# foges/pogs

Measured on AMD Instinct MI355X. Metric: admm_iterations_per_sec_dense_lasso_fp32 (per-GPU shard, summed over GPUs), higher is better.
Workload: dtype f32; 1 GPU; solve_lasso dense fp32 A=100000x10000 per GPU, lambda=0.1, default tolerances (BASELINE.json configs[1]); rows_per_gpu=100000, cols=10000, projector=direct (MFMA Gram + Cholesky), parallelism=row-shard x1, rccl_nranks=0

## Files before the change

include/pogs_amd.h:

```cpp
#ifndef POGS_AMD_H_
#define POGS_AMD_H_

#include <stddef.h>

#ifdef __cplusplus
extern "C" {
#endif


enum ORD { COL_MAJ, ROW_MAJ };

enum FUNCTION { ABS, EXP, HUBER, IDENTITY, INDBOX01, INDEQ0, INDGE0, INDLE0,
                LOGISTIC, MAXNEG0, MAXPOS0, NEGENTR, NEGLOG, RECIPR, SQUARE, ZERO };

enum POGS_STATUS { POGS_SUCCESS = 0, POGS_INFEASIBLE = 1, POGS_UNBOUNDED = 2,
                   POGS_MAX_ITER = 3, POGS_NAN_FOUND = 4, POGS_INVALID_CONE = 5,
                   POGS_ERROR = 6 };

int PogsD(enum ORD ord, size_t m, size_t n, const double *A,
          const double *f_a, const double *f_b, const double *f_c,
          const double *f_d, const double *f_e, const enum FUNCTION *f_h,
          const double *g_a, const double *g_b, const double *g_c,
          const double *g_d, const double *g_e, const enum FUNCTION *g_h,
          double rho, double abs_tol, double rel_tol, unsigned int max_iter,
          unsigned int verbose, int adaptive_rho, int gap_stop,
          double *x, double *y, double *l, double *optval, unsigned int *final_iter);

int PogsS(enum ORD ord, size_t m, size_t n, const float *A,
          const float *f_a, const float *f_b, const float *f_c,
          const float *f_d, const float *f_e, const enum FUNCTION *f_h,
          const float *g_a, const float *g_b, const float *g_c,
          const float *g_d, const float *g_e, const enum FUNCTION *g_h,
          float rho, float abs_tol, float rel_tol, unsigned int max_iter,
          unsigned int verbose, int adaptive_rho, int gap_stop,
          float *x, float *y, float *l, float *optval, unsigned int *final_iter);

int PogsSparseD(enum ORD ord, size_t m, size_t n, size_t nnz,
                const double *data, const int *ptr, const int *ind,
                const double *f_a, const double *f_b, const double *f_c,
                const double *f_d, const double *f_e, const enum FUNCTION *f_h,
                const double *g_a, const double *g_b, const double *g_c,
                const double *g_d, const double *g_e, const enum FUNCTION *g_h,
                double rho, double abs_tol, double rel_tol, unsigned int max_iter,
                unsigned int verbose, int adaptive_rho, int gap_stop,
                double *x, double *y, double *l, double *optval,
                unsigned int *final_iter);

int PogsSparseS(enum ORD ord, size_t m, size_t n, size_t nnz,
                const float *data, const int *ptr, const int *ind,
                const float *f_a, const float *f_b, const float *f_c,
                const float *f_d, const float *f_e, const enum FUNCTION *f_h,
                const float *g_a, const float *g_b, const float *g_c,
                const float *g_d, const float *g_e, const enum FUNCTION *g_h,
                float rho, float abs_tol, float rel_tol, unsigned int max_iter,
                unsigned int verbose, int adaptive_rho, int gap_stop,
                float *x, float *y, float *l, float *optval,
                unsigned int *final_iter);


typedef struct PogsAmdSolver PogsAmdSolver;

enum POGS_AMD_DTYPE { POGS_AMD_F32 = 0, POGS_AMD_F64 = 1 };
enum POGS_AMD_MEM { POGS_AMD_HOST = 0, POGS_AMD_DEVICE = 1 };
enum POGS_AMD_PROJECTOR { POGS_AMD_PROJ_DEFAULT = 0,
                          POGS_AMD_PROJ_DIRECT = 1, POGS_AMD_PROJ_CGLS = 2 };

#define POGS_AMD_UNIQUE_ID_BYTES 128

typedef struct PogsAmdDist {
  int rank;
  int world;
  size_t m_global;
  char unique_id[POGS_AMD_UNIQUE_ID_BYTES];
} PogsAmdDist;

typedef struct PogsAmdOptions {
  int device;
  int projector;
  int profile;
  int reserved[5];
} PogsAmdOptions;

typedef struct PogsAmdStats {
  double t_total_s, t_init_s, t_loop_s, t_h2d_s;
  unsigned int iterations;
  unsigned int exact_iters;
  unsigned int norm_est_iters;
  unsigned int rho_updates;
  unsigned long long cg_iters;
  unsigned long long matvecs;
  unsigned long long matvecs_init;
  double rho_final, nrmA;
  double stream_ms;
  unsigned long long stream_launches;
  double stream_bytes;
  double equil_ms, normest_ms, gram_ms, chol_ms, trtri_ms;
  double gram_flops;
  double reserved[8];
} PogsAmdStats;

int PogsAmdDistUniqueId(char *out);

int PogsAmdCreateDense(PogsAmdSolver **out, int dtype, enum ORD ord, size_t m,
                       size_t n, const void *A, int mem,
                       const PogsAmdOptions *opt, const PogsAmdDist *dist);

int PogsAmdCreateSparse(PogsAmdSolver **out, int dtype, enum ORD ord, size_t m,
                        size_t n, size_t nnz, const void *data, const int *ptr,
                        const int *ind, int mem, const PogsAmdOptions *opt,
                        const PogsAmdDist *dist);

int PogsAmdSolve(PogsAmdSolver *s,
                 const void *f_a, const void *f_b, const void *f_c, const void *f_d,
                 const void *f_e, const int *f_h,
                 const void *g_a, const void *g_b, const void *g_c, const void *g_d,
                 const void *g_e, const int *g_h,
                 double rho, double abs_tol, double rel_tol, unsigned int max_iter,
                 unsigned int verbose, int adaptive_rho, int gap_stop,
                 void *x, void *y, void *l, void *mu, double *optval,
                 unsigned int *final_iter);

typedef struct PogsAmdFn {
  const void *a, *b, *c, *d, *e;
  const int *h;
  double a0, b0, c0, d0, e0;
  int h0;
} PogsAmdFn;
int PogsAmdSolveFn(PogsAmdSolver *s, const PogsAmdFn *f, const PogsAmdFn *g,
                   double rho, double abs_tol, double rel_tol, unsigned int max_iter,
                   unsigned int verbose, int adaptive_rho, int gap_stop,
                   void *x, void *y, void *l, void *mu, double *optval,
                   unsigned int *final_iter);
int PogsAmdBeginRunFn(PogsAmdSolver *s, const PogsAmdFn *f, const PogsAmdFn *g,
                      double rho, double abs_tol, double rel_tol, unsigned int max_iter,
                      int adaptive_rho, int gap_stop);

#define POGS_AMD_BATCH_MAX 16
int PogsAmdSolveBatchFn(PogsAmdSolver *s, int k, const PogsAmdFn *f, const PogsAmdFn *g, const double *rho,
                        double abs_tol, double rel_tol, unsigned int max_iter, unsigned int verbose,
                        int adaptive_rho, int gap_stop, void *x, void *y, void *l, void *mu,
                        double *optval, unsigned int *final_iter, int *status);

int PogsAmdSolveBatchSparseFn(PogsAmdSolver *s, int k, const PogsAmdFn *f, const PogsAmdFn *g, const double *rho,
                              double abs_tol, double rel_tol, unsigned int max_iter, unsigned int verbose,
                              int adaptive_rho, int gap_stop, void *x, void *y, void *l, void *mu,
                              double *optval, unsigned int *final_iter, int *status);

#define POGS_AMD_MANY_MIN_DIM_MAX 512
#define POGS_AMD_MANY_MAX_DIM_MAX 16384
int PogsAmdSolveManyFn(int dtype, enum ORD ord, int k, size_t m, size_t n, const void *A, int mem,
                       const PogsAmdOptions *opt, const PogsAmdFn *f, const PogsAmdFn *g, const double *rho,
                       double abs_tol, double rel_tol, unsigned int max_iter, unsigned int verbose,
                       int adaptive_rho, int gap_stop, void *x, void *y, void *l, void *mu,
                       double *optval, unsigned int *final_iter, int *status);

int PogsAmdBeginRun(PogsAmdSolver *s,
                    const void *f_a, const void *f_b, const void *f_c, const void *f_d,
                    const void *f_e, const int *f_h,
                    const void *g_a, const void *g_b, const void *g_c, const void *g_d,
                    const void *g_e, const int *g_h,
                    double rho, double abs_tol, double rel_tol, unsigned int max_iter,
                    int adaptive_rho, int gap_stop);
int PogsAmdIterate(PogsAmdSolver *s, unsigned int iters, double *seconds,
                   unsigned int *solves_completed);

int PogsAmdSetWarmStart(PogsAmdSolver *s, const void *x0, const void *l0);

int PogsAmdGetStats(const PogsAmdSolver *s, PogsAmdStats *out);
int PogsAmdResetStats(PogsAmdSolver *s);
void PogsAmdDestroy(PogsAmdSolver *s);

const char *PogsAmdLastError(void);

typedef struct PogsAmdPoolInfo {
  unsigned long long mallocs;
  unsigned long long reuses;
  unsigned long long frees;
  double malloc_ms, free_ms;
  size_t cached_bytes;
  size_t live_bytes;
  size_t peak_cached_bytes;
} PogsAmdPoolInfo;
int PogsAmdPoolStats(int device, PogsAmdPoolInfo *out);
int PogsAmdPoolTrim(int device, size_t *freed_bytes);


int PogsAmdProxEval(int dtype, size_t n, const int *h, const void *a, const void *b,
                    const void *c, const void *d, const void *e, double rho,
                    const void *in, void *out);
int PogsAmdFuncEval(int dtype, size_t n, const int *h, const void *a, const void *b,
                    const void *c, const void *d, const void *e, const void *in,
                    double *out);
int PogsAmdProjSubgradEval(int dtype, size_t n, const int *h, const void *a, const void *b,
                           const void *c, const void *d, const void *e, const void *x_in,
                           const void *v_in, void *v_out);
int PogsAmdGetEquil(const PogsAmdSolver *s, void *A_eq, void *d, void *e, double *nrmA);
int PogsAmdProject(PogsAmdSolver *s, const void *x0, const void *y0, double tol,
                   void *x, void *y);
int PogsAmdMul(PogsAmdSolver *s, char trans, double alpha, const void *x, double beta,
               void *y);
int PogsAmdReadBandwidth(int device, size_t bytes, int reps, double *gb_per_s, int *pattern);
int PogsAmdWaveSumCheck(int dtype, size_t n, const void *in_host, void *alu_host, void *lds_host);

int PogsAmdBatchRowsCheck(int dtype, int tri, int rows, int cols, const void *M, size_t ldm, int k, const int *act,
                          int nact, const void *X, size_t ldx, void *Y, size_t ldy);
int PogsAmdBatchColsCheck(int dtype, int rows, int cols, const void *M, size_t ldm, int k, const int *act, int nact,
                          const void *U, size_t ldu, const void *add, void *Z, size_t ldz, int *nrb_used, int *rpb);
int PogsAmdSpBatchSpmvCheck(int dtype, int nrows, int ncols, const int *ptr, const int *ind, const void *val, int k,
                            const int *act, int nact, const void *X, size_t ldx, double beta, const void *yin,
                            size_t ldin, void *Y, size_t ldy, double *part, int num_cu, int *geom);
int PogsAmdManySetupCheck(int dtype, enum ORD ord, int k, size_t m, size_t n, const void *A, int mem, void *A_eq,
                          void *d, void *e, double *nrmA, void *W);
int PogsAmdGramCheck(int dtype, int kdim, int k, const void *P, size_t lda, int num_cu, int force, void *G, size_t ldg,
                     int *info);
int PogsAmdCholCheck(int dtype, int n, const void *H, size_t ldh, void *L, void *W, void *U, size_t ldo);
int PogsAmdSpmvCheck(int dtype, enum ORD ord, int nrows, int ncols, const int *ptr, const int *ind, const void *val,
                     int num_cu, int format, int force_rr_rows, int force_ncg, double scale, char trans, int sq,
                     double x_nrm2, double alpha, double beta, const void *x, size_t xlen, void *y, size_t ylen,
                     double *sumsq, int *info, int *t_ptr, int *t_ind, void *t_val);
int PogsAmdGetFactor(const PogsAmdSolver *s, void *W, void *U);
int PogsAmdRandUniform(int dtype, size_t n, void *out_host);

#ifdef __cplusplus
}
#endif
#endif
```

pogs_amd/_lib.py:

```python
import ctypes
import os
import sys

_PKG = os.path.dirname(os.path.abspath(__file__))
LIB_PATH = os.path.join(_PKG, "libpogs_amd.so")

TORCH_LOADED_FIRST = "torch" in sys.modules
if not TORCH_LOADED_FIRST and os.environ.get("POGS_AMD_TORCH_PRELOAD", "0") == "1":
    try:
        import torch

        TORCH_LOADED_FIRST = True
    except ImportError:
        pass


def check_device_pointer_interop():
    if "torch" in sys.modules and not TORCH_LOADED_FIRST:
        raise RuntimeError(
            "pogs_amd was imported before torch: the two then run on separate HIP runtimes and a torch device "
            "pointer is not valid here.  Import torch first, or set POGS_AMD_TORCH_PRELOAD=1.")


if not os.path.exists(LIB_PATH):
    raise ImportError(
        "pogs_amd: %s not found. Build it with:\n"
        "  python pogs_amd/build.py        (needs hipcc; cross-compiles for gfx950 without a GPU)\n" % LIB_PATH
    )

lib = ctypes.CDLL(LIB_PATH)

c_int, c_uint, c_size_t, c_double, c_float, c_void_p, c_char = (
    ctypes.c_int, ctypes.c_uint, ctypes.c_size_t, ctypes.c_double, ctypes.c_float, ctypes.c_void_p, ctypes.c_char)

UNIQUE_ID_BYTES = 128
F32, F64 = 0, 1
HOST, DEVICE = 0, 1
COL_MAJ, ROW_MAJ = 0, 1
PROJ_DEFAULT, PROJ_DIRECT, PROJ_CGLS = 0, 1, 2


class PogsAmdDist(ctypes.Structure):
    _fields_ = [("rank", c_int), ("world", c_int), ("m_global", c_size_t), ("unique_id", c_char * UNIQUE_ID_BYTES)]


class PogsAmdOptions(ctypes.Structure):
    _fields_ = [("device", c_int), ("projector", c_int), ("profile", c_int), ("reserved", c_int * 5)]


class PogsAmdStats(ctypes.Structure):
    _fields_ = [
        ("t_total_s", c_double), ("t_init_s", c_double), ("t_loop_s", c_double), ("t_h2d_s", c_double),
        ("iterations", c_uint), ("exact_iters", c_uint), ("norm_est_iters", c_uint), ("rho_updates", c_uint),
        ("cg_iters", ctypes.c_ulonglong), ("matvecs", ctypes.c_ulonglong), ("matvecs_init", ctypes.c_ulonglong),
        ("rho_final", c_double), ("nrmA", c_double),
        ("stream_ms", c_double), ("stream_launches", ctypes.c_ulonglong), ("stream_bytes", c_double),
        ("equil_ms", c_double), ("normest_ms", c_double), ("gram_ms", c_double), ("chol_ms", c_double),
        ("trtri_ms", c_double), ("gram_flops", c_double), ("reserved", c_double * 8),
    ]

    def as_dict(self):
        d = {k: getattr(self, k) for k, _ in self._fields_ if k != "reserved"}
        d["spec_hits"], d["spec_misses"] = self.reserved[0], self.reserved[1]
        d["collectives"] = int(self.reserved[2])
        d["comm_nranks"] = int(self.reserved[3])
        d["batch_problem_iters"] = int(self.reserved[4])
        d["batch_pass_ms"], d["batch_pass_launches"] = self.reserved[5], int(self.reserved[6])
        d["batch_pass_bytes"] = self.reserved[7]
        return d


def _dense_sig(real):
    return [c_int, c_size_t, c_size_t, c_void_p] + [c_void_p] * 5 + [c_void_p] + [c_void_p] * 5 + [c_void_p] + \
        [real, real, real, c_uint, c_uint, c_int, c_int, c_void_p, c_void_p, c_void_p, c_void_p, c_void_p]


def _sparse_sig(real):
    return [c_int, c_size_t, c_size_t, c_size_t, c_void_p, c_void_p, c_void_p] + [c_void_p] * 5 + [c_void_p] + \
        [c_void_p] * 5 + [c_void_p] + [real, real, real, c_uint, c_uint, c_int, c_int,
                                        c_void_p, c_void_p, c_void_p, c_void_p, c_void_p]


lib.PogsD.argtypes = _dense_sig(c_double)
lib.PogsS.argtypes = _dense_sig(c_float)
lib.PogsSparseD.argtypes = _sparse_sig(c_double)
lib.PogsSparseS.argtypes = _sparse_sig(c_float)
for _f in (lib.PogsD, lib.PogsS, lib.PogsSparseD, lib.PogsSparseS):
    _f.restype = c_int

lib.PogsAmdDistUniqueId.argtypes = [c_void_p]
lib.PogsAmdCreateDense.argtypes = [ctypes.POINTER(c_void_p), c_int, c_int, c_size_t, c_size_t, c_void_p, c_int,
                                   ctypes.POINTER(PogsAmdOptions), ctypes.POINTER(PogsAmdDist)]
lib.PogsAmdCreateSparse.argtypes = [ctypes.POINTER(c_void_p), c_int, c_int, c_size_t, c_size_t, c_size_t, c_void_p,
                                    c_void_p, c_void_p, c_int, ctypes.POINTER(PogsAmdOptions),
                                    ctypes.POINTER(PogsAmdDist)]
lib.PogsAmdSolve.argtypes = [c_void_p] + [c_void_p] * 12 + [c_double, c_double, c_double, c_uint, c_uint, c_int, c_int,
                                                            c_void_p, c_void_p, c_void_p, c_void_p,
                                                            ctypes.POINTER(c_double), ctypes.POINTER(c_uint)]
class PogsAmdFn(ctypes.Structure):
    _fields_ = [("a", c_void_p), ("b", c_void_p), ("c", c_void_p), ("d", c_void_p), ("e", c_void_p), ("h", c_void_p),
                ("a0", c_double), ("b0", c_double), ("c0", c_double), ("d0", c_double), ("e0", c_double), ("h0", c_int)]


lib.PogsAmdSolveFn.argtypes = [c_void_p, ctypes.POINTER(PogsAmdFn), ctypes.POINTER(PogsAmdFn), c_double, c_double, c_double,
                               c_uint, c_uint, c_int, c_int, c_void_p, c_void_p, c_void_p, c_void_p,
                               ctypes.POINTER(c_double), ctypes.POINTER(c_uint)]
lib.PogsAmdSolveBatchFn.argtypes = [c_void_p, c_int, ctypes.POINTER(PogsAmdFn), ctypes.POINTER(PogsAmdFn), c_void_p,
                                    c_double, c_double, c_uint, c_uint, c_int, c_int, c_void_p, c_void_p, c_void_p,
                                    c_void_p, c_void_p, c_void_p, c_void_p]
lib.PogsAmdSolveBatchSparseFn.argtypes = lib.PogsAmdSolveBatchFn.argtypes
BATCH_MAX = 16
lib.PogsAmdSolveManyFn.argtypes = [c_int, c_int, c_int, c_size_t, c_size_t, c_void_p, c_int, ctypes.POINTER(PogsAmdOptions),
                                   ctypes.POINTER(PogsAmdFn), ctypes.POINTER(PogsAmdFn), c_void_p, c_double, c_double,
                                   c_uint, c_uint, c_int, c_int, c_void_p, c_void_p, c_void_p, c_void_p, c_void_p,
                                   c_void_p, c_void_p]
MANY_MIN_DIM_MAX = 512
MANY_MAX_DIM_MAX = 16384
lib.PogsAmdBeginRunFn.argtypes = [c_void_p, ctypes.POINTER(PogsAmdFn), ctypes.POINTER(PogsAmdFn), c_double, c_double, c_double,
                                  c_uint, c_int, c_int]
lib.PogsAmdBeginRun.argtypes = [c_void_p] + [c_void_p] * 12 + [c_double, c_double, c_double, c_uint, c_int, c_int]
lib.PogsAmdIterate.argtypes = [c_void_p, c_uint, ctypes.POINTER(c_double), ctypes.POINTER(c_uint)]
lib.PogsAmdSetWarmStart.argtypes = [c_void_p, c_void_p, c_void_p]
lib.PogsAmdGetStats.argtypes = [c_void_p, ctypes.POINTER(PogsAmdStats)]
lib.PogsAmdResetStats.argtypes = [c_void_p]
lib.PogsAmdDestroy.argtypes = [c_void_p]
lib.PogsAmdDestroy.restype = None
lib.PogsAmdLastError.restype = ctypes.c_char_p
lib.PogsAmdProxEval.argtypes = [c_int, c_size_t] + [c_void_p] * 6 + [c_double, c_void_p, c_void_p]
lib.PogsAmdFuncEval.argtypes = [c_int, c_size_t] + [c_void_p] * 6 + [c_void_p, ctypes.POINTER(c_double)]
lib.PogsAmdProjSubgradEval.argtypes = [c_int, c_size_t] + [c_void_p] * 6 + [c_void_p, c_void_p, c_void_p]
lib.PogsAmdGetEquil.argtypes = [c_void_p, c_void_p, c_void_p, c_void_p, ctypes.POINTER(c_double)]
lib.PogsAmdProject.argtypes = [c_void_p, c_void_p, c_void_p, c_double, c_void_p, c_void_p]
lib.PogsAmdMul.argtypes = [c_void_p, c_char, c_double, c_void_p, c_double, c_void_p]
lib.PogsAmdRandUniform.argtypes = [c_int, c_size_t, c_void_p]
lib.PogsAmdReadBandwidth.argtypes = [c_int, c_size_t, c_int, ctypes.POINTER(c_double), ctypes.POINTER(c_int)]
lib.PogsAmdWaveSumCheck.argtypes = [c_int, c_size_t, c_void_p, c_void_p, c_void_p]
lib.PogsAmdBatchRowsCheck.argtypes = [c_int, c_int, c_int, c_int, c_void_p, c_size_t, c_int, c_void_p, c_int,
                                      c_void_p, c_size_t, c_void_p, c_size_t]
lib.PogsAmdBatchColsCheck.argtypes = [c_int, c_int, c_int, c_void_p, c_size_t, c_int, c_void_p, c_int, c_void_p,
                                      c_size_t, c_void_p, c_void_p, c_size_t, ctypes.POINTER(c_int),
                                      ctypes.POINTER(c_int)]
lib.PogsAmdSpBatchSpmvCheck.argtypes = [c_int, c_int, c_int, c_void_p, c_void_p, c_void_p, c_int, c_void_p, c_int,
                                        c_void_p, c_size_t, c_double, c_void_p, c_size_t, c_void_p, c_size_t, c_void_p,
                                        c_int, c_void_p]
lib.PogsAmdManySetupCheck.argtypes = [c_int, c_int, c_int, c_size_t, c_size_t, c_void_p, c_int, c_void_p, c_void_p,
                                      c_void_p, c_void_p, c_void_p]
lib.PogsAmdGramCheck.argtypes = [c_int, c_int, c_int, c_void_p, c_size_t, c_int, c_int, c_void_p, c_size_t, c_void_p]
lib.PogsAmdCholCheck.argtypes = [c_int, c_int, c_void_p, c_size_t, c_void_p, c_void_p, c_void_p, c_size_t]
lib.PogsAmdSpmvCheck.argtypes = [c_int, c_int, c_int, c_int, c_void_p, c_void_p, c_void_p, c_int, c_int, c_int, c_int,
                                 c_double, c_char, c_int, c_double, c_double, c_double, c_void_p, c_size_t, c_void_p,
                                 c_size_t, ctypes.POINTER(c_double), c_void_p, c_void_p, c_void_p, c_void_p]
lib.PogsAmdGetFactor.argtypes = [c_void_p, c_void_p, c_void_p]
GRAM_AUTO, GRAM_NATIVE, GRAM_TILE_128, GRAM_TILE_256 = 0, 1, 128, 256
GRAM_INFO = ("path", "tile", "ksplit", "kchunk", "kacc", "units", "unit_rows", "tile_map")
SPMV_AUTO, SPMV_TAGS, SPMV_TWO, SPMV_PLAIN = 0, 1, 2, 3
SPMV_INFO = ("tiled", "two", "rr_rows", "nrr", "ncb", "ncg", "units", "why")
SPMV_WHY = {0: "tiled", 1: "no non-zeros", 2: "plan too large", 3: "planner range", 4: "padding", 5: "row count over 16 bits",
            6: "pinned plain"}


class PogsAmdPoolInfo(ctypes.Structure):
    _fields_ = [("mallocs", ctypes.c_ulonglong), ("reuses", ctypes.c_ulonglong), ("frees", ctypes.c_ulonglong),
                ("malloc_ms", c_double), ("free_ms", c_double), ("cached_bytes", c_size_t), ("live_bytes", c_size_t),
                ("peak_cached_bytes", c_size_t)]


lib.PogsAmdPoolStats.argtypes = [c_int, ctypes.POINTER(PogsAmdPoolInfo)]
lib.PogsAmdPoolTrim.argtypes = [c_int, ctypes.POINTER(c_size_t)]


def pool_stats(device=-1):
    info = PogsAmdPoolInfo()
    if lib.PogsAmdPoolStats(device, ctypes.byref(info)) != 0:
        raise RuntimeError(last_error())
    return {k: getattr(info, k) for k, _ in info._fields_}


def pool_trim(device=-1):
    freed = c_size_t(0)
    if lib.PogsAmdPoolTrim(device, ctypes.byref(freed)) != 0:
        raise RuntimeError(last_error())
    return freed.value

ABI_SYMBOLS = [
    "PogsD", "PogsS", "PogsSparseD", "PogsSparseS",
    "PogsAmdDistUniqueId", "PogsAmdCreateDense", "PogsAmdCreateSparse", "PogsAmdSolve", "PogsAmdSolveFn", "PogsAmdSolveBatchFn", "PogsAmdSolveBatchSparseFn",
    "PogsAmdSolveManyFn", "PogsAmdBeginRun", "PogsAmdBeginRunFn",
    "PogsAmdIterate", "PogsAmdSetWarmStart", "PogsAmdGetStats", "PogsAmdResetStats", "PogsAmdDestroy", "PogsAmdLastError",
    "PogsAmdPoolStats", "PogsAmdPoolTrim",
    "PogsAmdProxEval", "PogsAmdFuncEval", "PogsAmdProjSubgradEval", "PogsAmdGetEquil", "PogsAmdProject", "PogsAmdMul", "PogsAmdRandUniform",
    "PogsAmdReadBandwidth", "PogsAmdWaveSumCheck", "PogsAmdBatchRowsCheck", "PogsAmdBatchColsCheck",
    "PogsAmdSpBatchSpmvCheck", "PogsAmdManySetupCheck", "PogsAmdGramCheck", "PogsAmdCholCheck",
    "PogsAmdSpmvCheck", "PogsAmdGetFactor",
]


def read_bandwidth(device=-1, nbytes=4 << 30, reps=10):
    gbs, pat = c_double(0.0), c_int(0)
    if lib.PogsAmdReadBandwidth(device, nbytes, reps, ctypes.byref(gbs), ctypes.byref(pat)) != 0:
        raise RuntimeError(last_error())
    return gbs.value, ("side-by-side grid stride", "row blocks")[pat.value]


def wave_sum_check(values):
    import numpy as np
    v = np.ascontiguousarray(values)
    assert v.dtype in (np.float32, np.float64) and v.size % 64 == 0
    a, b = np.empty_like(v), np.empty_like(v)
    if lib.PogsAmdWaveSumCheck(0 if v.dtype == np.float32 else 1, v.size, v.ctypes.data, a.ctypes.data, b.ctypes.data) != 0:
        raise RuntimeError(last_error())
    return a, b


def _dtype_code(*arrays):
    import numpy as np
    dt = arrays[0].dtype
    if dt not in (np.float32, np.float64) or any(a.dtype != dt for a in arrays[1:]):
        raise ValueError("float32 or float64 arrays of one dtype")
    return 0 if dt == np.float32 else 1


def _act(act):
    import numpy as np
    return np.ascontiguousarray(act, dtype=np.int32).ravel()


def batch_rows_check(tri, M, cols, X, Y, act):
    import numpy as np
    M, X = np.ascontiguousarray(M), np.ascontiguousarray(X)
    Y = np.array(Y, order="C", copy=True)
    code = _dtype_code(M, X, Y)
    if M.ndim != 2 or X.ndim != 2 or Y.ndim != 2 or X.shape[0] != Y.shape[0]:
        raise ValueError("M (rows, ldm), X (k, ldx), Y (k, ldy)")
    a = _act(act)
    if lib.PogsAmdBatchRowsCheck(code, tri, M.shape[0], cols, M.ctypes.data, M.shape[1], X.shape[0], a.ctypes.data,
                                 a.size, X.ctypes.data, X.shape[1], Y.ctypes.data, Y.shape[1]) != 0:
        raise RuntimeError(last_error())
    return Y


def batch_cols_check(M, cols, U, Z, act, add=None):
    import numpy as np
    M, U = np.ascontiguousarray(M), np.ascontiguousarray(U)
    Z = np.array(Z, order="C", copy=True)
    arrays = (M, U, Z) if add is None else (M, U, Z, np.ascontiguousarray(add))
    code = _dtype_code(*arrays)
    if M.ndim != 2 or U.ndim != 2 or Z.ndim != 2 or U.shape[0] != Z.shape[0] or \
            (add is not None and arrays[3].shape != Z.shape):
        raise ValueError("M (rows, ldm), U (k, ldu), Z and add (k, ldz)")
    a = _act(act)
    nrb, rpb = c_int(0), c_int(0)
    if lib.PogsAmdBatchColsCheck(code, M.shape[0], cols, M.ctypes.data, M.shape[1], U.shape[0], a.ctypes.data, a.size,
                                 U.ctypes.data, U.shape[1], None if add is None else arrays[3].ctypes.data,
                                 Z.ctypes.data, Z.shape[1], ctypes.byref(nrb), ctypes.byref(rpb)) != 0:
        raise RuntimeError(last_error())
    return Z, nrb.value, rpb.value


def sp_batch_spmv_check(ptr, ind, val, ncols, X, Y, act, beta=0.0, yin=None, part_fill=None, num_cu=0):
    import numpy as np
    ptr, ind = np.ascontiguousarray(ptr, dtype=np.int32), np.ascontiguousarray(ind, dtype=np.int32)
    val, X = np.ascontiguousarray(val), np.ascontiguousarray(X)
    Y = np.array(Y, order="C", copy=True)
    arrays = (val, X, Y) if yin is None else (val, X, Y, np.ascontiguousarray(yin))
    code = _dtype_code(*arrays)
    nrows = ptr.size - 1
    if X.ndim != 2 or Y.ndim != 2 or X.shape[0] != Y.shape[0] or nrows < 0 or \
            (yin is not None and (arrays[3].ndim != 2 or arrays[3].shape[0] != Y.shape[0])):
        raise ValueError("ptr (nrows + 1), X (k, ldx), Y (k, ldy), yin (k, ldin)")
    nnz = max(int(ptr[-1]), 0) if ptr.size else 0
    if ind.size < nnz or val.size < nnz:
        raise ValueError("ind and val must hold ptr[-1] entries")
    a = _act(act)
    k = X.shape[0]
    part = None
    if part_fill is not None:
        part = np.full(k * max(1, -(-nrows // 4)), part_fill, dtype=np.float64)
    geom = np.zeros(3, dtype=np.int32)
    if lib.PogsAmdSpBatchSpmvCheck(code, nrows, ncols, ptr.ctypes.data, ind.ctypes.data, val.ctypes.data, k,
                                   a.ctypes.data, a.size, X.ctypes.data, X.shape[1], beta,
                                   None if yin is None else arrays[3].ctypes.data,
                                   0 if yin is None else arrays[3].shape[1], Y.ctypes.data, Y.shape[1],
                                   None if part is None else part.ctypes.data, num_cu, geom.ctypes.data) != 0:
        raise RuntimeError(last_error())
    grid = int(geom[2])
    return Y, (None if part is None else part[:k * grid].reshape(k, grid)), tuple(int(g) for g in geom)


def many_setup_check(A, ord=ROW_MAJ):
    import numpy as np
    A = np.asarray(A)
    if A.ndim != 3:
        raise ValueError("A must be k x m x n")
    code = _dtype_code(A)
    k, m, n = A.shape
    src = np.ascontiguousarray(A.transpose(0, 2, 1) if ord == COL_MAJ else A)
    K = min(m, n)
    out = dict(A_eq=np.empty((k, m, n), A.dtype), d=np.empty((k, m), A.dtype), e=np.empty((k, n), A.dtype),
               nrmA=np.empty(k, np.float64), W=np.empty((k, K, K), A.dtype))
    if lib.PogsAmdManySetupCheck(code, ord, k, m, n, src.ctypes.data, HOST, out["A_eq"].ctypes.data,
                                 out["d"].ctypes.data, out["e"].ctypes.data, out["nrmA"].ctypes.data,
                                 out["W"].ctypes.data) != 0:
        raise RuntimeError(last_error())
    return out


def gram_check(P, k, G, force=GRAM_AUTO, num_cu=0):
    import numpy as np
    P = np.ascontiguousarray(P)
    G = np.array(G, order="C", copy=True)
    code = _dtype_code(P, G)
    if P.ndim != 2 or G.ndim != 2 or G.shape[0] != k:
        raise ValueError("P (kdim, lda), G (k, ldg)")
    info = np.zeros(8, dtype=np.int32)
    if lib.PogsAmdGramCheck(code, P.shape[0], k, P.ctypes.data, P.shape[1], num_cu, force, G.ctypes.data, G.shape[1],
                            info.ctypes.data) != 0:
        raise RuntimeError(last_error())
    return G, dict(zip(GRAM_INFO, (int(v) for v in info)))


def spmv_check(ptr, ind, val, shape, x, y, trans="n", ord=ROW_MAJ, num_cu=0, format=SPMV_AUTO, force_rr_rows=0,
               force_ncg=0, scale=1.0, sq=False, x_nrm2=0.0, alpha=1.0, beta=0.0, transpose=False):
    import numpy as np
    ptr, ind = np.ascontiguousarray(ptr, dtype=np.int32), np.ascontiguousarray(ind, dtype=np.int32)
    val, x = np.ascontiguousarray(val), np.ascontiguousarray(x)
    y = np.array(y, order="C", copy=True)
    code = _dtype_code(val, x, y)
    nrows, ncols = int(shape[0]), int(shape[1])
    r1, c1 = (nrows, ncols) if ord == ROW_MAJ else (ncols, nrows)
    if ptr.ndim != 1 or ptr.size != r1 + 1 or x.ndim != 1 or y.ndim != 1:
        raise ValueError("ptr (rows of the given copy + 1), x and y vectors")
    nnz = max(int(ptr[-1]), 0)
    if ind.size < nnz or val.size < nnz:
        raise ValueError("ind and val must hold ptr[-1] entries")
    info = np.zeros(16, dtype=np.int32)
    sumsq = c_double(0.0)
    t = None
    if transpose:
        t = (np.zeros(c1 + 1, np.int32), np.zeros(max(nnz, 1), np.int32), np.zeros(max(nnz, 1), val.dtype))
    if lib.PogsAmdSpmvCheck(code, ord, nrows, ncols, ptr.ctypes.data, ind.ctypes.data, val.ctypes.data, num_cu, format,
                            force_rr_rows, force_ncg, scale, trans.encode(), int(bool(sq)), x_nrm2, alpha, beta,
                            x.ctypes.data, x.size, y.ctypes.data, y.size, ctypes.byref(sumsq), info.ctypes.data,
                            *((None, None, None) if t is None else (a.ctypes.data for a in t))) != 0:
        raise RuntimeError(last_error())
    infos = tuple(dict(zip(SPMV_INFO, (int(v) for v in info[8 * c:8 * c + 8]))) for c in range(2))
    if t is None:
        return y, sumsq.value, infos
    return y, sumsq.value, infos, (t[0], t[1][:nnz], t[2][:nnz])


def chol_check(H, ldo=None):
    import numpy as np
    H = np.ascontiguousarray(H)
    code = _dtype_code(H)
    if H.ndim != 2 or H.shape[1] < H.shape[0]:
        raise ValueError("H (n, ldh >= n)")
    n = H.shape[0]
    ldo = n if ldo is None else ldo
    L, W, U = (np.full((n, ldo), np.nan, H.dtype) for _ in range(3))
    if lib.PogsAmdCholCheck(code, n, H.ctypes.data, H.shape[1], L.ctypes.data, W.ctypes.data, U.ctypes.data, ldo) != 0:
        raise RuntimeError(last_error())
    return L, W, U


def get_factor(handle, k, dtype):
    import numpy as np
    W, U = np.zeros((k, k), dtype), np.zeros((k, k), dtype)
    if lib.PogsAmdGetFactor(handle, W.ctypes.data, U.ctypes.data) != 0:
        raise RuntimeError(last_error())
    return W, U


def last_error():
    msg = lib.PogsAmdLastError()
    return msg.decode() if msg else ""
```

pogs_amd/csrc/abi.hip:

```cpp
#include <cmath>
#include <cstring>
#include <string>
#include <utility>
#include <vector>

#include "engine.h"
#include "factor_check.h"
#include "many_kernels.h"
#include "sparse_batch_kernels.h"
#include "spmv_check.h"
#include "prox.h"
#include "stream.h"
#include "vec_kernels.h"

namespace pogs_amd {

#define POGS_DECLARE_PLAN(TPB_, NV_)                                                                               \
  SolverBase *make_dense_solver_f32_p##TPB_##_##NV_(int, size_t, size_t, const void *, int, const PogsAmdOptions *, \
                                                    const PogsAmdDist *);                                          \
  SolverBase *make_dense_solver_f64_p##TPB_##_##NV_(int, size_t, size_t, const void *, int, const PogsAmdOptions *, \
                                                    const PogsAmdDist *);
POGS_STREAM_PLANS(POGS_DECLARE_PLAN)
#undef POGS_DECLARE_PLAN
SolverBase *make_dense_solver_f32_xl(int, size_t, size_t, const void *, int, const PogsAmdOptions *, const PogsAmdDist *);
// ... 237 lines not shown
    DistComm::unique_id(out);
    return 0;
  });
}

int PogsAmdCreateDense(PogsAmdSolver **out, int dtype, enum ORD ord, size_t m, size_t n, const void *A, int mem,
                       const PogsAmdOptions *opt, const PogsAmdDist *dist) {
  return guarded([&]() {
    *out = nullptr;
    DeviceGuard guard(opt ? opt->device : -1);
    std::unique_ptr<PogsAmdSolver> h(new PogsAmdSolver);
    h->impl.reset(make_dense_solver(dtype, ord, m, n, A, mem, opt, dist));
    *out = h.release();
    return 0;
  });
}

int PogsAmdCreateSparse(PogsAmdSolver **out, int dtype, enum ORD ord, size_t m, size_t n, size_t nnz,
                        const void *data, const int *ptr, const int *ind, int mem, const PogsAmdOptions *opt,
                        const PogsAmdDist *dist) {
  return guarded([&]() {
    *out = nullptr;
    DeviceGuard guard(opt ? opt->device : -1);
    std::unique_ptr<PogsAmdSolver> h(new PogsAmdSolver);
    h->impl.reset(make_sparse_solver(dtype, ord, m, n, nnz, data, ptr, ind, mem, opt, dist));
    *out = h.release();
    return 0;
  });
}

int PogsAmdSolve(PogsAmdSolver *s, const void *f_a, const void *f_b, const void *f_c, const void *f_d,
                 const void *f_e, const int *f_h, const void *g_a, const void *g_b, const void *g_c,
                 const void *g_d, const void *g_e, const int *g_h, double rho, double abs_tol, double rel_tol,
                 unsigned int max_iter, unsigned int verbose, int adaptive_rho, int gap_stop, void *x, void *y,
                 void *l, void *mu, double *optval, unsigned int *final_iter) {
  return guarded([&]() {
    POGS_CHECK(s && s->impl, "null solver");
    DeviceGuard guard(s->impl->device());
    const FnHost f = fn_arrays(f_a, f_b, f_c, f_d, f_e, f_h, "f");
    const FnHost g = fn_arrays(g_a, g_b, g_c, g_d, g_e, g_h, "g");
    return s->impl->solve(f, g, make_params(rho, abs_tol, rel_tol, max_iter, verbose, adaptive_rho, gap_stop), x,
                          y, l, mu, optval, final_iter);
  }, s);
}

namespace {
FnHost fn_host(const PogsAmdFn *p) {
  POGS_CHECK(p != nullptr, "null function description");
  FnHost f{p->a, p->b, p->c, p->d, p->e, p->h};
  f.s0[0] = p->a0; f.s0[1] = p->b0; f.s0[2] = p->c0; f.s0[3] = p->d0; f.s0[4] = p->e0;
  f.h0 = p->h0;
  POGS_CHECK(p->h || (p->h0 >= 0 && p->h0 <= 15), "function code out of range");
  return f;
}
std::pair<std::vector<FnHost>, std::vector<FnHost>> fn_hosts(const std::string &what, int k, const PogsAmdFn *f,
                                                             const PogsAmdFn *g, const void *x,
                                                             const unsigned *final_iter, const int *status) {
  POGS_CHECK(f && g, (what + ": null function descriptions").c_str());
  POGS_CHECK(x && final_iter && status, (what + ": x, final_iter and status must not be NULL").c_str());
  std::pair<std::vector<FnHost>, std::vector<FnHost>> fg;
  for (int j = 0; j < k; ++j) {
    fg.first.push_back(fn_host(&f[j]));
    fg.second.push_back(fn_host(&g[j]));
  }
  return fg;
}
}

int PogsAmdSolveFn(PogsAmdSolver *s, const PogsAmdFn *f, const PogsAmdFn *g, double rho, double abs_tol, double rel_tol,
                   unsigned int max_iter, unsigned int verbose, int adaptive_rho, int gap_stop, void *x, void *y, void *l,
                   void *mu, double *optval, unsigned int *final_iter) {
  return guarded([&]() {
    POGS_CHECK(s && s->impl, "null solver");
    DeviceGuard guard(s->impl->device());
    const FnHost fh = fn_host(f), gh = fn_host(g);
    return s->impl->solve(fh, gh, make_params(rho, abs_tol, rel_tol, max_iter, verbose, adaptive_rho, gap_stop), x, y, l, mu,
                          optval, final_iter);
  }, s);
}

int PogsAmdSolveBatchFn(PogsAmdSolver *s, int k, const PogsAmdFn *f, const PogsAmdFn *g, const double *rho,
                        double abs_tol, double rel_tol, unsigned int max_iter, unsigned int verbose, int adaptive_rho,
                        int gap_stop, void *x, void *y, void *l, void *mu, double *optval, unsigned int *final_iter,
                        int *status) {
  return guarded([&]() {
    POGS_CHECK(s && s->impl, "null solver");
    POGS_CHECK(k >= 1 && k <= POGS_AMD_BATCH_MAX, "batched solve: k must be in [1, POGS_AMD_BATCH_MAX]");
    const auto fg = fn_hosts("batched solve", k, f, g, x, final_iter, status);
    DeviceGuard guard(s->impl->device());
    s->impl->solve_batch(k, fg.first.data(), fg.second.data(), rho,
                         make_params(1.0, abs_tol, rel_tol, max_iter, verbose, adaptive_rho, gap_stop),
                         BatchOut{x, y, l, mu, optval, final_iter, status});
    return 0;
  }, s);
}

int PogsAmdSolveBatchSparseFn(PogsAmdSolver *s, int k, const PogsAmdFn *f, const PogsAmdFn *g, const double *rho,
                              double abs_tol, double rel_tol, unsigned int max_iter, unsigned int verbose,
                              int adaptive_rho, int gap_stop, void *x, void *y, void *l, void *mu, double *optval,
                              unsigned int *final_iter, int *status) {
  return guarded([&]() {
    POGS_CHECK(s && s->impl, "null solver");
    POGS_CHECK(k >= 1 && k <= POGS_AMD_BATCH_MAX, "batched solve: k must be in [1, POGS_AMD_BATCH_MAX]");
    const auto fg = fn_hosts("batched solve", k, f, g, x, final_iter, status);
    DeviceGuard guard(s->impl->device());
    s->impl->solve_batch_sparse(k, fg.first.data(), fg.second.data(), rho,
                                make_params(1.0, abs_tol, rel_tol, max_iter, verbose, adaptive_rho, gap_stop),
                                BatchOut{x, y, l, mu, optval, final_iter, status});
    return 0;
  }, s);
}

int PogsAmdSolveManyFn(int dtype, enum ORD ord, int k, size_t m, size_t n, const void *A, int mem,
                       const PogsAmdOptions *opt, const PogsAmdFn *f, const PogsAmdFn *g, const double *rho,
                       double abs_tol, double rel_tol, unsigned int max_iter, unsigned int verbose, int adaptive_rho,
                       int gap_stop, void *x, void *y, void *l, void *mu, double *optval, unsigned int *final_iter,
                       int *status) {
  return guarded([&]() {
    POGS_CHECK(k >= 1, "many-problem solve: k must be >= 1");
    const int projector = opt ? opt->projector : POGS_AMD_PROJ_DEFAULT;
    POGS_CHECK(projector == POGS_AMD_PROJ_DEFAULT || projector == POGS_AMD_PROJ_DIRECT,
               "many-problem solve: only the direct projector is supported (CGLS refused)");
    const int device = opt ? opt->device : -1;
    const auto fg = fn_hosts("many-problem solve", k, f, g, x, final_iter, status);
    DeviceGuard guard(device);
    solve_many(dtype, static_cast<int>(ord), k, m, n, A, mem, device, fg.first.data(), fg.second.data(), rho,
               make_params(1.0, abs_tol, rel_tol, max_iter, verbose, adaptive_rho, gap_stop),
               BatchOut{x, y, l, mu, optval, final_iter, status});
    return 0;
  });
}

int PogsAmdBeginRunFn(PogsAmdSolver *s, const PogsAmdFn *f, const PogsAmdFn *g, double rho, double abs_tol, double rel_tol,
                      unsigned int max_iter, int adaptive_rho, int gap_stop) {
  return guarded([&]() {
    POGS_CHECK(s && s->impl, "null solver");
    DeviceGuard guard(s->impl->device());
    const FnHost fh = fn_host(f), gh = fn_host(g);
    s->impl->begin_run(fh, gh, make_params(rho, abs_tol, rel_tol, max_iter, 0, adaptive_rho, gap_stop));
    return 0;
  }, s);
}

int PogsAmdBeginRun(PogsAmdSolver *s, const void *f_a, const void *f_b, const void *f_c, const void *f_d,
                    const void *f_e, const int *f_h, const void *g_a, const void *g_b, const void *g_c,
                    const void *g_d, const void *g_e, const int *g_h, double rho, double abs_tol, double rel_tol,
                    unsigned int max_iter, int adaptive_rho, int gap_stop) {
  return guarded([&]() {
    POGS_CHECK(s && s->impl, "null solver");
    DeviceGuard guard(s->impl->device());
    const FnHost f = fn_arrays(f_a, f_b, f_c, f_d, f_e, f_h, "f");
    const FnHost g = fn_arrays(g_a, g_b, g_c, g_d, g_e, g_h, "g");
    s->impl->begin_run(f, g, make_params(rho, abs_tol, rel_tol, max_iter, 0, adaptive_rho, gap_stop));
    return 0;
  }, s);
}

int PogsAmdIterate(PogsAmdSolver *s, unsigned int iters, double *seconds, unsigned int *solves_completed) {
  return guarded([&]() {
    POGS_CHECK(s && s->impl, "null solver");
    DeviceGuard guard(s->impl->device());
    s->impl->iterate(iters, seconds, solves_completed);
    return 0;
  }, s);
}

int PogsAmdSetWarmStart(PogsAmdSolver *s, const void *x0, const void *l0) {
  return guarded([&]() {
    POGS_CHECK(s && s->impl && x0 && l0, "warm start needs both x0 and l0 (pogs.cpp:159-179)");
    DeviceGuard guard(s->impl->device());
    s->impl->set_warm_start(x0, l0);
    return 0;
  });
}

int PogsAmdGetStats(const PogsAmdSolver *s, PogsAmdStats *out) {
  return guarded([&]() {
    POGS_CHECK(s && s->impl && out, "null argument");
    *out = const_cast<PogsAmdSolver *>(s)->impl->stats();
    return 0;
  });
}

int PogsAmdResetStats(PogsAmdSolver *s) {
  return guarded([&]() {
    POGS_CHECK(s && s->impl, "null solver");
    DeviceGuard guard(s->impl->device());
    PogsAmdStats &st = s->impl->stats();
    st.t_loop_s = 0; st.iterations = 0; st.exact_iters = 0; st.rho_updates = 0;
    st.cg_iters = 0; st.matvecs = 0;
    st.stream_ms = 0; st.stream_launches = 0; st.stream_bytes = 0;
    st.reserved[0] = 0; st.reserved[1] = 0;
    return 0;
  });
}

void PogsAmdDestroy(PogsAmdSolver *s) {
  try {
    if (!s) return;
    DeviceGuard guard(s->impl ? s->impl->device() : -1);
    delete s;
  } catch (...) {}
}

const char *PogsAmdLastError(void) { return g_last_error.c_str(); }

int PogsAmdPoolStats(int device, PogsAmdPoolInfo *out) {
  return guarded([&]() {
    POGS_CHECK(out, "null argument");
    int dev = device;
    if (dev < 0) POGS_HIP_CHECK(hipGetDevice(&dev));
    const PoolCounters c = DevicePool::get().counters(dev);
    out->mallocs = c.mallocs; out->reuses = c.reuses; out->frees = c.frees;
    out->malloc_ms = c.malloc_ms; out->free_ms = c.free_ms;
    out->cached_bytes = c.cached_bytes; out->live_bytes = c.live_bytes;
    out->peak_cached_bytes = c.peak_cached_bytes;
    return 0;
  });
}

int PogsAmdPoolTrim(int device, size_t *freed_bytes) {
  return guarded([&]() {
    const size_t b = DevicePool::get().trim(device);
    if (freed_bytes) *freed_bytes = b;
    return 0;
  });
}

int PogsAmdProxEval(int dtype, size_t n, const int *h, const void *a, const void *b, const void *c, const void *d,
                    const void *e, double rho, const void *in, void *out) {
  return guarded([&]() {
    if (dtype == POGS_AMD_F32) prox_eval_host<float>(n, h, a, b, c, d, e, rho, in, out, nullptr);
    else prox_eval_host<double>(n, h, a, b, c, d, e, rho, in, out, nullptr);
    return 0;
  });
}

int PogsAmdFuncEval(int dtype, size_t n, const int *h, const void *a, const void *b, const void *c, const void *d,
                    const void *e, const void *in, double *out) {
  return guarded([&]() {
    if (dtype == POGS_AMD_F32) prox_eval_host<float>(n, h, a, b, c, d, e, 1.0, in, nullptr, out);
    else prox_eval_host<double>(n, h, a, b, c, d, e, 1.0, in, nullptr, out);
    return 0;
  });
}

int PogsAmdProjSubgradEval(int dtype, size_t n, const int *h, const void *a, const void *b, const void *c,
                           const void *d, const void *e, const void *x_in, const void *v_in, void *v_out) {
  return guarded([&]() {
    POGS_CHECK(x_in && v_in && v_out, "null argument");
    if (dtype == POGS_AMD_F32) prox_eval_host<float>(n, h, a, b, c, d, e, 1.0, v_in, v_out, nullptr, x_in);
    else prox_eval_host<double>(n, h, a, b, c, d, e, 1.0, v_in, v_out, nullptr, x_in);
    return 0;
  });
}

int PogsAmdGetEquil(const PogsAmdSolver *s, void *A_eq, void *d, void *e, double *nrmA) {
  return guarded([&]() {
    POGS_CHECK(s && s->impl, "null solver");
    DeviceGuard guard(s->impl->device());
    const_cast<PogsAmdSolver *>(s)->impl->get_equil(A_eq, d, e, nrmA);
    return 0;
  });
}

int PogsAmdProject(PogsAmdSolver *s, const void *x0, const void *y0, double tol, void *x, void *y) {
  return guarded([&]() {
    POGS_CHECK(s && s->impl, "null solver");
    DeviceGuard guard(s->impl->device());
    s->impl->project(x0, y0, tol, x, y);
    return 0;
  });
}

int PogsAmdMul(PogsAmdSolver *s, char trans, double alpha, const void *x, double beta, void *y) {
  return guarded([&]() {
    POGS_CHECK(s && s->impl, "null solver");
    DeviceGuard guard(s->impl->device());
    s->impl->mul(trans, alpha, x, beta, y);
    return 0;
  });
}

int PogsAmdReadBandwidth(int device, size_t bytes, int reps, double *gb_per_s, int *pattern) {
  return guarded([&]() {
    POGS_CHECK(gb_per_s && bytes >= (1u << 20), "null argument / fewer than 1 MiB");
    DeviceGuard guard(device);
    int pat = 0;
    *gb_per_s = measure_read_bandwidth_gbs(bytes, reps, &pat);
    if (pattern) *pattern = pat;
    return 0;
  });
}

int PogsAmdWaveSumCheck(int dtype, size_t n, const void *in_host, void *alu_host, void *lds_host) {
  return guarded([&]() {
    POGS_CHECK(in_host && alu_host && lds_host, "null argument");
    if (dtype == POGS_AMD_F32) wave_sum_check(static_cast<const float *>(in_host), n, static_cast<float *>(alu_host), static_cast<float *>(lds_host));
    else wave_sum_check(static_cast<const double *>(in_host), n, static_cast<double *>(alu_host), static_cast<double *>(lds_host));
    return 0;
  });
}

int PogsAmdBatchRowsCheck(int dtype, int tri, int rows, int cols, const void *M, size_t ldm, int k, const int *act,
                          int nact, const void *X, size_t ldx, void *Y, size_t ldy) {
  return guarded([&]() {
    POGS_CHECK(dtype == POGS_AMD_F32 || dtype == POGS_AMD_F64, "unknown dtype");
    if (dtype == POGS_AMD_F32)
      batch_rows_check<float>(tri, rows, cols, static_cast<const float *>(M), ldm, k, act, nact,
                              static_cast<const float *>(X), ldx, static_cast<float *>(Y), ldy);
    else
      batch_rows_check<double>(tri, rows, cols, static_cast<const double *>(M), ldm, k, act, nact,
                               static_cast<const double *>(X), ldx, static_cast<double *>(Y), ldy);
    return 0;
  });
}

int PogsAmdBatchColsCheck(int dtype, int rows, int cols, const void *M, size_t ldm, int k, const int *act, int nact,
                          const void *U, size_t ldu, const void *add, void *Z, size_t ldz, int *nrb_used, int *rpb) {
  return guarded([&]() {
    POGS_CHECK(dtype == POGS_AMD_F32 || dtype == POGS_AMD_F64, "unknown dtype");
    if (dtype == POGS_AMD_F32)
      batch_cols_check<float>(rows, cols, static_cast<const float *>(M), ldm, k, act, nact,
                              static_cast<const float *>(U), ldu, static_cast<const float *>(add),
                              static_cast<float *>(Z), ldz, nrb_used, rpb);
    else
      batch_cols_check<double>(rows, cols, static_cast<const double *>(M), ldm, k, act, nact,
                               static_cast<const double *>(U), ldu, static_cast<const double *>(add),
                               static_cast<double *>(Z), ldz, nrb_used, rpb);
    return 0;
  });
}

int PogsAmdSpBatchSpmvCheck(int dtype, int nrows, int ncols, const int *ptr, const int *ind, const void *val, int k,
                            const int *act, int nact, const void *X, size_t ldx, double beta, const void *yin,
                            size_t ldin, void *Y, size_t ldy, double *part, int num_cu, int *geom) {
  return guarded([&]() {
    POGS_CHECK(dtype == POGS_AMD_F32 || dtype == POGS_AMD_F64, "unknown dtype");
    if (dtype == POGS_AMD_F32)
      sp_batch_spmv_check<float>(nrows, ncols, ptr, ind, static_cast<const float *>(val), k, act, nact,
                                 static_cast<const float *>(X), ldx, static_cast<float>(beta),
                                 static_cast<const float *>(yin), ldin, static_cast<float *>(Y), ldy, part, num_cu,
                                 geom);
    else
      sp_batch_spmv_check<double>(nrows, ncols, ptr, ind, static_cast<const double *>(val), k, act, nact,
                                  static_cast<const double *>(X), ldx, beta, static_cast<const double *>(yin), ldin,
                                  static_cast<double *>(Y), ldy, part, num_cu, geom);
    return 0;
  });
}

int PogsAmdManySetupCheck(int dtype, enum ORD ord, int k, size_t m, size_t n, const void *A, int mem, void *A_eq,
                          void *d, void *e, double *nrmA, void *W) {
  return guarded([&]() {
    many_setup_check(dtype, static_cast<int>(ord), k, m, n, A, mem, A_eq, d, e, nrmA, W);
    return 0;
  });
}

int PogsAmdGramCheck(int dtype, int kdim, int k, const void *P, size_t lda, int num_cu, int force, void *G, size_t ldg,
                     int *info) {
  return guarded([&]() {
    POGS_CHECK(dtype == POGS_AMD_F32 || dtype == POGS_AMD_F64, "unknown dtype");
    if (dtype == POGS_AMD_F32)
      gram_check<float>(kdim, k, static_cast<const float *>(P), lda, num_cu, force, static_cast<float *>(G), ldg, info);
    else
      gram_check<double>(kdim, k, static_cast<const double *>(P), lda, num_cu, force, static_cast<double *>(G), ldg, info);
    return 0;
  });
}

int PogsAmdCholCheck(int dtype, int n, const void *H, size_t ldh, void *L, void *W, void *U, size_t ldo) {
  return guarded([&]() {
    POGS_CHECK(dtype == POGS_AMD_F32 || dtype == POGS_AMD_F64, "unknown dtype");
    if (dtype == POGS_AMD_F32)
      chol_check<float>(n, static_cast<const float *>(H), ldh, static_cast<float *>(L), static_cast<float *>(W),
                        static_cast<float *>(U), ldo);
    else
      chol_check<double>(n, static_cast<const double *>(H), ldh, static_cast<double *>(L), static_cast<double *>(W),
                         static_cast<double *>(U), ldo);
    return 0;
  });
}

int PogsAmdSpmvCheck(int dtype, enum ORD ord, int nrows, int ncols, const int *ptr, const int *ind, const void *val,
                     int num_cu, int format, int force_rr_rows, int force_ncg, double scale, char trans, int sq,
                     double x_nrm2, double alpha, double beta, const void *x, size_t xlen, void *y, size_t ylen,
                     double *sumsq, int *info, int *t_ptr, int *t_ind, void *t_val) {
  return guarded([&]() {
    const SpmvCheckArgs a{dtype, static_cast<int>(ord), nrows, ncols, ptr, ind, val, num_cu, format, force_rr_rows,
                          force_ncg, scale, trans, sq, x_nrm2, alpha, beta, x, xlen, y, ylen, sumsq, info, t_ptr, t_ind,
                          t_val};
    spmv_check(a);
    return 0;
  });
}

int PogsAmdGetFactor(const PogsAmdSolver *s, void *W, void *U) {
  return guarded([&]() {
    POGS_CHECK(s && s->impl, "null solver");
    DeviceGuard guard(s->impl->device());
    const_cast<PogsAmdSolver *>(s)->impl->get_factor(W, U);
    return 0;
  });
}

int PogsAmdRandUniform(int dtype, size_t n, void *out_host) {
  return guarded([&]() {
    if (dtype == POGS_AMD_F32) rand_uniform_host(static_cast<float *>(out_host), n);
    else rand_uniform_host(static_cast<double *>(out_host), n);
    return 0;
  });
}

}
```

pogs_amd/csrc/dense_factor.h:

```cpp

template <typename T, typename Tag>
void DenseSolver<T, Tag>::factor() {
  hipStream_t s = ctx_.stream;
  const size_t ld = k_pad_;
  planW_ = make_stream_plan<T>(k_pad_, ctx_.num_cu);
  ensure_xl(planW_, k_, k_pad_);
  const size_t slab = static_cast<size_t>(k_) * ld;
  fac_.alloc(slab * 4);
  fac_.zero(s);
  T *G = fac_.p, *tmp = fac_.p + slab;
  Wp_ = fac_.p + 2 * slab;
  Up_ = fac_.p + 3 * slab;
  {
    PhaseTimer pt(s);
    const int kdim = tall_ ? m_ : n_;
    gram_product<T>(A_.p, lda_, kdim, k_, tall_ || tmode_, amax_, ctx_.num_cu, G, ld, 0, ctx_);
    if (multi_) {
      const size_t cnt = packed_lower_count(k_, ld);
      if (ld % Vec16<T>::N == 0 && cnt <= slab) {
        launch_pack_lower<T>(G, ld, k_, tmp, false, s);
        ctx_.dist.allreduce(tmp, cnt, s);
        launch_pack_lower<T>(G, ld, k_, tmp, true, s);
        POGS_HIP_CHECK(hipMemsetAsync(tmp, 0, cnt * sizeof(T), s));
      } else {
        ctx_.dist.allreduce(G, slab, s);
      }
    }
    ctx_.stats.gram_ms = pt.stop_ms();
    ctx_.stats.gram_flops = static_cast<double>(kdim) * k_ * k_;
  }
  ctx_.tmark("gram");
  if (tall_) norm_est_gram(G, ld);
  else if (tmode_) norm_est_gram_wide(G, ld);
  ctx_.tmark("norm_est_gram");
  launch_add_diag<T>(G, ld, k_, static_cast<T>(1), s);
  {
    PhaseTimer pt(s);
    cholesky_lower<T>(G, ld, k_, Wp_, ld, s);
    ctx_.stats.chol_ms = pt.stop_ms();
  }
  ctx_.tmark("cholesky");
  {
    PhaseTimer pt(s);
    trtri_lower<T>(G, ld, k_, Wp_, ld, tmp, s);
    launch_transpose<T>(Wp_, ld, k_, k_, Up_, ld, s);
    ctx_.stats.trtri_ms = pt.stop_ms();
  }
  ctx_.sync();
  ctx_.tmark("trtri");
}

template <typename T, typename Tag>
template <typename TailOp>
void DenseSolver<T, Tag>::solve_gram(const T *rhs, const T *add, const TailOp &tail, double *tail_scalars) {
  hipStream_t s = ctx_.stream;
  StreamArgs<T> a;
  a.A = Wp_; a.lda = k_pad_; a.m = k_; a.n_pad = k_pad_;
  a.xin = rhs; a.xin_add = add; a.xin_nrm2 = nullptr;
  double *part = defer_sums_ ? ctx_.spart.p + sp_tail_off_ : ctx_.spart.p;
  a.col_partials = nullptr; a.scalar_partials = part;
  a.xl_scratch = xl_buf_.p;
  launch_stream<T, true, false, false, kLower, Tag>(planW_, a, GemvNOp<T>{1, 0, tvec_.p}, s);
  a.A = Up_;
  a.xin = tvec_.p; a.xin_add = nullptr;
  launch_stream<T, true, false, false, kUpper, Tag>(planW_, a, tail, s);
  if (TailOp::NS > 0 && tail_scalars) {
    SumJob j{part, stream_grid<true, false>(planW_, k_), TailOp::NS, tail_scalars};
    sum_now_or_later(j);
  }
}

template <typename T, typename Tag>
template <typename TailColOp>
void DenseSolver<T, Tag>::solve_gram_onepass(const T *rhs, const T *add, const TailColOp &tail, double *tail_scalars) {
  hipStream_t s = ctx_.stream;
  StreamArgs<T> a;
  a.A = Wp_; a.lda = k_pad_; a.m = k_; a.n_pad = k_pad_;
  a.xin = rhs; a.xin_add = add; a.xin_nrm2 = nullptr;
  a.col_partials = colpart_.p;
  a.scalar_partials = ctx_.spart.p;
  a.xl_scratch = xl_buf_.p;
  launch_stream<T, true, true, false, kLower, Tag>(planW_, a, IdentRowOp<T>{}, s);
  double *sp = ctx_.spart.p + sp_tail_off_;
  launch_reduce_cols<T, TailColOp>(colpart_.p, stream_grid<true, true>(planW_, k_), k_pad_, tail, sp, s);
  if (TailColOp::NS > 0 && tail_scalars) {
    SumJob j{sp, reduce_cols_grid(k_pad_, Vec16<T>::N), TailColOp::NS, tail_scalars};
    sum_now_or_later(j);
  }
}

template <typename T, typename Tag>
int DenseSolver<T, Tag>::cgls_project(const T *x0, const T *y0, T *x, T tol, const T *Ax_warm, T *yacc) {
  hipStream_t s = ctx_.stream;
  const int bx = vec_blocks(n_);
  const double shift = 1.0;
  const double kEps = std::numeric_limits<T>::epsilon();
  double *vp = ctx_.spart.p + static_cast<size_t>(planA_.grid_max) * 6;
  auto sum_vp = [&](int blocks, double *out) {
    SumJob j{vp, blocks, 1, out};
    launch_sum_jobs(&j, 1, s);
  };
  auto pass_n = [&](const T *xin, auto op, double *out, int ns) {
    StreamArgs<T> a = argsA();
    a.xin = xin;
    ctx_.stream_timer.begin(s);
    launch_stream<T, true, false, false, kFull, Tag>(planA_, a, op, s);
    ctx_.stream_timer.end(s);
    if (ns > 0) sum_row_scalars(stream_grid<true, false>(planA_, m_), ns, out);
    ctx_.stats.matvecs += 1;
  };
  auto pass_t = [&](const T *rin) {
    gemv_t_partials(rin);
    finish_cols(CgSColOp<T>{x, static_cast<T>(shift), cg_s_.p, n_}, ctx_.S.p + kCgS2, 0, 0);
    ctx_.stats.matvecs += 1;
  };
  if (Ax_warm) {
    hipLaunchKernelGGL(sub_norm_kernel<T>, dim3(vec_blocks(m_)), dim3(kVecTpb), 0, s, m_, y0, Ax_warm, cg_r_.p, vp);
    hipLaunchKernelGGL(sub_norm_kernel<T>, dim3(bx), dim3(kVecTpb), 0, s, n_, x, x0, x, vp);
  } else {
    hipLaunchKernelGGL(sub_norm_kernel<T>, dim3(bx), dim3(kVecTpb), 0, s, n_, x, x0, x, vp);
    sum_vp(bx, ctx_.S.p + kCgX2);
    pass_n(x0, SubDotOp<T>{y0, cg_q_.p}, nullptr, 0);
    const double *S0 = ctx_.fetch_scalars();
    if (std::sqrt(S0[kCgX2]) > 0.0) pass_n(x, SubDotOp<T>{cg_q_.p, cg_r_.p}, nullptr, 0);
    else POGS_HIP_CHECK(hipMemcpyAsync(cg_r_.p, cg_q_.p, m_ * sizeof(T), hipMemcpyDeviceToDevice, s));
  }
  pass_t(cg_r_.p);
  hipLaunchKernelGGL(set_gamma_kernel, dim3(1), dim3(1), 0, s, ctx_.S.p, cg_.p);
  hipLaunchKernelGGL(cg_update_p_kernel<T>, dim3(bx), dim3(kVecTpb), 0, s, n_, cg_.p, cg_s_.p, cg_p_.p, vp, true);
  sum_vp(bx, ctx_.S.p + kCgP2);
  const double *S = ctx_.fetch_scalars();
  const double norms0 = std::sqrt(S[kCgS2]);
  const int maxit = (norms0 < kEps) ? 0 : 500;
  int steps = 0;
  for (int k = 0; k < maxit; ++k) {
    pass_n(cg_p_.p, CgQRowOp<T>{cg_q_.p}, ctx_.S.p + kCgQ2, 1);
    hipLaunchKernelGGL(cg_alpha_kernel, dim3(1), dim3(1), 0, s, ctx_.S.p, cg_.p, shift, kEps);
    const int bm = vec_blocks(m_);
    hipLaunchKernelGGL(cg_update_xr_kernel<T>, dim3(bx + bm), dim3(kVecTpb), 0, s, n_, m_, cg_.p, cg_p_.p, x,
                       cg_q_.p, cg_r_.p, vp, bx,
                       (yacc && Ax_warm) ? (k == 0 ? Ax_warm : static_cast<const T *>(yacc)) : static_cast<const T *>(nullptr),
                       (yacc && Ax_warm) ? yacc : static_cast<T *>(nullptr));
    sum_vp(bx, ctx_.S.p + kCgX2);
    pass_t(cg_r_.p);
    hipLaunchKernelGGL(cg_beta_kernel, dim3(1), dim3(1), 0, s, ctx_.S.p, cg_.p);
    hipLaunchKernelGGL(cg_update_p_kernel<T>, dim3(bx), dim3(kVecTpb), 0, s, n_, cg_.p, cg_s_.p, cg_p_.p, vp, false);
    sum_vp(bx, ctx_.S.p + kCgP2);
    S = ctx_.fetch_scalars();
    const double norms = std::sqrt(S[kCgS2]), normx = std::sqrt(S[kCgX2]);
    ++ctx_.stats.cg_iters;
    ++steps;
    if ((norms <= norms0 * static_cast<double>(tol)) || (normx * static_cast<double>(tol) >= 1.0)) break;
  }
  launch_axpby<T>(n_, static_cast<T>(1), x0, static_cast<T>(1), x, s);
  return steps;
}
```

pogs_amd/csrc/dense_iter.h:

```cpp

template <typename T, typename Tag>
void DenseSolver<T, Tag>::load_problem(const FnHost &f, const FnHost &g, const SolveParams &p) {
  hipStream_t s = ctx_.stream;
  upload_fn<T>(f_, f, m_, s);
  upload_fn<T>(g_, g, n_, s);
  warn_negative_coeffs<T>(f, m_);
  warn_negative_coeffs<T>(g, n_);
  bool all_cheap = true, all_logistic = true;
  if (tmode_) {
    all_logistic = false;
    all_cheap = all_h(g, n_, [](int h) { return is_cheap_prox(h); });
  } else {
    all_cheap = all_h(f, m_, [](int h) { return is_cheap_prox(h); });
    all_logistic = all_h(f, m_, [](int h) { return h == kLogistic; });
  }
  pre_cheap_ = all_h(f, m_, [](int h) { return is_cheap_prox(h); }) && all_h(g, n_, [](int h) { return is_cheap_prox(h); });
  fused_now_ = fused_ok_ && (all_cheap || all_logistic);
  fused_logistic_ = fused_now_ && all_logistic && !all_cheap;
#ifndef POGS_NV5_CHEAP_BPC
#define POGS_NV5_CHEAP_BPC 2
#endif
  planA_.bpc_override = (POGS_NV5_CHEAP_BPC > 0 && fused_now_ && !fused_logistic_ && !tmode_ && std::is_same<T, float>::value &&
                         planA_.tpb == 256 && planA_.nv == 5) ? POGS_NV5_CHEAP_BPC : 0;
  planA_.pf = POGS_NV5_PREFETCH != 0 && fused_logistic_ && !tmode_ && std::is_same<T, float>::value && planA_.tpb == 256 &&
              planA_.nv == 5;
  launch_scale_objective<T>(f_.view(), fs_.a.p, fs_.c.p, fs_.d.p, fs_.e.p, d_.p, m_, true, s);
  launch_scale_objective<T>(g_.view(), gs_.a.p, gs_.c.p, gs_.d.p, gs_.e.p, e_.p, n_, false, s);
  ctl_ = make_admm_control<T>(p, p.rho, ctx_.m_global, n_);
  ctl_.say_rho = p.verbose > 3 && ctx_.dist.rank() == 0;
  loaded_ = true;
  ctx_.sync();
}

template <typename T, typename Tag>
void DenseSolver<T, Tag>::cold_start() {
  hipStream_t s = ctx_.stream;
  for (int i = 0; i < 2; ++i) { x_[i].zero(s); y_[i].zero(s); }
  xt_.zero(s); yt_.zero(s); xtemp_.zero(s); ytemp_.zero(s);
  cur_ = 0;
  zt_scale_ = 1;
  spec_valid_ = false;
  exact_mode_ = false;
  colparts_ = 0;
  proj_count_ = 0;
  ctl_.reset();
}

template <typename T, typename Tag>
void DenseSolver<T, Tag>::apply_warm_start() {
  if (!warm_pending_) return;
  warm_pending_ = false;
  hipStream_t s = ctx_.stream;
  const T rho = ctl_.rho;
  POGS_HIP_CHECK(hipMemcpyAsync(xtemp_.p, warm_x_.data(), n_ * sizeof(T), hipMemcpyHostToDevice, s));
  POGS_HIP_CHECK(hipMemcpyAsync(ytemp_.p, warm_l_.data(), m_ * sizeof(T), hipMemcpyHostToDevice, s));
  launch_scale_by<T>(n_, static_cast<T>(1), xtemp_.p, e_.p, true, x_[cur_].p, s);
  launch_scale_by<T>(m_, static_cast<T>(1), ytemp_.p, d_.p, true, yt_.p, s);
  if (tmode_) {
    t_mul_n(x_[cur_].p, nullptr, GemvNOp<T>{1, 0, y_[cur_].p}, nullptr);
    t_mul_t(yt_.p, StoreColOp<T>{static_cast<T>(1) / rho, 0, xt_.p, n_}, nullptr);
  } else {
    StreamArgs<T> a = argsA();
    a.xin = x_[cur_].p;
    launch_stream<T, true, false, false, kFull, Tag>(planA_, a, GemvNOp<T>{1, 0, y_[cur_].p}, s);
    gemv_t_partials(yt_.p);
    finish_cols(StoreColOp<T>{static_cast<T>(1) / rho, 0, xt_.p, n_}, nullptr, 0, 0);
  }
  launch_scal<T>(yt_.p, static_cast<T>(-1) / rho, m_, s);
  ctx_.sync();
  xtemp_.zero(s);
  ytemp_.zero(s);
}

template <typename T, typename Tag>
bool DenseSolver<T, Tag>::iteration(unsigned verbose) {
  if (fused_now_) return tmode_ ? iteration_fused_wide(verbose) : iteration_fused(verbose);
  hipStream_t s = ctx_.stream;
  const int nw = cur_ ^ 1;
  const bool multi = multi_;
  AdmmPreArgs<T> pa;
  pa.n_x = n_; pa.n_y = m_;
  pa.g = gview(); pa.f = fview();
  pa.x_cur = x_[cur_].p; pa.y_cur = y_[cur_].p;
  pa.xt = xt_.p; pa.yt = yt_.p;
  pa.zt_scale = zt_scale_;
  pa.x12 = x12_.p; pa.y12 = y12_.p;
  pa.xtemp = xtemp_.p; pa.ytemp = ytemp_.p;
  pa.rho = ctl_.rho; pa.alpha = ctl_.alpha(); pa.cheap = pre_cheap_;
  pa.partials = ctx_.spart.p;
  pa.blocks_x = pre_blocks(n_);
  launch_admm_pre<T>(pa, s);
  {
    SumJob j[2] = {{ctx_.spart.p, pa.blocks_x, 3, ctx_.S.p + kGapX},
                   {ctx_.spart.p + static_cast<size_t>(pa.blocks_x) * 3, pre_blocks(m_), 3, ctx_.S.p + kGapY}};
    launch_sum_jobs(j, 2, s);
  }
  if (use_cgls_) {
    POGS_HIP_CHECK(hipMemcpyAsync(x_[nw].p, x_[cur_].p, n_ * sizeof(T), hipMemcpyDeviceToDevice, s));
    const bool ysync = ysync_ <= 0 || (proj_count_ % static_cast<unsigned long long>(ysync_)) == 0;
    ++proj_count_;
    const int steps = cgls_project(xtemp_.p, ytemp_.p, x_[nw].p, ctl_.proj_tol(), y_[cur_].p, ysync ? nullptr : y_[nw].p);
    if (ysync) {
      StreamArgs<T> a = argsA();
      a.xin = x_[nw].p;
      ctx_.stream_timer.begin(s);
      launch_stream<T, true, false, false, kFull, Tag>(planA_, a,
                                                  ProjTailOp<T>{y_[nw].p, y_[cur_].p, y12_.p, ytemp_.p}, s);
      ctx_.stream_timer.end(s);
      sum_row_scalars(stream_grid<true, false>(planA_, m_), 2, ctx_.S.p + kDYprev2);
      ctx_.stats.matvecs += 1;
    } else {
      if (steps == 0) POGS_HIP_CHECK(hipMemcpyAsync(y_[nw].p, y_[cur_].p, m_ * sizeof(T), hipMemcpyDeviceToDevice, s));
      double *spy = ctx_.spart.p;
      launch_admm_tail<T>(m_, y_[nw].p, y_[cur_].p, y12_.p, ytemp_.p, spy, s);
      SumJob jy{spy, vec_blocks(m_), 2, ctx_.S.p + kDYprev2};
      launch_sum_jobs(&jy, 1, s);
    }
    double *sp2 = ctx_.spart.p + static_cast<size_t>(planA_.grid_max) * 6;
    launch_admm_tail<T>(n_, x_[nw].p, x_[cur_].p, x12_.p, xtemp_.p, sp2, s);
    SumJob jt{sp2, vec_blocks(n_), 2, ctx_.S.p + kDXprev2};
    launch_sum_jobs(&jt, 1, s);
  } else if (tall_) {
    gemv_t_partials(ytemp_.p);
    finish_cols(StoreColOp<T>{1, 0, rhs_.p, n_}, nullptr, kGapY, 3);
    solve_gram_onepass(rhs_.p, xtemp_.p, ProjTailSumColOp<T>{x_[nw].p, x_[cur_].p, x12_.p, xtemp_.p, n_},
                       ctx_.S.p + kDXprev2);
    StreamArgs<T> a = argsA();
    a.xin = x_[nw].p;
    ctx_.stream_timer.begin(s);
    launch_stream<T, true, false, false, kFull, Tag>(planA_, a,
                                                ProjTailOp<T>{y_[nw].p, y_[cur_].p, y12_.p, ytemp_.p}, s);
    ctx_.stream_timer.end(s);
    sum_row_scalars(stream_grid<true, false>(planA_, m_), 2, ctx_.S.p + kDYprev2);
    if (multi) ctx_.dist.allreduce(ctx_.S.p + kDYprev2, 2, s);
  } else {
    t_mul_n(xtemp_.p, nullptr, ResidOp<T>{ytemp_.p, rhs_.p}, nullptr);
    solve_gram_onepass(rhs_.p, static_cast<const T *>(nullptr),
                       ProjTailAddColOp<T>{y_[nw].p, y_[cur_].p, y12_.p, ytemp_.p, tmpn_.p, m_},
                       ctx_.S.p + kDYprev2);
    t_mul_t(tmpn_.p, ProjTailColOp<T>{x_[nw].p, x_[cur_].p, x12_.p, xtemp_.p, n_}, ctx_.S.p + kDXprev2);
  }
  if (!use_cgls_) ctx_.stats.matvecs += 2;
  const double *S = ctx_.fetch_scalars();
  ctl_.set_pre(S);
  bool exact = false;
  if (ctl_.set_approx(S, nrmA_)) {
    StreamArgs<T> a = argsA();
    const int grid = stream_grid<true, true>(planA_, srows_);
    if (tmode_) {
      launch_exact_u<T>(m_, y12_.p, yt_.p, y_[cur_].p, zt_scale_, uvec_.p, s);
      a.xin = uvec_.p;
      ctx_.stream_timer.begin(s);
      launch_stream<T, true, true, false, kFull, Tag>(planA_, a, ExactTRowOp<T>{x12_.p, xt_.p, x_[cur_].p, zt_scale_}, s);
      ctx_.stream_timer.end(s);
      sum_row_scalars(grid, 1, ctx_.S.p + kExactS2);
      double *sp = ctx_.spart.p + static_cast<size_t>(planA_.grid_max) * 6;
      launch_reduce_cols<T, ExactTColOp<T>>(colpart_.p, grid, scols_pad_, ExactTColOp<T>{y12_.p, m_}, sp, s);
      SumJob j{sp, reduce_cols_grid(scols_pad_, Vec16<T>::N), 1, ctx_.S.p + kExactR2};
      launch_sum_jobs(&j, 1, s);
    } else {
      a.xin = x12_.p;
      ctx_.stream_timer.begin(s);
      launch_stream<T, true, true, false, kFull, Tag>(planA_, a,
                                                 ExactRowOp<T>{y12_.p, yt_.p, y_[cur_].p, zt_scale_}, s);
      ctx_.stream_timer.end(s);
      sum_row_scalars(grid, 1, ctx_.S.p + kExactR2);
      finish_cols(ExactColOp<T>{x12_.p, xt_.p, x_[cur_].p, zt_scale_, n_}, ctx_.S.p + kExactS2, kExactR2, 1, grid);
    }
    ctx_.stats.matvecs += 1;
    S = ctx_.fetch_scalars();
    ctl_.set_exact(S);
    exact = true;
  }
  const bool stop = ctl_.check_stop(exact);
  log_iteration(verbose);
  if (stop) return true;
  std::swap(xt_, xtemp_);
  std::swap(yt_, ytemp_);
  cur_ = nw;
  zt_scale_ = ctl_.adapt();
  ++ctl_.k;
  return false;
}

template <typename T, typename Tag>
bool DenseSolver<T, Tag>::iteration_fused(unsigned verbose) {
  hipStream_t s = ctx_.stream;
  const int nw = cur_ ^ 1;
  const int by = pre_blocks(m_);
  const int gridC = pre_cols_grid(n_pad_, Vec16<T>::N);
  struct DeferGuard {
    bool &flag;
    DeferGuard(bool &f, bool on) : flag(f) { flag = on; }
    ~DeferGuard() { flag = false; }
  } defer_guard(defer_sums_, true);
  const bool spec = spec_valid_;
  double *pre_part = ctx_.spart.p + sp_pre_off_;
  double *pc_part = pre_part + static_cast<size_t>(by) * 3;
  double *tail = pack_.p ? pack_.p + 2 * static_cast<size_t>(n_pad_) : nullptr;
  const size_t pack_count = 2 * static_cast<size_t>(n_pad_) + 6;
#ifndef POGS_LEAN_F32_NV5
#define POGS_LEAN_F32_NV5 0
#endif
  constexpr bool kLeanType = std::is_same<T, double>::value || (POGS_LEAN_F32_NV5 != 0 && Tag::has(256, 5) && !Tag::windows);
  const bool lean = kLeanType && !multi_ && !exact_mode_;
  int nparts = colparts_ > 0 ? colparts_ : stream2_grid<2>(planA_, m_);
  if (!spec) {
    AdmmPreArgs<T> pa;
    pa.n_x = 0; pa.n_y = m_;
    pa.g = gview(); pa.f = fview();
    pa.x_cur = x_[cur_].p; pa.y_cur = y_[cur_].p;
    pa.xt = xt_.p; pa.yt = yt_.p;
    pa.zt_scale = zt_scale_;
    pa.x12 = x12_.p; pa.y12 = y12_.p;
    pa.xtemp = xtemp_.p; pa.ytemp = ytemp_.p;
    pa.rho = ctl_.rho; pa.alpha = ctl_.alpha(); pa.cheap = pre_cheap_;
    pa.partials = pre_part;
    pa.blocks_x = 0;
    launch_admm_pre<T>(pa, s);
    const SumJob jy{pre_part, by, 3, ctx_.S.p + kGapY};
    StreamArgs2<T> a2{A_.p, lda_, m_, n_pad_, nullptr, nullptr, colpart_.p, colpart2_.p, ctx_.spart.p};
    ctx_.stream_timer.begin(s);
    launch_stream2<T, 0, 2, Tag>(planA_, a2, PreAccOp<T>{ytemp_.p, y12_.p, yt_.p, y_[cur_].p, zt_scale_}, s);
    ctx_.stream_timer.end(s);
    nparts = stream2_grid<0>(planA_, m_);
    ctx_.stats.matvecs += 1;
    if (!multi_) {
      sum_now_or_later(jy);
    } else {
      PackJobs pj;
      pj.j[0] = jy; pj.j[1] = jy; pj.njobs = 1;
      launch_pack_cols<T>(colpart_.p, colpart2_.p, nparts, n_pad_, pack_.p, pj, s);
      ctx_.dist.allreduce(pack_.p, pack_count, s);
      ScalarOverlay ov;
      ov.src = tail; ov.slot[0] = kGapY; ov.n[0] = 3;
      launch_apply_overlay(ctx_.S.p, ov, s);
    }
  }
  {
    PreColsArgs<T> pc;
    pc.part0 = colpart_.p; pc.part1 = (lean && spec) ? nullptr : colpart2_.p; pc.nparts = nparts;
    pc.tot64 = pack_.p;
    pc.n = n_; pc.n_pad = n_pad_;
    pc.g = gview();
    pc.x_cur = x_[cur_].p; pc.xt = xt_.p;
    pc.zt_scale = zt_scale_; pc.rho = ctl_.rho; pc.alpha = ctl_.alpha();
    pc.x12 = x12_.p; pc.xtemp = xtemp_.p; pc.rhs = rhs_.p;
    pc.partials = pc_part;
    launch_pre_cols<T>(pc, multi_, s);
    sum_now_or_later(SumJob{pc_part, gridC, 3, ctx_.S.p + kGapX, 4, 0});
    sum_now_or_later(SumJob{pc_part, gridC, 1, ctx_.S.p + kExactS2, 4, 3});
  }
  solve_gram_onepass(rhs_.p, xtemp_.p, ProjTailSumColOp<T>{x_[nw].p, x_[cur_].p, x12_.p, xtemp_.p, n_},
                     ctx_.S.p + kDXprev2);
  {
    StreamArgs2<T> a2{A_.p, lda_, m_, n_pad_, x_[nw].p, x12_.p, colpart_.p, colpart2_.p, ctx_.spart.p};
    ctl_.predict(&rho_pred_, &zs_pred_);
    ctx_.stream_timer.begin(s);
    int grid = stream2_grid<2>(planA_, m_);
    if (fused_logistic_) {
      FusedIterOp<T, true> op{y_[nw].p, y_[cur_].p, y12_.p, ytemp_.p, fview(), rho_pred_, ctl_.alpha(), zs_pred_,
                              y12s_.p, ytemps_.p};
      if constexpr (kLeanType) {
        if (lean) { launch_stream2<T, 1, 1, Tag>(planA_, a2, op, s); grid = stream2_grid<1, 1>(planA_, m_); }
        else launch_stream2<T, 2, 2, Tag>(planA_, a2, op, s);
      } else {
        launch_stream2<T, 2, 2, Tag>(planA_, a2, op, s);
      }
    } else {
      FusedIterOp<T, false> op{y_[nw].p, y_[cur_].p, y12_.p, ytemp_.p, fview(), rho_pred_, ctl_.alpha(), zs_pred_,
                               y12s_.p, ytemps_.p};
      if constexpr (kLeanType) {
        if (lean) { launch_stream2<T, 1, 1, Tag>(planA_, a2, op, s); grid = stream2_grid<1, 1>(planA_, m_); }
        else launch_stream2<T, 2, 2, Tag>(planA_, a2, op, s);
      } else {
        launch_stream2<T, 2, 2, Tag>(planA_, a2, op, s);
      }
    }
    ctx_.stream_timer.end(s);
    colparts_ = grid;
    const SumJob jd{ctx_.spart.p, grid, 3, ctx_.S.p + kDYprev2, 6, 0};
    const SumJob js{ctx_.spart.p, grid, 3, ctx_.S.p + kSpecGapY, 6, 3};
    if (!multi_) {
      sum_now_or_later(jd);
      sum_now_or_later(js);
    } else {
      PackJobs pj;
      pj.j[0] = jd; pj.j[1] = js; pj.njobs = 2;
      launch_pack_cols<T>(colpart_.p, colpart2_.p, grid, n_pad_, pack_.p, pj, s);
      ctx_.dist.allreduce(pack_.p, pack_count, s);
      ScalarOverlay ov;
      ov.src = tail;
      ov.slot[0] = kDYprev2; ov.n[0] = 3;
      ov.slot[1] = kSpecGapY; ov.n[1] = 3;
      ctx_.set_overlay(ov);
    }
    ctx_.stats.matvecs += 1;
  }
  double S[kNumSlots];
  std::memcpy(S, ctx_.fetch_scalars(), sizeof(S));
  if (spec)
    for (int q = 0; q < 3; ++q) S[kGapY + q] = spec_gap_[q];
  ctl_.set_pre(S);
  bool exact = false;
  bool drop_spec = false;
  if (ctl_.set_approx(S, nrmA_)) {
    if (lean) {
      StreamArgs<T> a = argsA();
      a.xin = x12_.p;
      a.col_partials = colpart2_.p;
      const int g1 = stream_grid<true, true>(planA_, srows_);
      ctx_.stream_timer.begin(s);
      launch_stream<T, true, true, false, kFull, Tag>(planA_, a, ExactRowOp<T>{y12_.p, yt_.p, y_[cur_].p, zt_scale_}, s);
      ctx_.stream_timer.end(s);
      sum_row_scalars(g1, 1, ctx_.S.p + kExactR2);
      finish_cols(ExactColOp<T>{x12_.p, xt_.p, x_[cur_].p, zt_scale_, n_}, ctx_.S.p + kExactS2, kExactR2, 1, g1, colpart2_.p);
      ctx_.stats.matvecs += 1;
      const double *S2 = ctx_.fetch_scalars();
      S[kExactR2] = S2[kExactR2];
      S[kExactS2] = S2[kExactS2];
      exact_mode_ = true;
      drop_spec = true;
    }
    ctl_.set_exact(S);
    exact = true;
  }
  const bool stop = ctl_.check_stop(exact);
  log_iteration(verbose);
  if (stop) return true;
  std::swap(xt_, xtemp_);
  std::swap(yt_, ytemp_);
  cur_ = nw;
  zt_scale_ = ctl_.adapt();
  if (!drop_spec && ctl_.rho == rho_pred_ && zt_scale_ == zs_pred_) {
    std::swap(ytemp_, ytemps_);
    std::swap(y12_, y12s_);
    for (int q = 0; q < 3; ++q) spec_gap_[q] = S[kSpecGapY + q];
    spec_valid_ = true;
    ctx_.stats.reserved[0] += 1;
  } else {
    spec_valid_ = false;
// ... 66 lines not shown
```

pogs_amd/csrc/dense_setup.h:

```cpp

template <typename T, typename Tag>
void DenseSolver<T, Tag>::upload(int ord, const void *A, int mem) {
  hipStream_t s = ctx_.stream;
  A_.alloc(static_cast<size_t>(srows_) * lda_);
  const hipMemcpyKind kind = (mem == POGS_AMD_DEVICE) ? hipMemcpyDeviceToDevice : hipMemcpyHostToDevice;
  const char *ae = std::getenv("POGS_AMD_ALIAS_INPUT");
  bool may_alias = mem == POGS_AMD_DEVICE && !(ae && ae[0] == '0') &&
                   (reinterpret_cast<uintptr_t>(A) % 16) == 0;
  if (may_alias) {
    hipPointerAttribute_t attr;
    if (hipPointerGetAttributes(&attr, A) != hipSuccess) {
      (void)hipGetLastError();
      may_alias = false;
    } else {
      may_alias = attr.type == hipMemoryTypeDevice && attr.device == ctx_.device;
    }
  }
  if (tmode_) {
    if (lda_ != static_cast<size_t>(m_)) A_.zero(s);
    if (ord != ROW_MAJ && may_alias && lda_ == static_cast<size_t>(m_)) {
      A_src_ = static_cast<const T *>(A);
    } else if (ord != ROW_MAJ) {
      POGS_HIP_CHECK(hipMemcpy2DAsync(A_.p, lda_ * sizeof(T), A, m_ * sizeof(T), m_ * sizeof(T), n_, kind, s));
    } else {
      DevBuf<T> stage;
      const T *src = static_cast<const T *>(A);
      if (mem != POGS_AMD_DEVICE) {
        stage.alloc(static_cast<size_t>(m_) * n_);
        POGS_HIP_CHECK(hipMemcpyAsync(stage.p, A, static_cast<size_t>(m_) * n_ * sizeof(T), kind, s));
        src = stage.p;
      }
      launch_transpose<T>(src, n_, m_, n_, A_.p, lda_, s);
      ctx_.sync();
    }
  } else if (ord == ROW_MAJ && may_alias && lda_ == static_cast<size_t>(n_)) {
    A_src_ = static_cast<const T *>(A);
  } else if (ord == ROW_MAJ) {
    if (lda_ != static_cast<size_t>(n_)) A_.zero(s);
    POGS_HIP_CHECK(hipMemcpy2DAsync(A_.p, lda_ * sizeof(T), A, n_ * sizeof(T), n_ * sizeof(T), m_, kind, s));
  } else {
    DevBuf<T> stage;
    const T *src = static_cast<const T *>(A);
    if (mem != POGS_AMD_DEVICE) {
      stage.alloc(static_cast<size_t>(m_) * n_);
      POGS_HIP_CHECK(hipMemcpyAsync(stage.p, A, static_cast<size_t>(m_) * n_ * sizeof(T), kind, s));
      src = stage.p;
    }
    if (lda_ != static_cast<size_t>(n_)) A_.zero(s);
    launch_transpose<T>(src, m_, n_, m_, A_.p, lda_, s);
    ctx_.sync();
  }
  ctx_.sync();
}

template <typename T, typename Tag>
void DenseSolver<T, Tag>::alloc_state() {
  hipStream_t s = ctx_.stream;
  const size_t np = n_pad_;
  const size_t mp = m_pad_;
  for (int i = 0; i < 2; ++i) { x_[i].alloc(np); y_[i].alloc(mp); x_[i].zero(s); y_[i].zero(s); }
  xt_.alloc(np); yt_.alloc(mp); xtemp_.alloc(np); ytemp_.alloc(mp);
  const size_t kp = std::max<size_t>(np, k_pad_);
  x12_.alloc(np); y12_.alloc(mp); rhs_.alloc(kp); tvec_.alloc(kp); tmpn_.alloc(kp);
  xt_.zero(s); yt_.zero(s); xtemp_.zero(s); ytemp_.zero(s); x12_.zero(s); y12_.zero(s);
  rhs_.zero(s); tvec_.zero(s); tmpn_.zero(s);
  d_.alloc(mp); d_.zero(s); e_.alloc(np); e_.zero(s);
  if (tmode_) { uvec_.alloc(mp); uvec_.zero(s); }
  xout_.alloc(np); yout_.alloc(m_); lout_.alloc(m_); muout_.alloc(np);
  f_.alloc(m_); g_.alloc(n_); fs_.alloc(m_); gs_.alloc(n_);
  colpart_.alloc(static_cast<size_t>(planA_.grid_max) * scols_pad_);
  ensure_xl(planA_, srows_, scols_pad_);
  if (use_cgls_) {
    cg_p_.alloc(np); cg_s_.alloc(np); cg_q_.alloc(m_); cg_r_.alloc(m_); cg_.alloc(kCgNumSlots);
    cg_p_.zero(s); cg_s_.zero(s); cg_.zero(s);
  }
  const char *fe = std::getenv("POGS_AMD_FUSED");
  fused_ok_ = (tall_ || tmode_) && !use_cgls_ && stream2_supported(planA_) && !(fe && fe[0] == '0');
  if (fused_ok_ && tmode_) {
    colpart2_.alloc(static_cast<size_t>(planA_.grid_max) * scols_pad_);
    x12s_.alloc(np); xtemps_.alloc(np);
    x12s_.zero(s); xtemps_.zero(s);
  } else if (fused_ok_) {
    colpart2_.alloc(static_cast<size_t>(planA_.grid_max) * np);
    if (multi_) {
      pack_.alloc(2 * np + 8);
      pack_.zero(s);
    }
    y12s_.alloc(m_); ytemps_.alloc(m_);
    y12s_.zero(s); ytemps_.zero(s);
  }
  const size_t vb = vec_blocks(n_) + vec_blocks(m_);
  const size_t r01 = static_cast<size_t>(planA_.grid_max) * 6 + std::max<size_t>(4096, vb * 3 + 64);
  sp_pre_off_ = r01;
  sp_tail_off_ = r01 + vb * 3 + static_cast<size_t>(pre_cols_grid(n_pad_, Vec16<T>::N)) * 4 + 64;
  ctx_.ensure_spart(sp_tail_off_ + static_cast<size_t>(ctx_.num_cu) * 32);
}

template <typename T, typename Tag>
void DenseSolver<T, Tag>::equilibrate() {
  hipStream_t s = ctx_.stream;
  PhaseTimer pt(s);
  const double mg = static_cast<double>(ctx_.m_global), nn = n_;
  const T ce = static_cast<T>(1e-4) * static_cast<T>(mg + nn) / static_cast<T>(mg);
  const T cd = static_cast<T>(1e-4) * static_cast<T>(mg + nn) / static_cast<T>(nn);
  const int gridACC = stream_grid<false, true>(planA_, srows_);
  const int gridBOTH = stream_grid<true, true>(planA_, srows_);
  StreamArgs<T> a = argsA();
  if (A_src_) a.A = A_src_;
  ctx_.tmark("  eq: start");
  const char *sk_env = std::getenv("POGS_AMD_SK_FULL");
  const bool sk_probe = !(sk_env && sk_env[0] == '1');
  double *mark = sk_probe ? ctx_.S.p + kSkMark : nullptr;
  const T sk_tol = (std::is_same<T, float>::value ? 16 : 64) * std::numeric_limits<T>::epsilon();
  double r_ref = 0, gamma = 0, gamma_prev = 0;
  bool extrapolate = false, was_uniform = false;
  auto sk_uniform = [&](int k, int count) {
    if (!mark || k < 1) return false;
    const double *S = ctx_.fetch_scalars();
    const double r_mean = S[kSkRatio] / count;
    const bool uniform = k >= 2 && S[kSkMark] < k + 1.0 && r_mean > 0.5 && r_mean < 2.0;
    r_ref = r_mean;
    gamma_prev = gamma;
    gamma = r_mean - 1.0;
    if (std::getenv("POGS_AMD_TRACE"))
      std::fprintf(stderr, "[pogs_amd trace]   sk pass %d: gamma %.6e, %s\n", k, r_mean - 1.0, uniform ? "uniform" : "stamped");
    const bool fire = uniform && (std::is_same<T, float>::value || was_uniform);
    was_uniform = uniform;
    return fire;
  };
  auto sk_log_growth = [&](int first, int count) {
    double q = 1.0;
    if (std::is_same<T, double>::value && gamma != 0 && gamma_prev != 0) {
      q = gamma / gamma_prev;
      if (!(q > 0.999 && q < 1.001)) q = 1.0;
    }
    double L = 0, gi = gamma * std::pow(q, first);
    for (int i = 0; i < count; ++i, gi *= q) L += std::log1p(gi);
    return L;
  };
  int k = 0;
  if (tmode_) {
    double *sp = ctx_.spart.p + static_cast<size_t>(planA_.grid_max) * 6;
    launch_fill<T>(d_.p, static_cast<T>(1), m_, s);
    for (; k < 50; ++k) {
      a.xin = d_.p;
      launch_stream<T, true, true, true, kFull, Tag>(planA_, a, SkRowOp<T>{static_cast<T>(mg), ce, e_.p}, s);
      launch_reduce_cols<T, SkColOp<T>>(
          colpart_.p, gridBOTH, scols_pad_,
          SkColOp<T>{static_cast<T>(nn), cd, d_.p, m_, mark, k + 1.0, sk_tol, static_cast<T>(r_ref)}, sp, s);
      SumJob j{sp, reduce_cols_grid(scols_pad_, Vec16<T>::N), 1, ctx_.S.p + kSkRatio};
      launch_sum_jobs(&j, 1, s);
      if (sk_uniform(k, m_)) { extrapolate = true; ++k; break; }
    }
    ctx_.stats.matvecs_init += k;
    if (extrapolate) {
      const double Ld = sk_log_growth(1, 50 - k);
      const double Le = -sk_log_growth(0, 50 - k);
      launch_scal<T>(d_.p, static_cast<T>(std::exp(Ld)), m_, s);
      launch_scal<T>(e_.p, static_cast<T>(std::exp(Le)), n_, s);
    }
  } else {
    launch_stream<T, false, true, true, kFull, Tag>(planA_, a, OnesOp<T>{}, s);
    ctx_.tmark("  eq: first pass");
    finish_cols(SkColOp<T>{static_cast<T>(mg), ce, e_.p, n_}, nullptr, 0, 0, gridACC);
    ctx_.tmark("  eq: first cols");
    for (; k < 50; ++k) {
      a.xin = e_.p;
      if (k < 49) {
        launch_stream<T, true, true, true, kFull, Tag>(planA_, a, SkRowOp<T>{static_cast<T>(nn), cd, d_.p}, s);
        finish_cols(SkColOp<T>{static_cast<T>(mg), ce, e_.p, n_, mark, k + 1.0, sk_tol, static_cast<T>(r_ref)},
                    ctx_.S.p + kSkRatio, 0, 0, gridBOTH);
        if (sk_uniform(k, n_)) { extrapolate = true; ++k; break; }
      } else {
        launch_stream<T, true, false, true, kFull, Tag>(planA_, a, SkRowOp<T>{static_cast<T>(nn), cd, d_.p}, s);
      }
    }
    ctx_.stats.matvecs_init += k + 1;
    if (extrapolate) {
      const double Le = sk_log_growth(1, 49 - k);
      const double Ld = -sk_log_growth(0, 50 - k);
      launch_scal<T>(d_.p, static_cast<T>(std::exp(Ld)), m_, s);
      launch_scal<T>(e_.p, static_cast<T>(std::exp(Le)), n_, s);
    }
  }
  ctx_.tmark("  eq: sk loop");
  launch_sqrt_inplace<T>(d_.p, m_, s);
  launch_sqrt_inplace<T>(e_.p, n_, s);
  const int sgrid = std::min(srows_, ctx_.num_cu * 8);
  const T *src = A_src_ ? A_src_ : A_.p;
  const T *dr = tmode_ ? e_.p : d_.p, *dc = tmode_ ? d_.p : e_.p;
  hipLaunchKernelGGL((scale_de_kernel<T, false>), dim3(sgrid), dim3(256), 0, s, src, static_cast<T *>(nullptr), lda_,
                     srows_, scols_pad_, dr, dc, static_cast<T>(1), ctx_.spart.p, ctx_.spart.p + sgrid);
  sum_row_scalars(sgrid, 1, ctx_.S.p + kFro2);
  launch_max_partials(ctx_.spart.p + sgrid, sgrid, ctx_.S.p + kAmax, s);
  if (multi_) ctx_.dist.allreduce(ctx_.S.p + kFro2, 1, s);
  const double *S = ctx_.fetch_scalars();
  const T normA = static_cast<T>(std::sqrt(S[kFro2])) /
                  std::sqrt(static_cast<T>(std::min<double>(mg, nn)));
  amax_ = S[kAmax] / static_cast<double>(normA);
  hipLaunchKernelGGL((scale_de_kernel<T, true>), dim3(sgrid), dim3(256), 0, s, src, A_.p, lda_, srows_, scols_pad_,
                     dr, dc, static_cast<T>(1) / normA, static_cast<double *>(nullptr),
                     static_cast<double *>(nullptr));
  A_src_ = nullptr;
  const T invs = static_cast<T>(1) / std::sqrt(normA);
  launch_scal<T>(d_.p, invs, m_, s);
  launch_scal<T>(e_.p, invs, n_, s);
  ctx_.stats.equil_ms = pt.stop_ms();
}

template <typename T, typename Tag>
void DenseSolver<T, Tag>::norm_est() {
  hipStream_t s = ctx_.stream;
  PhaseTimer pt(s);
  std::vector<T> x0(n_pad_, 0);
  rand_uniform_host(x0.data(), n_);
  POGS_HIP_CHECK(hipMemcpyAsync(xtemp_.p, x0.data(), n_pad_ * sizeof(T), hipMemcpyHostToDevice, s));
  ctx_.sync();
  T *xa = xtemp_.p, *xb = rhs_.p;
  const T kTol = static_cast<T>(1e-4);
  T norm_est = 0, last;
  const int grid = stream_grid<true, true>(planA_, srows_);
  unsigned i = 0;
  for (i = 0; tmode_ && i < 50; ++i) {
    last = norm_est;
    t_mul_n(xa, nullptr, StoreNormRowOp<T>{ytemp_.p}, ctx_.S.p + kPowSx2, (i == 0) ? nullptr : ctx_.S.p + kPowX2);
    t_mul_t(ytemp_.p, PowerColOp<T>{xb, n_}, ctx_.S.p + kPowX2);
    const double *S = ctx_.fetch_scalars();
    norm_est = static_cast<T>(std::sqrt(S[kPowX2])) / static_cast<T>(std::sqrt(S[kPowSx2]));
    std::swap(xa, xb);
    ctx_.stats.matvecs_init += 2;
    if (std::abs(last - norm_est) < kTol * norm_est) { ++i; break; }
  }
  for (; !tmode_ && i < 50; ++i) {
    last = norm_est;
    StreamArgs<T> a = argsA();
    a.xin = xa;
    a.xin_nrm2 = (i == 0) ? nullptr : ctx_.S.p + kPowX2;
    launch_stream<T, true, true, false, kFull, Tag>(planA_, a, PowerRowOp<T>{}, s);
    sum_row_scalars(grid, 1, ctx_.S.p + kPowSx2);
    finish_cols(PowerColOp<T>{xb, n_}, ctx_.S.p + kPowX2, kPowSx2, 1, grid);
    const double *S = ctx_.fetch_scalars();
    const T normx = static_cast<T>(std::sqrt(S[kPowX2]));
    const T normSx = static_cast<T>(std::sqrt(S[kPowSx2]));
    norm_est = normx / normSx;
    std::swap(xa, xb);
    ctx_.stats.matvecs_init += 1;
    if (std::abs(last - norm_est) < kTol * norm_est) { ++i; break; }
  }
  nrmA_ = norm_est;
  ctx_.stats.nrmA = nrmA_;
  ctx_.stats.norm_est_iters = i;
  xtemp_.zero(s);
  rhs_.zero(s);
  ytemp_.zero(s);
  ctx_.stats.normest_ms = pt.stop_ms();
}

template <typename T, typename Tag>
void DenseSolver<T, Tag>::norm_est_gram(T *G, size_t ld) {
  hipStream_t s = ctx_.stream;
  PhaseTimer pt(s);
  launch_zero_upper<T>(G, ld, n_, s);
  ctx_.tmark("  ne: zero_upper");
  std::vector<T> x0(n_pad_, 0);
  rand_uniform_host(x0.data(), n_);
  ctx_.tmark("  ne: rand host");
  POGS_HIP_CHECK(hipMemcpyAsync(xtemp_.p, x0.data(), n_pad_ * sizeof(T), hipMemcpyHostToDevice, s));
  ctx_.sync();
  ctx_.tmark("  ne: h2d");
  T *xa = xtemp_.p, *xb = rhs_.p;
  const T kTol = static_cast<T>(1e-4);
  T norm_est = 0, last;
  const int grid = stream_grid<true, true>(planW_, n_);
  double *sp = ctx_.spart.p + static_cast<size_t>(planA_.grid_max) * 6;
  unsigned i = 0;
  for (i = 0; i < 50; ++i) {
    last = norm_est;
    const double *nrm = (i == 0) ? nullptr : ctx_.S.p + kPowX2;
    StreamArgs<T> a;
    a.A = G; a.lda = ld; a.m = n_; a.n_pad = n_pad_;
    a.xin = xa; a.xin_add = nullptr; a.xin_nrm2 = nrm;
    a.col_partials = colpart_.p; a.scalar_partials = ctx_.spart.p;
    a.xl_scratch = xl_buf_.p;
    launch_stream<T, true, true, false, kLower, Tag>(planW_, a, SymRowOp<T>{G, ld, xa, nrm, tvec_.p}, s);
    launch_reduce_cols<T, SymColOp<T>>(colpart_.p, grid, n_pad_, SymColOp<T>{tvec_.p, xa, nrm, xb, n_}, sp, s);
    SumJob j{sp, reduce_cols_grid(n_pad_, Vec16<T>::N), 2, ctx_.S.p + kPowX2};
    launch_sum_jobs(&j, 1, s);
    const double *S = ctx_.fetch_scalars();
    const T normx = static_cast<T>(std::sqrt(S[kPowX2]));
    const T normSx = static_cast<T>(std::sqrt(S[kPowXGx]));
    norm_est = normx / normSx;
    std::swap(xa, xb);
    if (std::abs(last - norm_est) < kTol * norm_est) { ++i; break; }
  }
  nrmA_ = norm_est;
  ctx_.stats.nrmA = nrmA_;
  ctx_.stats.norm_est_iters = i;
  xtemp_.zero(s);
  rhs_.zero(s);
  tvec_.zero(s);
  ctx_.stats.normest_ms = pt.stop_ms();
}

template <typename T, typename Tag>
void DenseSolver<T, Tag>::norm_est_gram_wide(T *G, size_t ld) {
  hipStream_t s = ctx_.stream;
  PhaseTimer pt(s);
  launch_zero_upper<T>(G, ld, k_, s);
  std::vector<T> x0(n_pad_, 0);
  rand_uniform_host(x0.data(), n_);
  POGS_HIP_CHECK(hipMemcpyAsync(xtemp_.p, x0.data(), n_pad_ * sizeof(T), hipMemcpyHostToDevice, s));
  ctx_.sync();
  T *ya = ytemp_.p, *yb = uvec_.p;
  t_mul_n(xtemp_.p, nullptr, StoreNormRowOp<T>{ya}, ctx_.S.p + kPowSx2);
  ctx_.stats.matvecs_init += 1;
  const T kTol = static_cast<T>(1e-4);
  T norm_est = 0, last;
  const int grid = stream_grid<true, true>(planW_, k_);
  double *sp = ctx_.spart.p + static_cast<size_t>(planA_.grid_max) * 6;
  double y2 = ctx_.fetch_scalars()[kPowSx2];
  unsigned i = 0;
  for (i = 0; i < 50; ++i) {
    last = norm_est;
    const double *nrm = (i == 0) ? nullptr : ctx_.S.p + kPowXGx;
    StreamArgs<T> a;
    a.A = G; a.lda = ld; a.m = k_; a.n_pad = k_pad_;
    a.xin = ya; a.xin_add = nullptr; a.xin_nrm2 = nrm;
    a.col_partials = colpart_.p; a.scalar_partials = ctx_.spart.p;
    a.xl_scratch = xl_buf_.p;
    launch_stream<T, true, true, false, kLower, Tag>(planW_, a, SymRowOp<T>{G, ld, ya, nrm, tvec_.p}, s);
    launch_reduce_cols<T, SymColOp<T>>(colpart_.p, grid, k_pad_, SymColOp<T>{tvec_.p, ya, nrm, yb, k_}, sp, s);
    double *tmp2 = ctx_.S.p + kPowX2;
    const double prev_xgx = (i == 0) ? 1.0 : ctx_.S_host.p[kPowXGx];
    const double prev_w2 = (i == 0) ? y2 : ctx_.S_host.p[kPowX2];
    SumJob j{sp, reduce_cols_grid(k_pad_, Vec16<T>::N), 2, tmp2};
    launch_sum_jobs(&j, 1, s);
    const double *S = ctx_.fetch_scalars();
    y2 = prev_w2 / prev_xgx;
    norm_est = static_cast<T>(std::sqrt(S[kPowXGx])) / static_cast<T>(std::sqrt(y2));
    std::swap(ya, yb);
    if (std::abs(last - norm_est) < kTol * norm_est) { ++i; break; }
  }
  nrmA_ = norm_est;
  ctx_.stats.nrmA = nrmA_;
  ctx_.stats.norm_est_iters = i;
  xtemp_.zero(s);
  ytemp_.zero(s);
  uvec_.zero(s);
  tvec_.zero(s);
  ctx_.stats.normest_ms = pt.stop_ms();
}
```

pogs_amd/csrc/dense_solver.h:

```cpp
#pragma once
#include <algorithm>
#include <array>
#include <cmath>
#include <cstdint>
#include <cstdio>
#include <cstdlib>
#include <limits>
#include <thread>

#include "batch_admm.h"
#include "batch_kernels.h"
#include "cg_kernels.h"
#include "engine.h"
#include "fused_cols.h"
#include "gemm.h"
#include "gram_phase.h"
#include "ops.h"
#include "reduce.h"
#include "stream.h"
#include "vec_kernels.h"

namespace pogs_amd {

void rand_uniform_host(float *x, size_t n);
void rand_uniform_host(double *x, size_t n);

namespace {

template <typename T, bool WRITE>
__global__ void __launch_bounds__(256) scale_de_kernel(const T *src, T *dst, size_t lda, int m, int n_pad, const T *d,
                                                       const T *e, T post, double *partials, double *max_partials) {
  using V = typename Vec16<T>::type;
  constexpr int VEC = Vec16<T>::N;
  __shared__ double s_red[4];
  __shared__ double s_max[4];
  const int vpr = n_pad / VEC;
  double acc[1] = {0.0};
  T amax = 0;
  for (int row = blockIdx.x; row < m; row += gridDim.x) {
    const T di = d[row];
    const T *rp = src + static_cast<size_t>(row) * lda;
    for (int v = threadIdx.x; v < vpr; v += 256) {
      V a = WRITE ? stream_load<V>(rp + v * VEC) : *reinterpret_cast<const V *>(rp + v * VEC);
      const V ev = *reinterpret_cast<const V *>(e + v * VEC);
      T *ap = reinterpret_cast<T *>(&a);
      const T *ep = reinterpret_cast<const T *>(&ev);
#pragma unroll
      for (int c = 0; c < VEC; ++c) {
        const T val = ap[c] * (di * ep[c]);
        if (WRITE) {
          ap[c] = val * post;
        } else {
          dev::prod_acc(acc[0], val, val);
          amax = fmax(amax, fabs(val));
        }
      }
      if (WRITE) *reinterpret_cast<V *>(dst + static_cast<size_t>(row) * lda + v * VEC) = a;
    }
  }
  if (WRITE) return;
  dev::block_sum<1, 256>(acc, s_red);
  double mx = static_cast<double>(amax);
  for (int off = 32; off > 0; off >>= 1) mx = fmax(mx, __shfl_xor(mx, off, 64));
  if ((threadIdx.x & 63) == 0) s_max[threadIdx.x >> 6] = mx;
  __syncthreads();
  if (threadIdx.x == 0) {
    partials[blockIdx.x] = acc[0];
    max_partials[blockIdx.x] = fmax(fmax(s_max[0], s_max[1]), fmax(s_max[2], s_max[3]));
  }
}

template <typename T, typename Tag = AllPlans>
class DenseSolver final : public SolverBase {
 public:
  ~DenseSolver() override { begin_destroy(ctx_); }
  DenseSolver(int ord, size_t m, size_t n, const void *A, int mem, const PogsAmdOptions *opt,
              const PogsAmdDist *dist) {
    const double t0 = wall_s();
    struct Joiner {
      std::thread t;
      ~Joiner() { if (t.joinable()) t.join(); }
    } preload;
    {
      int dev = opt ? opt->device : -1;
      if (dev < 0 && hipGetDevice(&dev) != hipSuccess) dev = -1;
      static std::atomic<bool> preloaded{false};
      if (dev >= 0 && !preloaded.exchange(true))
        preload.t = std::thread([dev] {
          hipFuncAttributes fa;
          if (hipSetDevice(dev) != hipSuccess) return;
          (void)hipFuncGetAttributes(&fa, reinterpret_cast<const void *>(scale_de_kernel<T, true>));
          preload_vec_code();
          preload_gemm_code();
        });
    }
    ctx_.init(opt ? opt->device : -1, opt ? opt->profile : 0);
    m_ = static_cast<int>(m);
    n_ = static_cast<int>(n);
    POGS_CHECK(m > 0 && n > 0 && m < (1u << 31) && n < (1u << 31), "bad dimensions");
    if (dist && dist->world >= 1) {
      ctx_.dist.init(dist->rank, dist->world, dist->unique_id);
      ctx_.m_global = dist->m_global;
    } else {
      ctx_.m_global = m;
    }
    multi_ = ctx_.dist.active();
    tall_ = ctx_.m_global > n;
    POGS_CHECK(tall_ || !multi_, "row sharding needs m > n (SURVEY.md section 8(e))");
    use_cgls_ = opt && opt->projector == POGS_AMD_PROJ_CGLS;
    if (const char *ys = std::getenv("POGS_AMD_YSYNC")) ysync_ = std::max(0, std::atoi(ys));
    POGS_CHECK(!(use_cgls_ && multi_), "the CGLS projector is single-GPU");
    constexpr int VEC = Vec16<T>::N;
    n_pad_ = static_cast<int>(round_up(n, VEC));
    m_pad_ = static_cast<int>(round_up(m, VEC));
    k_ = tall_ ? n_ : m_;
    k_pad_ = static_cast<int>(round_up(k_, VEC));
    tmode_ = !tall_ && !use_cgls_;
    srows_ = tmode_ ? n_ : m_;
    scols_pad_ = tmode_ ? m_pad_ : n_pad_;
    lda_ = scols_pad_;
    planA_ = make_stream_plan<T>(scols_pad_, ctx_.num_cu);
    POGS_CHECK(planA_.ok, tmode_ || tall_ ? "min(m, n) too large for the register-tiled streaming kernel"
                                          : "n too large for the register-tiled streaming kernel (CGLS projector)");
    POGS_CHECK(planA_.xl ? Tag::windows : Tag::has(planA_.tpb, planA_.nv),
               "dense solver built for another streaming shape (abi.hip: make_dense_solver)");
    ctx_.tmark_last = t0;
    ctx_.tmark("ctx init");
    upload(ord, A, mem);
    if (mem != POGS_AMD_DEVICE) ctx_.sync();
    ctx_.stats.t_h2d_s = wall_s() - t0;
    ctx_.tmark("upload");
    alloc_state();
    ctx_.tmark("alloc_state");
    equilibrate();
    ctx_.tmark("equilibrate");
    if (use_cgls_) norm_est();
    if (!use_cgls_) factor();
    ctx_.sync();
    ctx_.stats.t_init_s = wall_s() - t0;
  }

  int dtype() const override { return sizeof(T) == 4 ? POGS_AMD_F32 : POGS_AMD_F64; }
  int device() const override { return ctx_.device; }
  void on_entry() override { ctx_.on_entry(); }
  void on_error() override { ctx_.on_error(); }
  PogsAmdStats &stats() override { return ctx_.stats; }

  int solve(const FnHost &f, const FnHost &g, const SolveParams &p, void *x, void *y, void *l, void *mu,
            double *optval, unsigned *final_iter) override {
    const double t0 = wall_s();
    load_problem(f, g, p);
    cold_start();
    apply_warm_start();
    ctx_.sync();
    const double t1 = wall_s();
    if (ctx_.dist.rank() == 0) print_banner(p.verbose);
    while (!iteration(p.verbose)) {}
    ctx_.sync();
    const double t2 = wall_s();
    const int status = epilogue(x, y, l, mu, optval);
    *final_iter = ctl_.k;
    PogsAmdStats &st = ctx_.stats;
    st.t_loop_s = t2 - t1;
    st.t_total_s = st.t_init_s + (wall_s() - t0);
    st.iterations = ctl_.k + 1;
    st.exact_iters = ctl_.exact_iters;
    st.rho_updates = ctl_.rho_updates;
    st.rho_final = ctl_.rho;
    collect_stream_timer();
    if (p.verbose > 0 && ctx_.dist.rank() == 0) {
      print_summary(status, st.t_total_s, st.t_init_s, ctl_);
      if (p.verbose > 3) print_timing_breakdown(st.t_loop_s, st.iterations);
      std::printf("POGS-AMD dense/%s: status %d, iter %u, init %.3e s, loop %.3e s\n", use_cgls_ ? "cgls" : "direct",
                  status, ctl_.k, st.t_init_s, st.t_loop_s);
    }
    return status;
  }

  void begin_run(const FnHost &f, const FnHost &g, const SolveParams &p) override {
    load_problem(f, g, p);
    cold_start();
    apply_warm_start();
    ctx_.sync();
  }

  void solve_batch(int k, const FnHost *f, const FnHost *g, const double *rho, const SolveParams &p,
                   const BatchOut &out) override;

  void set_warm_start(const void *x0, const void *l0) override {
    warm_x_.assign(static_cast<const T *>(x0), static_cast<const T *>(x0) + n_);
    warm_l_.assign(static_cast<const T *>(l0), static_cast<const T *>(l0) + m_);
    warm_pending_ = true;
  }

  void iterate(unsigned iters, double *seconds, unsigned *solves) override {
    POGS_CHECK(loaded_, "PogsAmdIterate before PogsAmdBeginRun / PogsAmdSolve: no problem is loaded");
    unsigned done = 0;
    ctx_.sync();
    const double t0 = wall_s();
    for (unsigned i = 0; i < iters; ++i) {
      if (ctl_.finished) {
        cold_start();
        ++done;
      }
      iteration(0);
    }
    ctx_.sync();
    const double t1 = wall_s();
    if (seconds) *seconds = t1 - t0;
    if (solves) *solves = done;
    ctx_.stats.t_loop_s += t1 - t0;
    ctx_.stats.iterations += iters;
    collect_stream_timer();
  }

  void get_equil(void *A_eq, void *d, void *e, double *nrmA) override {
    ctx_.sync();
    if (A_eq && tmode_) {
      DevBuf<T> rm(static_cast<size_t>(m_) * n_);
      launch_transpose<T>(A_.p, lda_, n_, m_, rm.p, n_, ctx_.stream);
      ctx_.sync();
      POGS_HIP_CHECK(hipMemcpy(A_eq, rm.p, static_cast<size_t>(m_) * n_ * sizeof(T), hipMemcpyDeviceToHost));
    } else if (A_eq) {
      POGS_HIP_CHECK(hipMemcpy2D(A_eq, n_ * sizeof(T), A_.p, lda_ * sizeof(T), n_ * sizeof(T), m_,
                                 hipMemcpyDeviceToHost));
    }
    if (d) POGS_HIP_CHECK(hipMemcpy(d, d_.p, m_ * sizeof(T), hipMemcpyDeviceToHost));
    if (e) POGS_HIP_CHECK(hipMemcpy(e, e_.p, n_ * sizeof(T), hipMemcpyDeviceToHost));
    if (nrmA) *nrmA = nrmA_;
  }

  void get_factor(void *W, void *U) override {
    POGS_CHECK(!use_cgls_ && Wp_ && Up_, "no factor: the handle runs the CGLS projector");
    ctx_.sync();
    const size_t row = static_cast<size_t>(k_) * sizeof(T), pitch = static_cast<size_t>(k_pad_) * sizeof(T);
    if (W) POGS_HIP_CHECK(hipMemcpy2D(W, row, Wp_, pitch, row, k_, hipMemcpyDeviceToHost));
    if (U) POGS_HIP_CHECK(hipMemcpy2D(U, row, Up_, pitch, row, k_, hipMemcpyDeviceToHost));
  }

  void project(const void *x0, const void *y0, double tol, void *x, void *y) override {
    hipStream_t s = ctx_.stream;
    POGS_HIP_CHECK(hipMemcpyAsync(xtemp_.p, x0, n_ * sizeof(T), hipMemcpyHostToDevice, s));
    POGS_HIP_CHECK(hipMemcpyAsync(ytemp_.p, y0, m_ * sizeof(T), hipMemcpyHostToDevice, s));
    if (use_cgls_) {
      x_[0].zero(s);
      cgls_project(xtemp_.p, ytemp_.p, x_[0].p, static_cast<T>(tol), nullptr);
      StreamArgs<T> a = argsA();
      a.xin = x_[0].p;
      launch_stream<T, true, false, false, kFull, Tag>(planA_, a, GemvNOp<T>{1, 0, y_[0].p}, s);
    } else if (tall_) {
      gemv_t_partials(ytemp_.p);
      finish_cols(StoreColOp<T>{1, 0, rhs_.p, n_}, nullptr, 0, 0);
      solve_gram(rhs_.p, xtemp_.p, GemvNOp<T>{1, 0, x_[0].p}, nullptr);
      StreamArgs<T> a = argsA();
      a.xin = x_[0].p;
      launch_stream<T, true, false, false, kFull, Tag>(planA_, a, GemvNOp<T>{1, 0, y_[0].p}, s);
    } else {
      t_mul_n(xtemp_.p, nullptr, ResidOp<T>{ytemp_.p, rhs_.p}, nullptr);
      solve_gram(rhs_.p, static_cast<const T *>(nullptr), GemvNOp<T>{1, 0, tmpn_.p}, nullptr);
      launch_axpby<T>(m_, static_cast<T>(1), ytemp_.p, static_cast<T>(0), y_[0].p, s);
      launch_axpby<T>(m_, static_cast<T>(1), tmpn_.p, static_cast<T>(1), y_[0].p, s);
      launch_axpby<T>(n_, static_cast<T>(1), xtemp_.p, static_cast<T>(0), x_[0].p, s);
      t_mul_t(tmpn_.p, StoreColOp<T>{static_cast<T>(-1), static_cast<T>(1), x_[0].p, n_}, nullptr);
    }
    POGS_HIP_CHECK(hipMemcpyAsync(x, x_[0].p, n_ * sizeof(T), hipMemcpyDeviceToHost, s));
    POGS_HIP_CHECK(hipMemcpyAsync(y, y_[0].p, m_ * sizeof(T), hipMemcpyDeviceToHost, s));
    ctx_.sync();
  }

  void mul(char trans, double alpha, const void *x, double beta, void *y) override {
    hipStream_t s = ctx_.stream;
    const bool tr = (trans == 't' || trans == 'T');
    if (tmode_) {
      if (!tr) {
        POGS_HIP_CHECK(hipMemcpyAsync(xtemp_.p, x, n_ * sizeof(T), hipMemcpyHostToDevice, s));
        POGS_HIP_CHECK(hipMemcpyAsync(ytemp_.p, y, m_ * sizeof(T), hipMemcpyHostToDevice, s));
        t_mul_n(xtemp_.p, nullptr, GemvNOp<T>{static_cast<T>(alpha), static_cast<T>(beta), ytemp_.p}, nullptr);
        POGS_HIP_CHECK(hipMemcpyAsync(y, ytemp_.p, m_ * sizeof(T), hipMemcpyDeviceToHost, s));
      } else {
        POGS_HIP_CHECK(hipMemcpyAsync(ytemp_.p, x, m_ * sizeof(T), hipMemcpyHostToDevice, s));
        POGS_HIP_CHECK(hipMemcpyAsync(xtemp_.p, y, n_ * sizeof(T), hipMemcpyHostToDevice, s));
        t_mul_t(ytemp_.p, StoreColOp<T>{static_cast<T>(alpha), static_cast<T>(beta), xtemp_.p, n_}, nullptr);
        POGS_HIP_CHECK(hipMemcpyAsync(y, xtemp_.p, n_ * sizeof(T), hipMemcpyDeviceToHost, s));
      }
      ctx_.sync();
      return;
    }
    if (!tr) {
      POGS_HIP_CHECK(hipMemcpyAsync(xtemp_.p, x, n_ * sizeof(T), hipMemcpyHostToDevice, s));
      POGS_HIP_CHECK(hipMemcpyAsync(ytemp_.p, y, m_ * sizeof(T), hipMemcpyHostToDevice, s));
      StreamArgs<T> a = argsA();
      a.xin = xtemp_.p;
      launch_stream<T, true, false, false, kFull, Tag>(planA_, a,
                                                  GemvNOp<T>{static_cast<T>(alpha), static_cast<T>(beta), ytemp_.p}, s);
      POGS_HIP_CHECK(hipMemcpyAsync(y, ytemp_.p, m_ * sizeof(T), hipMemcpyDeviceToHost, s));
    } else {
      POGS_HIP_CHECK(hipMemcpyAsync(ytemp_.p, x, m_ * sizeof(T), hipMemcpyHostToDevice, s));
      POGS_HIP_CHECK(hipMemcpyAsync(xtemp_.p, y, n_ * sizeof(T), hipMemcpyHostToDevice, s));
      gemv_t_partials(ytemp_.p);
      if (multi_) {
        finish_cols(StoreColOp<T>{1, 0, rhs_.p, n_}, nullptr, 0, 0);
        launch_axpby<T>(n_, static_cast<T>(alpha), rhs_.p, static_cast<T>(beta), xtemp_.p, s);
      } else {
        finish_cols(StoreColOp<T>{static_cast<T>(alpha), static_cast<T>(beta), xtemp_.p, n_}, nullptr, 0, 0);
      }
      POGS_HIP_CHECK(hipMemcpyAsync(y, xtemp_.p, n_ * sizeof(T), hipMemcpyDeviceToHost, s));
    }
    ctx_.sync();
  }

 private:
  void upload(int ord, const void *A, int mem);

  void alloc_state();

  StreamArgs<T> argsA() const {
    StreamArgs<T> a;
    a.A = A_.p; a.lda = lda_; a.m = srows_; a.n_pad = scols_pad_;
    a.xin = nullptr; a.xin_add = nullptr; a.xin_nrm2 = nullptr;
    a.col_partials = colpart_.p; a.scalar_partials = ctx_.spart.p;
    a.xl_scratch = xl_buf_.p;
    return a;
  }
  void ensure_xl(const StreamPlan &p, int rows, int n_pad) {
    const size_t need = stream_xl_scratch<T>(p, rows, n_pad);
    if (need > xl_buf_.n) {
      ctx_.sync();
      xl_buf_.alloc(need);
    }
  }

  template <typename RowOp>
  void t_mul_n(const T *xin, const T *xin_add, const RowOp &op, double *scalar_out, const double *x_nrm2 = nullptr) {
    hipStream_t s = ctx_.stream;
    if (!tmode_) {
      StreamArgs<T> a = argsA();
      a.xin = xin; a.xin_add = xin_add; a.xin_nrm2 = x_nrm2;
      ctx_.stream_timer.begin(s);
      launch_stream<T, true, false, false, kFull, Tag>(planA_, a, op, s);
      ctx_.stream_timer.end(s);
      if (RowOp::NS > 0 && scalar_out) sum_row_scalars(stream_grid<true, false>(planA_, srows_), RowOp::NS, scalar_out);
      return;
    }
    StreamArgs<T> a = argsA();
    ctx_.stream_timer.begin(s);
    launch_stream<T, false, true, false, kFull, Tag>(planA_, a, VecCoefOp<T>{xin, xin_add, x_nrm2}, s);
    ctx_.stream_timer.end(s);
    double *sp = ctx_.spart.p + static_cast<size_t>(planA_.grid_max) * 6;
    launch_reduce_cols<T, RowAsColOp<T, RowOp>>(colpart_.p, stream_grid<false, true>(planA_, srows_), scols_pad_,
                                                RowAsColOp<T, RowOp>{op, m_}, sp, s);
    if (RowOp::NS > 0 && scalar_out) {
      SumJob j{sp, reduce_cols_grid(scols_pad_, Vec16<T>::N), RowOp::NS, scalar_out};
      launch_sum_jobs(&j, 1, s);
    }
  }
  template <typename ColOp>
  void t_mul_t(const T *u, const ColOp &op, double *scalar_out) {
    hipStream_t s = ctx_.stream;
    if (!tmode_) {
      gemv_t_partials(u);
      finish_cols(op, scalar_out, 0, 0);
      return;
    }
    StreamArgs<T> a = argsA();
    a.xin = u;
    ctx_.stream_timer.begin(s);
    launch_stream<T, true, false, false, kFull, Tag>(planA_, a, ColAsRowOp<T, ColOp>{op}, s);
    ctx_.stream_timer.end(s);
    if (ColOp::NS > 0 && scalar_out) sum_row_scalars(stream_grid<true, false>(planA_, srows_), ColOp::NS, scalar_out);
  }

  template <typename ColOp>
  void finish_cols(const ColOp &op, double *colop_scalar_out, int yslot, int yslot_count,
                   int nparts_override = -1, const T *partials_src = nullptr) {
    hipStream_t s = ctx_.stream;
    const T *colpart = partials_src ? partials_src : colpart_.p;
    const int nparts = nparts_override > 0 ? nparts_override : stream_grid<false, true>(planA_, m_);
    double *sp = ctx_.spart.p + static_cast<size_t>(planA_.grid_max) * 6;
    if (!multi_) {
      launch_reduce_cols<T, ColOp>(colpart, nparts, n_pad_, op, sp, s);
    } else {
      launch_reduce_cols<T, StoreColOp<T>>(colpart, nparts, n_pad_, StoreColOp<T>{1, 0, tmpn_.p, n_}, sp, s);
      if (yslot_count > 0) ctx_.dist.allreduce2<T>(tmpn_.p, n_pad_, ctx_.S.p + yslot, yslot_count, s);
      else ctx_.dist.allreduce(tmpn_.p, n_pad_, s);
      launch_reduce_cols<T, ColOp>(tmpn_.p, 1, n_pad_, op, sp, s);
    }
    if (ColOp::NS > 0 && colop_scalar_out) {
      SumJob j{sp, reduce_cols_grid(n_pad_, Vec16<T>::N), ColOp::NS, colop_scalar_out};
      sum_now_or_later(j);
    }
  }

  void sum_now_or_later(const SumJob &j) {
    if (defer_sums_) ctx_.queue_sum(j);
    else launch_sum_jobs(&j, 1, ctx_.stream);
  }

  void gemv_t_partials(const T *u) {
    StreamArgs<T> a = argsA();
    ctx_.stream_timer.begin(ctx_.stream);
    launch_stream<T, false, true, false, kFull, Tag>(planA_, a, GemvTOp<T>{1, u}, ctx_.stream);
    ctx_.stream_timer.end(ctx_.stream);
  }

  void sum_row_scalars(int grid, int ns, double *out) {
    SumJob j{ctx_.spart.p, grid, ns, out};
    launch_sum_jobs(&j, 1, ctx_.stream);
  }

  void equilibrate();

  void norm_est();

  void norm_est_gram(T *G, size_t ld);

  void norm_est_gram_wide(T *G, size_t ld);

  void factor();

  template <typename TailOp>
  void solve_gram(const T *rhs, const T *add, const TailOp &tail, double *tail_scalars);

  template <typename TailColOp>
  void solve_gram_onepass(const T *rhs, const T *add, const TailColOp &tail, double *tail_scalars);

  int cgls_project(const T *x0, const T *y0, T *x, T tol, const T *Ax_warm, T *yacc = nullptr);

  void load_problem(const FnHost &f, const FnHost &g, const SolveParams &p);
  FnView<T> fview() const { return FnView<T>{f_.h.p, fs_.a.p, f_.b.p, fs_.c.p, fs_.d.p, fs_.e.p}; }
  FnView<T> gview() const { return FnView<T>{g_.h.p, gs_.a.p, g_.b.p, gs_.c.p, gs_.d.p, gs_.e.p}; }

  void cold_start();

  void apply_warm_start();

  bool iteration(unsigned verbose);

  bool iteration_fused(unsigned verbose);

  bool iteration_fused_wide(unsigned verbose);

  double eval_objective();
  void log_iteration(unsigned verbose);

  int epilogue(void *x, void *y, void *l, void *mu, double *optval);

  void collect_stream_timer();

  Ctx ctx_;
  int m_ = 0, n_ = 0, n_pad_ = 0, k_ = 0, k_pad_ = 0;
  bool tall_ = true, multi_ = false, use_cgls_ = false;
  double amax_ = 0;
  bool defer_sums_ = false;
  size_t sp_pre_off_ = 0, sp_tail_off_ = 0;
  double spec_gap_[3] = {0, 0, 0};
  bool tmode_ = false;
  int m_pad_ = 0, srows_ = 0, scols_pad_ = 0;
  DevBuf<T> xl_buf_;
  DevBuf<T> uvec_;
  DevBuf<T> x12s_, xtemps_;
  DevBuf<T> cg_p_, cg_s_, cg_q_, cg_r_;
  DevBuf<double> cg_;
  size_t lda_ = 0;
  StreamPlan planA_, planW_;
  const T *A_src_ = nullptr;
  bool pre_cheap_ = false;
  T *Wp_ = nullptr, *Up_ = nullptr;
  DevBuf<T> A_, fac_, d_, e_, colpart_, colpart2_, y12s_, ytemps_;
  DevBuf<double> pack_;
  bool fused_ok_ = false, fused_now_ = false, fused_logistic_ = false, spec_valid_ = false;
  bool exact_mode_ = false;
  int colparts_ = 0;
  bool warm_pending_ = false;
  std::vector<T> warm_x_, warm_l_;
  T rho_pred_ = 1, zs_pred_ = 1;
  int ysync_ = 16;
  unsigned long long proj_count_ = 0;
  DevBuf<T> x_[2], y_[2], xt_, yt_, xtemp_, ytemp_, x12_, y12_, rhs_, tvec_, tmpn_;
  DevBuf<T> xout_, yout_, lout_, muout_;
  FnBuf<T> f_, g_, fs_, gs_;
  AdmmControl<T> ctl_;
  bool loaded_ = false;
  int cur_ = 0;
  T zt_scale_ = 1;
  T nrmA_ = 0;
};

#include "dense_setup.h"
#include "dense_factor.h"
#include "dense_iter.h"
#include "dense_wide.h"
#include "dense_batch.h"

}

template <typename T, typename Tag>
SolverBase *make_dense_solver_t(int ord, size_t m, size_t n, const void *A, int mem, const PogsAmdOptions *opt,
                                const PogsAmdDist *dist) {
  return new DenseSolver<T, Tag>(ord, m, n, A, mem, opt, dist);
}

}
```

pogs_amd/csrc/engine.h:

```cpp
#pragma once
#include <hip/hip_runtime.h>

#include <algorithm>
#include <chrono>
#include <cmath>
#include <cstdio>
#include <cstdlib>
#include <limits>
#include <cstring>
#include <memory>
#include <mutex>
#include <string>
#include <vector>

#include "../../include/pogs_amd.h"
#include "common.h"
#include "dist.h"
#include "vec_kernels.h"

namespace pogs_amd {

inline double wall_s() {
  return std::chrono::duration<double>(std::chrono::steady_clock::now().time_since_epoch()).count();
}

class DeviceGuard {
 public:
  explicit DeviceGuard(int dev) {
    if (dev < 0) return;
    if (hipGetDevice(&prev_) != hipSuccess) { prev_ = -1; }
    if (prev_ != dev) {
      POGS_HIP_CHECK(hipSetDevice(dev));
      restore_ = prev_ >= 0;
    }
  }
  ~DeviceGuard() {
    if (restore_) (void)hipSetDevice(prev_);
  }
  DeviceGuard(const DeviceGuard &) = delete;
  DeviceGuard &operator=(const DeviceGuard &) = delete;
 private:
  int prev_ = -1;
  bool restore_ = false;
};

class EventTimer {
 public:
  void enable(bool on) { on_ = on; }
  bool enabled() const { return on_; }
  void set_every(unsigned k) { every_ = k ? k : 1; }
  static constexpr size_t npos = static_cast<size_t>(-1);
  size_t begin(hipStream_t s) {
    active_ = on_ && (calls_++ % every_) == 0;
    if (!active_) return npos;
    if (used_ == ev_.size()) {
      hipEvent_t a, b;
      POGS_HIP_CHECK(hipEventCreate(&a));
      POGS_HIP_CHECK(hipEventCreate(&b));
      ev_.push_back({a, b});
      dropped_.push_back(0);
    }
    dropped_[used_] = 0;
    POGS_HIP_CHECK(hipEventRecord(ev_[used_].first, s));
    return used_;
  }
  void drop(size_t idx) {
    if (on_ && idx < dropped_.size()) dropped_[idx] = 1;
  }
  void end(hipStream_t s) {
    if (!active_) return;
    POGS_HIP_CHECK(hipEventRecord(ev_[used_].second, s));
    ++used_;
    active_ = false;
  }
  double collect_ms(unsigned long long *count) {
    double tot = 0;
    size_t kept = 0;
    for (size_t i = 0; i < used_; ++i) {
      if (dropped_[i]) continue;
      float ms = 0;
      if (hipEventElapsedTime(&ms, ev_[i].first, ev_[i].second) == hipSuccess) tot += ms;
      ++kept;
    }
    if (count) *count += kept;
    used_ = 0;
    return tot;
  }
  ~EventTimer() {
    for (auto &p : ev_) { (void)hipEventDestroy(p.first); (void)hipEventDestroy(p.second); }
  }
 private:
  bool on_ = false, active_ = false;
  unsigned every_ = 1;
  unsigned long long calls_ = 0;
  size_t used_ = 0;
  std::vector<std::pair<hipEvent_t, hipEvent_t>> ev_;
  std::vector<char> dropped_;
};

struct PhaseTimer {
  hipEvent_t a = nullptr, b = nullptr;
  hipStream_t s;
  explicit PhaseTimer(hipStream_t st) : s(st) {
    POGS_HIP_CHECK(hipEventCreate(&a));
    POGS_HIP_CHECK(hipEventCreate(&b));
    POGS_HIP_CHECK(hipEventRecord(a, s));
  }
  double stop_ms() {
    POGS_HIP_CHECK(hipEventRecord(b, s));
    POGS_HIP_CHECK(hipEventSynchronize(b));
    float ms = 0;
    POGS_HIP_CHECK(hipEventElapsedTime(&ms, a, b));
    return ms;
  }
  ~PhaseTimer() {
    if (a) (void)hipEventDestroy(a);
    if (b) (void)hipEventDestroy(b);
  }
};

struct CtxResources {
  hipStream_t stream = nullptr;
  double *host = nullptr;
  int device = -1;
};
inline std::mutex &ctx_pool_mutex() { static std::mutex *m = new std::mutex; return *m; }
inline std::vector<CtxResources> &ctx_pool() { static auto *v = new std::vector<CtxResources>; return *v; }
struct Ctx {
  int device = 0;
  int num_cu = 256;
  hipStream_t stream = nullptr;
  DistComm dist;
  size_t m_global = 0;
  DevBuf<double> S;
  struct HostMirror { double *p = nullptr; } S_host;
  DevBuf<double> spart;
  size_t spart_cap = 0;
  EventTimer stream_timer;
  PogsAmdStats stats;

  void init(int dev, int profile) {
    if (dev >= 0) POGS_HIP_CHECK(hipSetDevice(dev));
    POGS_HIP_CHECK(hipGetDevice(&device));
    hipDeviceProp_t prop;
    POGS_HIP_CHECK(hipGetDeviceProperties(&prop, device));
    num_cu = prop.multiProcessorCount > 0 ? prop.multiProcessorCount : 256;
    {
      std::lock_guard<std::mutex> lock(ctx_pool_mutex());
      auto &pool = ctx_pool();
      for (size_t i = 0; i < pool.size(); ++i)
        if (pool[i].device == device) {
          stream = pool[i].stream;
          S_host.p = pool[i].host;
          pool.erase(pool.begin() + static_cast<long>(i));
          break;
        }
    }
    if (!stream) {
      POGS_HIP_CHECK(hipStreamCreateWithFlags(&stream, hipStreamNonBlocking));
      POGS_HIP_CHECK(hipHostMalloc(reinterpret_cast<void **>(&S_host.p), (kNumSlots + 1) * sizeof(double),
                                   hipHostMallocMapped | hipHostMallocCoherent));
    }
    S.alloc(kNumSlots);
    S.zero(stream);
    pub_counter.alloc(1);
    pub_counter.zero(stream);
    std::memset(S_host.p, 0, (kNumSlots + 1) * sizeof(double));
    {
      void *dp = nullptr;
      poll_fetch = true;
      if (hipHostGetDevicePointer(&dp, S_host.p, 0) == hipSuccess && dp) S_host_dev = static_cast<double *>(dp);
      else poll_fetch = false;
    }
    std::memset(&stats, 0, sizeof(stats));
    stream_timer.enable(profile != 0);
    stream_timer.set_every(profile > 1 ? static_cast<unsigned>(profile) : 1u);
  }
  void ensure_spart(size_t count) {
    if (count > spart_cap) {
      POGS_HIP_CHECK(hipStreamSynchronize(stream));
      spart.alloc(count);
      spart_cap = count;
    }
  }
  void queue_sum(const SumJob &j) {
    if (npending == kMaxSumJobs) flush_sums();
    pending[npending++] = j;
  }
  void flush_sums() {
    if (npending) launch_sum_jobs(pending, npending, stream);
    npending = 0;
  }
  void set_overlay(const ScalarOverlay &ov) { overlay = ov; }
  const double *wait_publish(unsigned long long want) {
    unsigned long long *seqp = reinterpret_cast<unsigned long long *>(S_host.p + kNumSlots);
    unsigned spins = 0, idle_seen = 0, checks = 0;
    double t_wait0 = 0;
    while (__atomic_load_n(seqp, __ATOMIC_ACQUIRE) != want) {
      if (++spins == (1u << 14)) {
        spins = 0;
        if (dist.active() && (++checks & 255u) == 0) {
          const double now = wall_s();
          if (t_wait0 == 0) t_wait0 = now;
          const char *ae = dist.async_error();
          if (ae[0] || now - t_wait0 > coll_timeout_s()) {
            const std::string why = ae[0] ? std::string("RCCL reported: ") + ae
                                          : "no progress for " + std::to_string(static_cast<int>(coll_timeout_s())) +
                                                " s inside a collective (a peer rank did not join it)";
            dist.abort();
            poisoned = true;
            throw Error("row-sharded solve aborted: " + why);
          }
        }
        const hipError_t q = hipStreamQuery(stream);
        if (q == hipSuccess) {
          if (__atomic_load_n(seqp, __ATOMIC_ACQUIRE) == want) break;
          if (++idle_seen >= 3) {
            POGS_HIP_CHECK(hipMemcpy(S_host.p, S.p, kNumSlots * sizeof(double), hipMemcpyDeviceToHost));
            poll_fetch = false;
            return S_host.p;
          }
        } else if (q != hipErrorNotReady) {
          POGS_HIP_CHECK(q);
        }
      }
#if defined(__x86_64__)
      __builtin_ia32_pause();
#endif
    }
    return S_host.p;
  }
  const double *fetch_scalars() {
    const ScalarOverlay ov = overlay;
    overlay = ScalarOverlay();
    if (!poll_fetch) {
      flush_sums();
      launch_apply_overlay(S.p, ov, stream);
      POGS_HIP_CHECK(hipMemcpyAsync(S_host.p, S.p, kNumSlots * sizeof(double), hipMemcpyDeviceToHost, stream));
      POGS_HIP_CHECK(hipStreamSynchronize(stream));
      return S_host.p;
    }
    const unsigned long long want = ++fetch_seq;
    if (npending) {
      launch_sum_publish(pending, npending, S.p, kNumSlots, S_host_dev,
                         reinterpret_cast<unsigned long long *>(S_host_dev + kNumSlots), want, pub_counter.p, stream, ov);
      npending = 0;
    } else {
      launch_publish_scalars(S.p, kNumSlots, S_host_dev, reinterpret_cast<unsigned long long *>(S_host_dev + kNumSlots),
                             want, stream, ov);
    }
    return wait_publish(want);
  }
  static double coll_timeout_s() {
    static const double v = [] {
      const char *e = std::getenv("POGS_AMD_COLL_TIMEOUT_S");
      const double t = e ? std::atof(e) : 300.0;
      return t > 0 ? t : 300.0;
    }();
    return v;
  }
  bool poll_fetch = true;
  ScalarOverlay overlay;
  SumJob pending[kMaxSumJobs];
  int npending = 0;
  DevBuf<unsigned> pub_counter;
  unsigned long long fetch_seq = 0;
  double *S_host_dev = nullptr;
  void sync() {
    flush_sums();
    POGS_HIP_CHECK(hipStreamSynchronize(stream));
  }
  void tmark(const char *label) {
    static const bool on = std::getenv("POGS_AMD_TRACE") != nullptr;
    if (!on) return;
    const double t1 = wall_s();
    POGS_HIP_CHECK(hipStreamSynchronize(stream));
    const double t2 = wall_s();
    const PoolCounters pc = DevicePool::get().counters(device);
    std::fprintf(stderr, "[pogs_amd trace] %-28s host +%8.3f ms, drain +%8.3f ms | pool: +%llu malloc %.3f ms, +%llu reuse, "
                 "+%llu free %.3f ms\n", label, (t1 - tmark_last) * 1e3, (t2 - t1) * 1e3,
                 pc.mallocs - tmark_pool.mallocs, pc.malloc_ms - tmark_pool.malloc_ms, pc.reuses - tmark_pool.reuses,
                 pc.frees - tmark_pool.frees, pc.free_ms - tmark_pool.free_ms);
    tmark_pool = pc;
    tmark_last = wall_s();
  }
  double tmark_last = 0;
  PoolCounters tmark_pool;
  bool poisoned = false;
  unsigned long long coll_mark = 0;
  void on_entry() { coll_mark = dist.collectives(); }
  void on_error() {
    if (dist.active() && dist.collectives() != coll_mark) {
      dist.abort();
      poisoned = true;
    }
  }
  ~Ctx() {
    if (!stream) return;
    DeviceGuard guard(device);
    const bool healthy = !poisoned && hipStreamSynchronize(stream) == hipSuccess;
    if (healthy) {
      std::lock_guard<std::mutex> lock(ctx_pool_mutex());
      CtxResources r;
      r.stream = stream;
      r.host = S_host.p;
      r.device = device;
      ctx_pool().push_back(r);
    } else {
      (void)hipStreamDestroy(stream);
      if (S_host.p) (void)hipHostFree(S_host.p);
    }
  }
};

#define POGS_HD __host__ __device__
#if defined(__HIP_DEVICE_COMPILE__)
#define POGS_SAY_RHO(fmt, ...) ((void)0)
#else
#define POGS_SAY_RHO(fmt, ...) do { if (say_rho) std::printf(fmt, __VA_ARGS__); } while (0)
#endif
POGS_HD inline float ctl_abs(float v) { return fabsf(v); }
POGS_HD inline double ctl_abs(double v) { return fabs(v); }
POGS_HD inline float ctl_sqrt(float v) { return sqrtf(v); }
POGS_HD inline double ctl_sqrt(double v) { return sqrt(v); }
POGS_HD inline float ctl_pow(float a, float b) { return powf(a, b); }
POGS_HD inline double ctl_pow(double a, double b) { return pow(a, b); }
template <typename T> POGS_HD inline T ctl_min(T a, T b) { return b < a ? b : a; }
template <typename T> POGS_HD inline T ctl_max(T a, T b) { return a < b ? b : a; }

template <typename T>
struct AdmmControl {
  T abs_tol = 0, rel_tol = 0;
  unsigned max_iter = 0;
  bool adaptive_rho = true, gap_stop = false;
  T rho0 = 1;
  size_t m_glob = 0, n = 0;
  T rho = 1, delta = 0, xi = 1;
  unsigned k = 0, kd = 0, ku = 0;
  T prev_nrm_r = 0;
  T nrm_r = 0, nrm_s = 0, gap = 0, eps_gap = 0, eps_pri = 0, eps_dua = 0;
  bool converged = false, finished = false;
  unsigned exact_iters = 0, rho_updates = 0;
  bool say_rho = false;
  T sqrtn_atol = 0, sqrtm_atol = 0, sqrtmn_atol = 0;

  static constexpr double kAlphaD = 1.7;
  POGS_HD T alpha() const { return static_cast<T>(kAlphaD); }

  void reset() {
    rho = rho0;
    delta = static_cast<T>(1.05);
    xi = 1;
    k = kd = ku = 0;
    prev_nrm_r = std::numeric_limits<T>::max();
    converged = finished = false;
    exact_iters = rho_updates = 0;
    sqrtn_atol = std::sqrt(static_cast<T>(n)) * abs_tol;
    sqrtm_atol = std::sqrt(static_cast<T>(m_glob)) * abs_tol;
    sqrtmn_atol = std::sqrt(static_cast<T>(m_glob + n)) * abs_tol;
  }

  POGS_HD void set_pre(const double *S) {
    gap = ctl_abs(static_cast<T>(S[kGapX] + S[kGapY]));
    const T nz = static_cast<T>(ctl_sqrt(S[kWX2] + S[kWY2]));
    const T nz12 = static_cast<T>(ctl_sqrt(S[kHX2] + S[kHY2]));
    const T ny12 = static_cast<T>(ctl_sqrt(S[kHY2]));
    const T nx = static_cast<T>(ctl_sqrt(S[kWX2]));
    eps_gap = sqrtmn_atol + rel_tol * nz * nz12;
    eps_pri = sqrtm_atol + rel_tol * ny12;
    eps_dua = rho * (sqrtn_atol + rel_tol * nx);
  }
  POGS_HD T proj_tol() const {
    T tol = static_cast<T>(1e-2) * ctl_pow(ctl_min(prev_nrm_r, static_cast<T>(1)), static_cast<T>(0.5));
    return ctl_max(tol, static_cast<T>(1e-8));
  }
  POGS_HD bool set_approx(const double *S, T nrmA) {
    nrm_s = rho * (nrmA * static_cast<T>(ctl_sqrt(S[kDYprev2])) + static_cast<T>(ctl_sqrt(S[kDXprev2])));
    nrm_r = nrmA * static_cast<T>(ctl_sqrt(S[kDX12])) + static_cast<T>(ctl_sqrt(S[kDY12]));
    return nrm_r < 10 * eps_pri && nrm_s < 10 * eps_dua;
  }
  POGS_HD void set_exact(const double *S) {
    nrm_r = static_cast<T>(ctl_sqrt(S[kExactR2]));
    nrm_s = rho * static_cast<T>(ctl_sqrt(S[kExactS2]));
    ++exact_iters;
  }
  POGS_HD bool check_stop(bool exact) {
    converged = exact && nrm_r < eps_pri && nrm_s < eps_dua && (!gap_stop || gap < eps_gap);
    if (converged || k == max_iter - 1) {
      finished = true;
      return true;
    }
    return false;
  }
  POGS_HD T adapt() {
    T scale = 1;
    const T kDeltaMin = static_cast<T>(1.05), kGamma = static_cast<T>(1.01), kTau = static_cast<T>(0.8);
    const T kRhoMin = static_cast<T>(1e-4), kRhoMax = static_cast<T>(1e4), kKappa = static_cast<T>(0.9);
    const T kOne = 1, kZero = 0;
    if (adaptive_rho) {
      const unsigned kRhoUpdateFreq = 50u;
      const T kRhoChangeMax = static_cast<T>(1.5), kRhoChangeMin = static_cast<T>(0.67);
      const T kImbalanceThresh = static_cast<T>(10);
      if (k > 0 && k % kRhoUpdateFreq == 0 && eps_pri > kZero && eps_dua > kZero) {
        const T pri_n = nrm_r / eps_pri, dua_n = nrm_s / eps_dua;
        if (pri_n > kZero && dua_n > kZero) {
          const T imbalance = pri_n / dua_n;
          if (imbalance > kImbalanceThresh || imbalance < kOne / kImbalanceThresh) {
            T ratio = ctl_sqrt(imbalance);
            ratio = ctl_max(kRhoChangeMin, ctl_min(kRhoChangeMax, ratio));
            T rho_new = rho * ratio;
            rho_new = ctl_max(kRhoMin, ctl_min(kRhoMax, rho_new));
            if (ctl_abs(rho_new - rho) / rho > static_cast<T>(0.05)) {
              scale = rho / rho_new;
              rho = rho_new;
              ++rho_updates;
              POGS_SAY_RHO("spectral rho update: %e (imbalance=%.1f)\n", (double)rho, (double)imbalance);
            }
          }
        }
      } else if (nrm_s < xi * eps_dua && nrm_r > xi * eps_pri && kTau * static_cast<T>(k) > static_cast<T>(kd)) {
        if (rho < kRhoMax) {
          rho *= delta;
          scale = 1 / delta;
          delta = kGamma * delta;
          ku = k;
          ++rho_updates;
          POGS_SAY_RHO("+ rho %e\n", (double)rho);
        }
      } else if (nrm_s > xi * eps_dua && nrm_r < xi * eps_pri && kTau * static_cast<T>(k) > static_cast<T>(ku)) {
        if (rho > kRhoMin) {
          rho /= delta;
          scale = delta;
          delta = kGamma * delta;
          kd = k;
          ++rho_updates;
          POGS_SAY_RHO("- rho %e\n", (double)rho);
        }
      } else if (nrm_s < xi * eps_dua && nrm_r < xi * eps_pri) {
        xi *= kKappa;
      } else {
        delta = kDeltaMin;
      }
    }
    prev_nrm_r = nrm_r;
    return scale;
  }
  POGS_HD void predict(T *rho_out, T *scale_out) const {
    AdmmControl<T> c = *this;
    c.say_rho = false;
    *scale_out = c.adapt();
    *rho_out = c.rho;
  }
  POGS_HD int status() const {
    if (!converged && k == max_iter - 1) return POGS_MAX_ITER;
    if (!converged) return POGS_NAN_FOUND;
    return POGS_SUCCESS;
  }
};

#define POGS_AMD_HBAR "----------------------------------------------------------------------------\n"
inline const char *status_string(int st) {
  switch (st) {
    case POGS_SUCCESS: return "Solved";
    case POGS_UNBOUNDED: return "Unbounded";
    case POGS_INFEASIBLE: return "Infeasible";
    case POGS_MAX_ITER: return "Reached max iter";
    case POGS_NAN_FOUND: return "Encountered NaN";
    case POGS_INVALID_CONE: return "Invalid cone found";
    default: return "Error";
  }
}
inline void print_banner(unsigned verbose) {
  if (verbose > 0)
    std::printf(POGS_AMD_HBAR
                "           POGS v0.4.0 - Proximal Graph Solver (MI355X / HIP engine)\n"
                "           graph-form ADMM of foges/pogs, rebuilt for gfx950\n");
  if (verbose > 1)
    std::printf(POGS_AMD_HBAR " Iter | pri res | pri tol | dua res | dua tol |   gap   | eps gap |"
                " pri obj\n" POGS_AMD_HBAR);
}
template <typename T>
inline bool wants_iter_line(unsigned verbose, const AdmmControl<T> &c) {
  return (verbose > 2 && c.k % 10 == 0) || (verbose > 1 && c.k % 100 == 0) || (verbose > 1 && c.converged);
}
template <typename T>
inline void print_iter_line(const AdmmControl<T> &c, double optval) {
  std::printf("%5d : %.2e  %.2e  %.2e  %.2e  %.2e  %.2e % .2e\n", static_cast<int>(c.k), (double)c.nrm_r,
              (double)c.eps_pri, (double)c.nrm_s, (double)c.eps_dua, (double)c.gap, (double)c.eps_gap, optval);
}
template <typename T>
inline void print_summary(int status, double t_total, double t_init, const AdmmControl<T> &c) {
  std::printf(POGS_AMD_HBAR
              "Status: %s\n"
              "Timing: Total = %3.2e s, Init = %3.2e s\n"
              "Iter  : %u\n",
              status_string(status), t_total, t_init, c.k);
  std::printf(POGS_AMD_HBAR
              "Error Metrics:\n"
              "Pri: "
              "|Ax - y|    / (abs_tol sqrt(m)     / rel_tol + |y|)          = %.2e\n"
              "Dua: "
              "|A'l + u|   / (abs_tol sqrt(n)     / rel_tol + |u|)          = %.2e\n"
              "Gap: "
              "|x'u + y'l| / (abs_tol sqrt(m + n) / rel_tol + |x,u| |y,l|)  = %.2e\n" POGS_AMD_HBAR,
              (double)(c.rel_tol * c.nrm_r / c.eps_pri), (double)(c.rel_tol * c.nrm_s / c.eps_dua),
              (double)(c.rel_tol * c.gap / c.eps_gap));
  std::fflush(stdout);
}

inline void print_timing_breakdown(double loop_s, unsigned iterations) {
  std::printf("Timing breakdown (per-iter avg): prox = %3.2e s, proj = %3.2e s, residual = %3.2e s\n", 0.0,
              loop_s / std::max(1u, iterations), 0.0);
  std::fflush(stdout);
}

struct SolveParams {
  double rho, abs_tol, rel_tol;
  unsigned max_iter, verbose;
  bool adaptive_rho, gap_stop;
};

template <typename T>
inline AdmmControl<T> make_admm_control(const SolveParams &p, double rho0, size_t m_glob, size_t n) {
  AdmmControl<T> c;
  c.abs_tol = static_cast<T>(p.abs_tol);
  c.rel_tol = static_cast<T>(p.rel_tol);
  c.max_iter = p.max_iter;
  c.adaptive_rho = p.adaptive_rho;
  c.gap_stop = p.gap_stop;
  c.rho0 = static_cast<T>(rho0);
  c.m_glob = m_glob;
  c.n = n;
  c.reset();
  return c;
}

struct FnHost {
  const void *a, *b, *c, *d, *e;
  const int *h;
  double s0[5] = {1.0, 0.0, 1.0, 0.0, 0.0};
  int h0 = 15;
  int hval(size_t i) const { return h ? h[i] : h0; }
};

template <typename Pred>
inline bool all_h(const FnHost &f, size_t count, Pred pred) {
  if (!f.h) return count == 0 || pred(f.h0);
  for (size_t i = 0; i < count; ++i)
    if (!pred(f.h[i])) return false;
  return true;
}

template <typename T>
inline void upload_fn(FnBuf<T> &dst, const FnHost &src, int cnt, hipStream_t s) {
  if (cnt <= 0) return;
  if (src.h) POGS_HIP_CHECK(hipMemcpyAsync(dst.h.p, src.h, cnt * sizeof(int), hipMemcpyHostToDevice, s));
  else launch_fill_int(dst.h.p, src.h0, static_cast<size_t>(cnt), s);
  const void *ptr[5] = {src.a, src.b, src.c, src.d, src.e};
  T *out[5] = {dst.a.p, dst.b.p, dst.c.p, dst.d.p, dst.e.p};
  for (int k = 0; k < 5; ++k) {
    if (ptr[k]) POGS_HIP_CHECK(hipMemcpyAsync(out[k], ptr[k], cnt * sizeof(T), hipMemcpyHostToDevice, s));
    else launch_fill<T>(out[k], static_cast<T>(src.s0[k]), static_cast<size_t>(cnt), s);
  }
}

template <typename T>
inline unsigned warn_negative_coeffs(const FnHost &f, size_t count) {
  constexpr unsigned kMaxWarn = 8;
  const T *c = static_cast<const T *>(f.c), *e = static_cast<const T *>(f.e);
  unsigned nc = 0, ne = 0;
  if (!c && count && f.s0[2] < 0.0) nc = static_cast<unsigned>(std::min<size_t>(count, 0xFFFFFFFFu));
  if (!e && count && f.s0[4] < 0.0) ne = static_cast<unsigned>(std::min<size_t>(count, 0xFFFFFFFFu));
  for (unsigned w = 0; w < std::min(nc, kMaxWarn); ++w) std::printf("WARNING c < 0. Function not convex. Using c = 0");
  for (unsigned w = 0; w < std::min(ne, kMaxWarn); ++w) std::printf("WARNING e < 0. Function not convex. Using e = 0");
  for (size_t i = 0; i < count && (c || e); ++i) {
    if (c && c[i] < static_cast<T>(0) && nc++ < kMaxWarn) std::printf("WARNING c < 0. Function not convex. Using c = 0");
    if (e && e[i] < static_cast<T>(0) && ne++ < kMaxWarn) std::printf("WARNING e < 0. Function not convex. Using e = 0");
  }
  if (nc > kMaxWarn) std::printf("\nWARNING c < 0 in %u more function objects", nc - kMaxWarn);
  if (ne > kMaxWarn) std::printf("\nWARNING e < 0 in %u more function objects", ne - kMaxWarn);
  if (nc + ne) {
    std::printf("\n");
    std::fflush(stdout);
  }
  return nc + ne;
}

struct BatchOut {
  void *x, *y, *l, *mu;
  double *optval;
  unsigned *final_iter;
  int *status;
};

struct SolverBase {
  virtual ~SolverBase() {}
  virtual int dtype() const = 0;
  virtual int device() const = 0;
  virtual int solve(const FnHost &f, const FnHost &g, const SolveParams &p, void *x, void *y, void *l,
                    void *mu, double *optval, unsigned *final_iter) = 0;
  virtual void begin_run(const FnHost &f, const FnHost &g, const SolveParams &p) = 0;
  virtual void solve_batch(int, const FnHost *, const FnHost *, const double *, const SolveParams &, const BatchOut &) {
    throw Error("batched solves need a dense handle");
  }
  virtual void solve_batch_sparse(int, const FnHost *, const FnHost *, const double *, const SolveParams &,
                                  const BatchOut &) {
    throw Error("a batched sparse solve needs a sparse handle");
  }
  virtual void iterate(unsigned iters, double *seconds, unsigned *solves) = 0;
  virtual void set_warm_start(const void *x0, const void *l0) = 0;
  virtual void get_equil(void *A_eq, void *d, void *e, double *nrmA) = 0;
  virtual void get_factor(void *, void *) { throw Error("PogsAmdGetFactor needs a dense handle"); }
// ... 27 lines not shown
```

pogs_amd/csrc/vec_kernels.h:

```cpp
#pragma once
#include <hip/hip_runtime.h>

#include "common.h"
#include "prox.h"

namespace pogs_amd {

enum Slot : int {
  kGapY = 0, kWY2, kHY2, kDYprev2, kDY12, kExactR2, kPowSx2, kFro2, kFvalF, kCgQ2,
  kAmax = 10,
  kSkMark = 11,
  kGapX = 12, kWX2, kHX2, kDXprev2, kDX12, kExactS2, kPowX2, kPowXGx, kFvalG, kCgP2, kCgS2, kCgX2,
  kSpecGapY = 26, kSpecWY2, kSpecHY2,
  kSpecGapX = 29, kSpecWX2, kSpecHX2,
  kSkRatio = 32,
  kFcDone = 40,
  kFcSteps,
  kFcNorms0,
  kFcGamma0, kFcGamma1,
  kFcAlpha, kFcBeta, kFcDelta, kFcIndef,
  kNumSlots = 52
};

template <typename T>
struct FnBuf {
  DevBuf<int> h;
  DevBuf<T> a, b, c, d, e;
  void alloc(size_t n) { h.alloc(n); a.alloc(n); b.alloc(n); c.alloc(n); d.alloc(n); e.alloc(n); }
  FnView<T> view() const { return FnView<T>{h.p, a.p, b.p, c.p, d.p, e.p}; }
};

template <typename T>
struct FnUniform {
  int mask = 0;
  int h = 0;
  T c = 0, d = 0, e = 0;
};
template <typename T>
FnUniform<T> probe_uniform(FnView<T> fn, int n, hipStream_t s);

template <typename T>
struct AdmmPreArgs {
  int n_x, n_y;
  FnView<T> g, f;
  const T *x_cur, *y_cur;
  const T *xt, *yt;
  T zt_scale;
  T *x12, *y12;
  T *xtemp, *ytemp;
  T rho, alpha;
  double *partials;
  int blocks_x;
  T *x_aux = nullptr, *y_aux = nullptr;
  double *cg_reset = nullptr;
  bool cheap = false;
  FnUniform<T> ug, uf;
};

template <typename T>
void launch_scale_objective(FnView<T> fn, T *a, T *c, T *d, T *e, const T *scale, int n, bool divide,
                            hipStream_t s);

constexpr int kVecTpb = 256;
inline int vec_blocks(int n) { return (n + kVecTpb - 1) / kVecTpb; }
constexpr int kPreU = 4;
inline int pre_blocks(int n) { return (n + kVecTpb * kPreU - 1) / (kVecTpb * kPreU); }

template <typename T>
void launch_admm_pre(const AdmmPreArgs<T> &a, hipStream_t s);

template <typename T>
void launch_admm_tail(int n, const T *znew, const T *zprev, const T *z12, T *ztemp, double *partials,
                      hipStream_t s);

template <typename T>
void launch_func_eval(int n, FnView<T> f, const T *v, double *partials, hipStream_t s);

template <typename T>
void launch_prox_eval(int n, FnView<T> f, T rho, const T *in, T *out, hipStream_t s);

template <typename T>
void launch_proj_subgrad(int n, FnView<T> f, const T *x, const T *v, T *out, hipStream_t s);

template <typename T>
struct UnscaleArgs {
  int n_x, n_y;
  const T *x12, *y12, *xt, *yt, *xprev, *yprev, *d, *e;
  T zt_scale, rho;
  T *x_out, *y_out, *l_out, *mu_out;
};
template <typename T>
void launch_unscale(const UnscaleArgs<T> &a, hipStream_t s);

struct SumJob {
  const double *partials;
  int nparts, ns;
  double *out;
  int stride = 0;
  int offset = 0;
};
struct ScalarOverlay {
  const double *src = nullptr;
  int slot[2] = {0, 0};
  int n[2] = {0, 0};
};
void preload_vec_code();
constexpr int kMaxSumJobs = 8;
void launch_sum_publish(const SumJob *jobs, int njobs, double *S, int count, double *host_S,
                        unsigned long long *host_seq, unsigned long long seq, unsigned *counter, hipStream_t s,
                        const ScalarOverlay &ov = ScalarOverlay());
void launch_publish_scalars(double *S, int count, double *host_S, unsigned long long *host_seq,
                            unsigned long long seq, hipStream_t s, const ScalarOverlay &ov = ScalarOverlay());
void launch_apply_overlay(double *S, const ScalarOverlay &ov, hipStream_t s);

template <typename T>
void launch_exact_u(int m, const T *y12, const T *yt, const T *yprev, T c, T *u, hipStream_t s);

void launch_max_partials(const double *partials, int n, double *out, hipStream_t s);

void launch_sum_jobs(const SumJob *jobs, int njobs, hipStream_t s);

void launch_sum_cg(const SumJob &job, double *S, double *cg, int mode, double shift, double eps, hipStream_t s);

double measure_read_bandwidth_gbs(size_t bytes, int reps, int *pattern);

template <typename T> void wave_sum_check(const T *in_host, size_t n, T *alu_host, T *lds_host);

template <typename T> void launch_fill(T *p, T v, size_t n, hipStream_t s);
void launch_fill_int(int *p, int v, size_t n, hipStream_t s);
template <typename T> void launch_sqrt_inplace(T *p, size_t n, hipStream_t s);
template <typename T> void launch_scal(T *p, T alpha, size_t n, hipStream_t s);
template <typename T> void launch_scale_by(size_t n, T alpha, const T *in, const T *sc, bool divide, T *out, hipStream_t s);
template <typename T> void launch_axpby(size_t n, T a, const T *x, T b, T *y, hipStream_t s);

}
```

pogs_amd/csrc/vec_kernels.hip:

```cpp
#include "vec_kernels.h"

#include "reduce.h"
#include "stream.h"

namespace pogs_amd {

namespace {

template <typename T>
__global__ void __launch_bounds__(kVecTpb) scale_objective_kernel(FnView<T> fn, T *a, T *c, T *d, T *e,
                                                                  const T *scale, int n, bool divide) {
  const int i = blockIdx.x * kVecTpb + threadIdx.x;
  if (i >= n) return;
  const T s = scale[i];
  const T zero = 0;
  T ai = fn.a[i], ci = fn.c[i], di = fn.d[i], ei = fn.e[i];
  ci = ci < zero ? zero : ci;
  ei = ei < zero ? zero : ei;
  if (divide) {
    ai /= s; di /= s; ei /= s * s;
  } else {
    ai *= s; di *= s; ei *= s * s;
  }
  a[i] = ai; c[i] = ci; d[i] = di; e[i] = ei;
// ... 106 lines not shown
  if (is_x) {
    if (i < a.n_x) {
      const T ei = a.e[i];
      a.x_out[i] = a.x12[i] * ei;
      if (a.mu_out)
        a.mu_out[i] = -a.rho * (a.zt_scale * a.xt[i] - a.xprev[i] + a.x12[i]) / ei;
    }
  } else {
    if (i < a.n_y) {
      const T di = a.d[i];
      a.y_out[i] = a.y12[i] / di;
      a.l_out[i] = -a.rho * (a.zt_scale * a.yt[i] - a.yprev[i] + a.y12[i]) * di;
    }
  }
}

struct SumJobs {
  SumJob j[kMaxSumJobs];
};

__device__ __forceinline__ void run_sum_job(const SumJob &job, double (&s_w)[4]) {
  const int t = threadIdx.x, lane = t & 63, wave = t >> 6;
  const size_t stride = job.stride > 0 ? job.stride : job.ns;
  for (int k = 0; k < job.ns; ++k) {
    const double *p = job.partials + job.offset + k;
    double s0 = 0, s1 = 0, s2 = 0, s3 = 0;
    int b = t;
    for (; b + 768 < job.nparts; b += 1024) {
      s0 += p[static_cast<size_t>(b) * stride];
      s1 += p[static_cast<size_t>(b + 256) * stride];
      s2 += p[static_cast<size_t>(b + 512) * stride];
      s3 += p[static_cast<size_t>(b + 768) * stride];
    }
    for (; b < job.nparts; b += 256) s0 += p[static_cast<size_t>(b) * stride];
    double s = dev::wave_sum((s0 + s1) + (s2 + s3));
    if (lane == 0) s_w[wave] = s;
    __syncthreads();
    if (t == 0) job.out[k] = (s_w[0] + s_w[1]) + (s_w[2] + s_w[3]);
    __syncthreads();
  }
}

__global__ void __launch_bounds__(256) sum_jobs_kernel(SumJobs jobs) {
  __shared__ double s_w[4];
  run_sum_job(jobs.j[blockIdx.x], s_w);
}

__global__ void __launch_bounds__(256) sum_publish_kernel(SumJobs jobs, int njobs, double *S, int count,
                                                          double *host_S, unsigned long long *host_seq,
                                                          unsigned long long seq, unsigned *counter, ScalarOverlay ov) {
  __shared__ double s_w[4];
  __shared__ unsigned s_last;
  run_sum_job(jobs.j[blockIdx.x], s_w);
  if (threadIdx.x == 0) {
    __threadfence();
    s_last = __hip_atomic_fetch_add(counter, 1u, __ATOMIC_ACQ_REL, __HIP_MEMORY_SCOPE_AGENT) == static_cast<unsigned>(njobs - 1);
  }
  __syncthreads();
  if (!s_last) return;
  __threadfence();
  const int t = threadIdx.x;
  if (t == 0) __hip_atomic_store(counter, 0u, __ATOMIC_RELAXED, __HIP_MEMORY_SCOPE_AGENT);
  if (t < count) {
    double v = __hip_atomic_load(S + t, __ATOMIC_RELAXED, __HIP_MEMORY_SCOPE_AGENT);
    int base = 0;
#pragma unroll
    for (int q = 0; q < 2; ++q) {
      if (t >= ov.slot[q] && t < ov.slot[q] + ov.n[q]) {
        v = ov.src[base + t - ov.slot[q]];
        S[t] = v;
      }
      base += ov.n[q];
    }
    host_S[t] = v;
  }
  __threadfence_system();
  __syncthreads();
  if (t == 0) __hip_atomic_store(host_seq, seq, __ATOMIC_RELEASE, __HIP_MEMORY_SCOPE_SYSTEM);
}

template <typename T>
__global__ void fill_kernel(T *p, T v, size_t n) {
  const size_t i = static_cast<size_t>(blockIdx.x) * blockDim.x + threadIdx.x;
  if (i < n) p[i] = v;
}
template <typename T>
__global__ void sqrt_kernel(T *p, size_t n) {
  const size_t i = static_cast<size_t>(blockIdx.x) * blockDim.x + threadIdx.x;
  if (i < n) p[i] = dev::Sqrt(p[i]);
}
template <typename T>
__global__ void scal_kernel(T *p, T alpha, size_t n) {
  const size_t i = static_cast<size_t>(blockIdx.x) * blockDim.x + threadIdx.x;
  if (i < n) p[i] *= alpha;
}
template <typename T>
__global__ void axpby_kernel(size_t n, T a, const T *x, T b, T *y) {
  const size_t i = static_cast<size_t>(blockIdx.x) * blockDim.x + threadIdx.x;
  if (i < n) y[i] = (b == static_cast<T>(0)) ? a * x[i] : a * x[i] + b * y[i];
}
template <typename T>
__global__ void scale_by_kernel(size_t n, T alpha, const T *in, const T *sc, bool divide, T *out) {
  const size_t i = static_cast<size_t>(blockIdx.x) * blockDim.x + threadIdx.x;
  if (i < n) out[i] = divide ? alpha * in[i] / sc[i] : alpha * in[i] * sc[i];
}

inline dim3 grid1d(size_t n, int tpb = 256) { return dim3(static_cast<unsigned>((n + tpb - 1) / tpb)); }

}

template <typename T>
void launch_scale_objective(FnView<T> fn, T *a, T *c, T *d, T *e, const T *scale, int n, bool divide,
                            hipStream_t s) {
  if (n <= 0) return;
  hipLaunchKernelGGL(scale_objective_kernel<T>, dim3(vec_blocks(n)), dim3(kVecTpb), 0, s, fn, a, c, d, e,
                     scale, n, divide);
}

namespace {
template <typename T>
struct UniformProbeOut {
  int differs;
  int h0;
  T c0, d0, e0;
};
template <typename T>
__global__ void __launch_bounds__(256) uniform_probe_kernel(FnView<T> fn, int n, UniformProbeOut<T> *out) {
  const int h0 = fn.h[0];
  const T c0 = fn.c[0], d0 = fn.d[0], e0 = fn.e[0];
  int bad = 0;
  for (int i = blockIdx.x * 256 + threadIdx.x; i < n; i += gridDim.x * 256) {
    bad |= (fn.h[i] != h0) ? 1 : 0;
    bad |= (fn.c[i] != c0) ? 2 : 0;
    bad |= (fn.d[i] != d0) ? 4 : 0;
    bad |= (fn.e[i] != e0) ? 8 : 0;
  }
  if (bad) atomicOr(&out->differs, bad);
  if (blockIdx.x == 0 && threadIdx.x == 0) { out->h0 = h0; out->c0 = c0; out->d0 = d0; out->e0 = e0; }
}
}
template <typename T>
FnUniform<T> probe_uniform(FnView<T> fn, int n, hipStream_t s) {
  FnUniform<T> u;
  if (n <= 0) return u;
  DevBuf<UniformProbeOut<T>> out(1);
  out.zero(s);
  hipLaunchKernelGGL(uniform_probe_kernel<T>, dim3(std::max(1, std::min((n + 255) / 256, 2048))), dim3(256), 0, s, fn, n, out.p);
  UniformProbeOut<T> h;
  POGS_HIP_CHECK(hipMemcpyAsync(&h, out.p, sizeof(h), hipMemcpyDeviceToHost, s));
  POGS_HIP_CHECK(hipStreamSynchronize(s));
  u.mask = ~h.differs & 15;
  u.h = h.h0; u.c = h.c0; u.d = h.d0; u.e = h.e0;
  return u;
}

template <typename T>
void launch_admm_pre(const AdmmPreArgs<T> &a, hipStream_t s) {
  const int blocks = a.blocks_x + pre_blocks(a.n_y);
  if (a.cheap) hipLaunchKernelGGL((admm_pre_kernel<T, true>), dim3(blocks), dim3(kVecTpb), 0, s, a);
  else hipLaunchKernelGGL((admm_pre_kernel<T, false>), dim3(blocks), dim3(kVecTpb), 0, s, a);
}

template <typename T>
void launch_admm_tail(int n, const T *znew, const T *zprev, const T *z12, T *ztemp, double *partials,
                      hipStream_t s) {
  hipLaunchKernelGGL(admm_tail_kernel<T>, dim3(vec_blocks(n)), dim3(kVecTpb), 0, s, n, znew, zprev, z12,
                     ztemp, partials);
}

template <typename T>
void launch_func_eval(int n, FnView<T> f, const T *v, double *partials, hipStream_t s) {
  hipLaunchKernelGGL(func_eval_kernel<T>, dim3(vec_blocks(n)), dim3(kVecTpb), 0, s, n, f, v, partials);
}

template <typename T>
void launch_prox_eval(int n, FnView<T> f, T rho, const T *in, T *out, hipStream_t s) {
  if (n <= 0) return;
  hipLaunchKernelGGL(prox_eval_kernel<T>, dim3(vec_blocks(n)), dim3(kVecTpb), 0, s, n, f, rho, in, out);
}

template <typename T>
void launch_proj_subgrad(int n, FnView<T> f, const T *x, const T *v, T *out, hipStream_t s) {
  if (n <= 0) return;
  hipLaunchKernelGGL(proj_subgrad_kernel<T>, dim3(vec_blocks(n)), dim3(kVecTpb), 0, s, n, f, x, v, out);
}

template <typename T>
void launch_unscale(const UnscaleArgs<T> &a, hipStream_t s) {
  const int bx = vec_blocks(a.n_x);
  hipLaunchKernelGGL(unscale_kernel<T>, dim3(bx + vec_blocks(a.n_y)), dim3(kVecTpb), 0, s, a, bx);
}

namespace {
__device__ __forceinline__ double overlay_value(double *S, int t, const ScalarOverlay &ov) {
  int base = 0;
#pragma unroll
  for (int q = 0; q < 2; ++q) {
    if (t >= ov.slot[q] && t < ov.slot[q] + ov.n[q]) {
      const double v = ov.src[base + t - ov.slot[q]];
      S[t] = v;
      return v;
    }
    base += ov.n[q];
  }
  return __hip_atomic_load(S + t, __ATOMIC_RELAXED, __HIP_MEMORY_SCOPE_AGENT);
}
__global__ void __launch_bounds__(64) publish_scalars_kernel(double *S, int count, double *host_S,
                                                           unsigned long long *host_seq, unsigned long long seq,
                                                           ScalarOverlay ov) {
  const int t = threadIdx.x;
  if (t < count) host_S[t] = overlay_value(S, t, ov);
  __threadfence_system();
  __syncthreads();
  if (t == 0) __hip_atomic_store(host_seq, seq, __ATOMIC_RELEASE, __HIP_MEMORY_SCOPE_SYSTEM);
}
__global__ void __launch_bounds__(64) apply_overlay_kernel(double *S, ScalarOverlay ov) {
  const int t = threadIdx.x;
  if (t < kNumSlots) (void)overlay_value(S, t, ov);
}
}

void launch_publish_scalars(double *S, int count, double *host_S, unsigned long long *host_seq,
                            unsigned long long seq, hipStream_t s, const ScalarOverlay &ov) {
  hipLaunchKernelGGL(publish_scalars_kernel, dim3(1), dim3(64), 0, s, S, count, host_S, host_seq, seq, ov);
}
void launch_apply_overlay(double *S, const ScalarOverlay &ov, hipStream_t s) {
  if (ov.n[0] + ov.n[1] > 0) hipLaunchKernelGGL(apply_overlay_kernel, dim3(1), dim3(64), 0, s, S, ov);
}

namespace {
__global__ void __launch_bounds__(256) max_partials_kernel(const double *partials, int n, double *out) {
  __shared__ double s_w[4];
  double v = 0.0;
  for (int b = threadIdx.x; b < n; b += 256) v = fmax(v, partials[b]);
  for (int off = 32; off > 0; off >>= 1) v = fmax(v, __shfl_xor(v, off, 64));
  if ((threadIdx.x & 63) == 0) s_w[threadIdx.x >> 6] = v;
  __syncthreads();
  if (threadIdx.x == 0) *out = fmax(fmax(s_w[0], s_w[1]), fmax(s_w[2], s_w[3]));
}
}

void preload_vec_code() {
  hipFuncAttributes fa;
  (void)hipFuncGetAttributes(&fa, reinterpret_cast<const void *>(max_partials_kernel));
}

void launch_max_partials(const double *partials, int n, double *out, hipStream_t s) {
  hipLaunchKernelGGL(max_partials_kernel, dim3(1), dim3(256), 0, s, partials, n, out);
}

namespace {
__global__ void __launch_bounds__(256) sum_cg_kernel(SumJob job, double *S, double *cg, int mode, double shift, double eps) {
  __shared__ double s_w[4];
  run_sum_job(job, s_w);
  if (threadIdx.x != 0) return;
  if (mode == 1) {
    double delta = S[kCgQ2] + shift * S[kCgP2];
    if (delta <= 0.0) cg[4] = 1.0;
    if (delta == 0.0) delta = eps;
    cg[3] = delta;
    cg[1] = cg[0] / delta;
  } else if (mode == 2) {
    const double g1 = cg[0], g = S[kCgS2];
    cg[0] = g;
    cg[2] = g / g1;
  } else if (mode == 3) {
    cg[0] = S[kCgS2];
    cg[4] = 0.0;
  }
}
}

void launch_sum_cg(const SumJob &job, double *S, double *cg, int mode, double shift, double eps, hipStream_t s) {
  hipLaunchKernelGGL(sum_cg_kernel, dim3(1), dim3(256), 0, s, job, S, cg, mode, shift, eps);
}

void launch_sum_jobs(const SumJob *jobs, int njobs, hipStream_t s) {
  POGS_CHECK(njobs >= 1 && njobs <= kMaxSumJobs, "sum jobs");
  SumJobs j;
  for (int i = 0; i < kMaxSumJobs; ++i) j.j[i] = jobs[i < njobs ? i : 0];
  hipLaunchKernelGGL(sum_jobs_kernel, dim3(njobs), dim3(256), 0, s, j);
}

void launch_sum_publish(const SumJob *jobs, int njobs, double *S, int count, double *host_S,
                        unsigned long long *host_seq, unsigned long long seq, unsigned *counter, hipStream_t s,
                        const ScalarOverlay &ov) {
  POGS_CHECK(njobs >= 1 && njobs <= kMaxSumJobs && count <= 256, "sum jobs");
  SumJobs j;
  for (int i = 0; i < kMaxSumJobs; ++i) j.j[i] = jobs[i < njobs ? i : 0];
  hipLaunchKernelGGL(sum_publish_kernel, dim3(njobs), dim3(256), 0, s, j, njobs, S, count, host_S, host_seq, seq,
                     counter, ov);
}

namespace {
template <typename T>
__global__ void exact_u_vec_kernel(int m, const T *y12, const T *yt, const T *yprev, T c, T *u) {
  const int i = blockIdx.x * blockDim.x + threadIdx.x;
  if (i < m) u[i] = y12[i] + c * yt[i] - yprev[i];
}
}
template <typename T>
void launch_exact_u(int m, const T *y12, const T *yt, const T *yprev, T c, T *u, hipStream_t s) {
  if (m) hipLaunchKernelGGL(exact_u_vec_kernel<T>, dim3((m + 255) / 256), dim3(256), 0, s, m, y12, yt, yprev, c, u);
}

template <typename T>
void launch_fill(T *p, T v, size_t n, hipStream_t s) {
  if (n) hipLaunchKernelGGL(fill_kernel<T>, grid1d(n), dim3(256), 0, s, p, v, n);
}
void launch_fill_int(int *p, int v, size_t n, hipStream_t s) {
  if (n) hipLaunchKernelGGL(fill_kernel<int>, grid1d(n), dim3(256), 0, s, p, v, n);
}
template <typename T>
void launch_sqrt_inplace(T *p, size_t n, hipStream_t s) {
  if (n) hipLaunchKernelGGL(sqrt_kernel<T>, grid1d(n), dim3(256), 0, s, p, n);
}
template <typename T>
void launch_scal(T *p, T alpha, size_t n, hipStream_t s) {
  if (n) hipLaunchKernelGGL(scal_kernel<T>, grid1d(n), dim3(256), 0, s, p, alpha, n);
}
template <typename T>
void launch_scale_by(size_t n, T alpha, const T *in, const T *sc, bool divide, T *out, hipStream_t s) {
  if (n) hipLaunchKernelGGL(scale_by_kernel<T>, grid1d(n), dim3(256), 0, s, n, alpha, in, sc, divide, out);
}
template <typename T>
void launch_axpby(size_t n, T a, const T *x, T b, T *y, hipStream_t s) {
  if (n) hipLaunchKernelGGL(axpby_kernel<T>, grid1d(n), dim3(256), 0, s, n, a, x, b, y);
}
namespace {
typedef float bw_v4 __attribute__((ext_vector_type(4)));
template <int U>
__global__ void __launch_bounds__(256) bw_stride_kernel(const bw_v4 *__restrict__ a, size_t nvec, float *out) {
  const size_t stride = static_cast<size_t>(gridDim.x) * blockDim.x;
  size_t i = static_cast<size_t>(blockIdx.x) * blockDim.x + threadIdx.x;
  bw_v4 acc = {0, 0, 0, 0};
  for (; i + (U - 1) * stride < nvec; i += U * stride) {
    bw_v4 v[U];
#pragma unroll
    for (int u = 0; u < U; ++u) v[u] = __builtin_nontemporal_load(a + i + u * stride);
#pragma unroll
    for (int u = 0; u < U; ++u) acc += v[u];
  }
  for (; i < nvec; i += stride) acc += __builtin_nontemporal_load(a + i);
  if (acc.x + acc.y + acc.z + acc.w == 123.456f) out[0] = acc.x;
}
template <int NV, int R>
__global__ void __launch_bounds__(256) bw_rows_kernel(const bw_v4 *__restrict__ a, int rows, int rowvec, float *out) {
  bw_v4 acc = {0, 0, 0, 0};
  for (int r0 = blockIdx.x * R; r0 < rows; r0 += gridDim.x * R) {
    bw_v4 v[R][NV];
#pragma unroll
    for (int r = 0; r < R; ++r)
#pragma unroll
      for (int k = 0; k < NV; ++k) {
        const int c = k * 256 + static_cast<int>(threadIdx.x);
        v[r][k] = __builtin_nontemporal_load(a + static_cast<size_t>(min(r0 + r, rows - 1)) * rowvec + min(c, rowvec - 1));
      }
#pragma unroll
    for (int r = 0; r < R; ++r)
#pragma unroll
      for (int k = 0; k < NV; ++k) acc += v[r][k];
  }
  if (acc.x + acc.y + acc.z + acc.w == 123.456f) out[0] = acc.x;
}
}

double measure_read_bandwidth_gbs(size_t bytes, int reps, int *pattern) {
  const int rowvec = 2500, rows = static_cast<int>(std::max<size_t>(1, bytes / (16 * static_cast<size_t>(rowvec))));
  const size_t nvec = static_cast<size_t>(rows) * rowvec;
  DevBuf<bw_v4> a(nvec);
  DevBuf<float> out(16);
  hipStream_t s = nullptr;
  a.zero(s);
  hipEvent_t e0, e1;
  POGS_HIP_CHECK(hipEventCreate(&e0));
  POGS_HIP_CHECK(hipEventCreate(&e1));
  double best = 0;
  reps = std::max(1, reps);
  for (int pat = 0; pat < 2; ++pat) {
    auto launch = [&]() {
      if (pat == 0) hipLaunchKernelGGL((bw_stride_kernel<4>), dim3(512), dim3(256), 0, s, a.p, nvec, out.p);
      else hipLaunchKernelGGL((bw_rows_kernel<10, 2>), dim3(512), dim3(256), 0, s, a.p, rows, rowvec, out.p);
    };
    for (int i = 0; i < 2; ++i) launch();
    POGS_HIP_CHECK(hipEventRecord(e0, s));
    for (int i = 0; i < reps; ++i) launch();
    POGS_HIP_CHECK(hipEventRecord(e1, s));
    POGS_HIP_CHECK(hipEventSynchronize(e1));
    float ms = 0;
    POGS_HIP_CHECK(hipEventElapsedTime(&ms, e0, e1));
    const double gbs = static_cast<double>(nvec) * 16.0 * reps / (static_cast<double>(ms) * 1e-3) / 1e9;
    if (gbs > best) { best = gbs; if (pattern) *pattern = pat; }
  }
  (void)hipEventDestroy(e0);
  (void)hipEventDestroy(e1);
  POGS_HIP_CHECK(hipDeviceSynchronize());
  return best;
}

namespace {
template <typename T>
__global__ void __launch_bounds__(256) wave_sum_check_kernel(const T *in, size_t n, T *out_alu, T *out_lds) {
  const size_t i = static_cast<size_t>(blockIdx.x) * 256 + threadIdx.x;
  if (i >= n) return;
  const T v = in[i];
  out_alu[i] = dev::wave_sum_valu(v);
  out_lds[i] = dev::wave_sum_shfl(v);
}
}
template <typename T>
void wave_sum_check(const T *in_host, size_t n, T *alu_host, T *lds_host) {
  POGS_CHECK(n > 0 && n % 64 == 0, "whole wavefronts of 64 values");
  DevBuf<T> in(n), a(n), b(n);
  hipStream_t s = nullptr;
  POGS_HIP_CHECK(hipMemcpyAsync(in.p, in_host, n * sizeof(T), hipMemcpyHostToDevice, s));
  hipLaunchKernelGGL((wave_sum_check_kernel<T>), dim3(static_cast<unsigned>((n + 255) / 256)), dim3(256), 0, s, in.p, n, a.p, b.p);
  POGS_HIP_CHECK(hipGetLastError());
  POGS_HIP_CHECK(hipMemcpyAsync(alu_host, a.p, n * sizeof(T), hipMemcpyDeviceToHost, s));
  POGS_HIP_CHECK(hipMemcpyAsync(lds_host, b.p, n * sizeof(T), hipMemcpyDeviceToHost, s));
  POGS_HIP_CHECK(hipDeviceSynchronize());
}
template void wave_sum_check<float>(const float *, size_t, float *, float *);
template void wave_sum_check<double>(const double *, size_t, double *, double *);

#define POGS_INST(T)                                                                                     \
  template void launch_scale_objective<T>(FnView<T>, T *, T *, T *, T *, const T *, int, bool, hipStream_t); \
  template void launch_admm_pre<T>(const AdmmPreArgs<T> &, hipStream_t);                                 \
  template FnUniform<T> probe_uniform<T>(FnView<T>, int, hipStream_t);                                   \
  template void launch_admm_tail<T>(int, const T *, const T *, const T *, T *, double *, hipStream_t);   \
  template void launch_func_eval<T>(int, FnView<T>, const T *, double *, hipStream_t);                   \
  template void launch_prox_eval<T>(int, FnView<T>, T, const T *, T *, hipStream_t);                     \
  template void launch_proj_subgrad<T>(int, FnView<T>, const T *, const T *, T *, hipStream_t);          \
  template void launch_unscale<T>(const UnscaleArgs<T> &, hipStream_t);                                  \
  template void launch_exact_u<T>(int, const T *, const T *, const T *, T, T *, hipStream_t);            \
  template void launch_fill<T>(T *, T, size_t, hipStream_t);                                             \
  template void launch_sqrt_inplace<T>(T *, size_t, hipStream_t);                                        \
  template void launch_scal<T>(T *, T, size_t, hipStream_t);                                             \
  template void launch_scale_by<T>(size_t, T, const T *, const T *, bool, T *, hipStream_t);             \
  template void launch_axpby<T>(size_t, T, const T *, T, T *, hipStream_t);
POGS_INST(float)
POGS_INST(double)
#undef POGS_INST

}
```

Baseline: 1493 it/s.

## Batch buffer zeroing, fork norm estimate onto aux stream, unroll scale_de loads

Replaces many per-buffer zero launches in setup and cold start with a single batched zero-list kernel. Adds an opt-in mode (POGS_AMD_SETUP_OVERLAP) that runs the Gram norm-estimate power iteration on an auxiliary stream alongside Cholesky/trtri, using a copy of the Gram matrix. Also restructures scale_de_kernel to issue four row loads before computing, for more memory-level parallelism. These mostly target setup cost; the ADMM iteration rate is largely unaffected, and the overlap path costs an extra Gram-sized buffer.

```diff
diff --git a/include/pogs_amd.h b/include/pogs_amd.h
--- a/include/pogs_amd.h
+++ b/include/pogs_amd.h
@@ -201,6 +201,7 @@
                void *y);
 int PogsAmdReadBandwidth(int device, size_t bytes, int reps, double *gb_per_s, int *pattern);
 int PogsAmdWaveSumCheck(int dtype, size_t n, const void *in_host, void *alu_host, void *lds_host);
+int PogsAmdZeroListCheck(int count, const size_t *offsets, const size_t *bytes, void *buf_host, size_t buf_bytes);
 
 int PogsAmdBatchRowsCheck(int dtype, int tri, int rows, int cols, const void *M, size_t ldm, int k, const int *act,
                           int nact, const void *X, size_t ldx, void *Y, size_t ldy);
diff --git a/pogs_amd/_lib.py b/pogs_amd/_lib.py
--- a/pogs_amd/_lib.py
+++ b/pogs_amd/_lib.py
@@ -135,6 +135,7 @@
 lib.PogsAmdRandUniform.argtypes = [c_int, c_size_t, c_void_p]
 lib.PogsAmdReadBandwidth.argtypes = [c_int, c_size_t, c_int, ctypes.POINTER(c_double), ctypes.POINTER(c_int)]
 lib.PogsAmdWaveSumCheck.argtypes = [c_int, c_size_t, c_void_p, c_void_p, c_void_p]
+lib.PogsAmdZeroListCheck.argtypes = [c_int, c_void_p, c_void_p, c_void_p, c_size_t]
 lib.PogsAmdBatchRowsCheck.argtypes = [c_int, c_int, c_int, c_int, c_void_p, c_size_t, c_int, c_void_p, c_int,
                                       c_void_p, c_size_t, c_void_p, c_size_t]
 lib.PogsAmdBatchColsCheck.argtypes = [c_int, c_int, c_int, c_void_p, c_size_t, c_int, c_void_p, c_int, c_void_p,
@@ -189,7 +190,7 @@
     "PogsAmdIterate", "PogsAmdSetWarmStart", "PogsAmdGetStats", "PogsAmdResetStats", "PogsAmdDestroy", "PogsAmdLastError",
     "PogsAmdPoolStats", "PogsAmdPoolTrim",
     "PogsAmdProxEval", "PogsAmdFuncEval", "PogsAmdProjSubgradEval", "PogsAmdGetEquil", "PogsAmdProject", "PogsAmdMul", "PogsAmdRandUniform",
-    "PogsAmdReadBandwidth", "PogsAmdWaveSumCheck", "PogsAmdBatchRowsCheck", "PogsAmdBatchColsCheck",
+    "PogsAmdReadBandwidth", "PogsAmdWaveSumCheck", "PogsAmdZeroListCheck", "PogsAmdBatchRowsCheck", "PogsAmdBatchColsCheck",
     "PogsAmdSpBatchSpmvCheck", "PogsAmdManySetupCheck", "PogsAmdGramCheck", "PogsAmdCholCheck",
     "PogsAmdSpmvCheck", "PogsAmdGetFactor",
 ]
@@ -210,6 +211,16 @@
     if lib.PogsAmdWaveSumCheck(0 if v.dtype == np.float32 else 1, v.size, v.ctypes.data, a.ctypes.data, b.ctypes.data) != 0:
         raise RuntimeError(last_error())
     return a, b
+
+
+def zero_list_check(buf, ranges):
+    import numpy as np
+    out = np.array(buf, dtype=np.uint8, order="C", copy=True)
+    off = np.ascontiguousarray([r[0] for r in ranges], dtype=np.uintp)
+    cnt = np.ascontiguousarray([r[1] for r in ranges], dtype=np.uintp)
+    if lib.PogsAmdZeroListCheck(len(ranges), off.ctypes.data, cnt.ctypes.data, out.ctypes.data, out.size) != 0:
+        raise RuntimeError(last_error())
+    return out
 
 
 def _dtype_code(*arrays):
diff --git a/pogs_amd/csrc/abi.hip b/pogs_amd/csrc/abi.hip
--- a/pogs_amd/csrc/abi.hip
+++ b/pogs_amd/csrc/abi.hip
@@ -563,6 +563,13 @@
   });
 }
 
+int PogsAmdZeroListCheck(int count, const size_t *offsets, const size_t *bytes, void *buf_host, size_t buf_bytes) {
+  return guarded([&]() {
+    zero_list_check(count, offsets, bytes, buf_host, buf_bytes);
+    return 0;
+  });
+}
+
 int PogsAmdBatchRowsCheck(int dtype, int tri, int rows, int cols, const void *M, size_t ldm, int k, const int *act,
                           int nact, const void *X, size_t ldx, void *Y, size_t ldy) {
   return guarded([&]() {
diff --git a/pogs_amd/csrc/dense_factor.h b/pogs_amd/csrc/dense_factor.h
--- a/pogs_amd/csrc/dense_factor.h
+++ b/pogs_amd/csrc/dense_factor.h
@@ -30,6 +30,10 @@
     ctx_.stats.gram_flops = static_cast<double>(kdim) * k_ * k_;
   }
   ctx_.tmark("gram");
+  if (overlap_) {
+    factor_forked(G, ld, tmp);
+    return;
+  }
   if (tall_) norm_est_gram(G, ld);
   else if (tmode_) norm_est_gram_wide(G, ld);
   ctx_.tmark("norm_est_gram");
@@ -48,6 +52,51 @@
   }
   ctx_.sync();
   ctx_.tmark("trtri");
+}
+
+template <typename T, typename Tag>
+void DenseSolver<T, Tag>::factor_forked(T *G, size_t ld, T *tmp) {
+  hipStream_t s = ctx_.stream, aux = ctx_.aux_stream();
+  struct Event {
+    hipEvent_t e = nullptr;
+    Event() { POGS_HIP_CHECK(hipEventCreate(&e)); }
+    ~Event() { if (e) (void)hipEventDestroy(e); }
+  } e0, e1;
+  const size_t slab = static_cast<size_t>(k_) * ld;
+  double y2 = 0, begin_ms = 0;
+  {
+    PhaseTimer pt(s);
+    if (tall_) norm_est_gram_begin(G, ld);
+    else y2 = norm_est_gram_wide_begin(G, ld);
+    begin_ms = pt.stop_ms();
+  }
+  DevBuf<T> Gn(slab);
+  POGS_HIP_CHECK(hipMemcpyAsync(Gn.p, G, slab * sizeof(T), hipMemcpyDeviceToDevice, s));
+  POGS_HIP_CHECK(hipEventRecord(e0.e, s));
+  POGS_HIP_CHECK(hipStreamWaitEvent(aux, e0.e, 0));
+  launch_add_diag<T>(G, ld, k_, static_cast<T>(1), s);
+  PhaseTimer pt_chol(s);
+  cholesky_lower<T>(G, ld, k_, Wp_, ld, s);
+  pt_chol.record_stop();
+  PhaseTimer pt_trtri(s);
+  trtri_lower<T>(G, ld, k_, Wp_, ld, tmp, s);
+  launch_transpose<T>(Wp_, ld, k_, k_, Up_, ld, s);
+  pt_trtri.record_stop();
+  PhaseTimer pt_ne(aux);
+  if (tall_) norm_est_gram_loop(Gn.p, ld, aux);
+  else norm_est_gram_wide_loop(Gn.p, ld, y2, aux);
+  pt_ne.record_stop();
+  POGS_HIP_CHECK(hipEventRecord(e1.e, aux));
+  POGS_HIP_CHECK(hipStreamWaitEvent(s, e1.e, 0));
+  ctx_.sync();
+  ctx_.stats.normest_ms = begin_ms + pt_ne.read_ms();
+  ctx_.stats.chol_ms = pt_chol.read_ms();
+  ctx_.stats.trtri_ms = pt_trtri.read_ms();
+  {
+    DevicePool::QuiescedScope quiet;
+    Gn.release();
+  }
+  ctx_.tmark("factor (forked)");
 }
 
 template <typename T, typename Tag>
diff --git a/pogs_amd/csrc/dense_iter.h b/pogs_amd/csrc/dense_iter.h
--- a/pogs_amd/csrc/dense_iter.h
+++ b/pogs_amd/csrc/dense_iter.h
@@ -35,8 +35,10 @@
 template <typename T, typename Tag>
 void DenseSolver<T, Tag>::cold_start() {
   hipStream_t s = ctx_.stream;
-  for (int i = 0; i < 2; ++i) { x_[i].zero(s); y_[i].zero(s); }
-  xt_.zero(s); yt_.zero(s); xtemp_.zero(s); ytemp_.zero(s);
+  ZeroBatch z(s);
+  for (int i = 0; i < 2; ++i) { z.add(x_[i]); z.add(y_[i]); }
+  z.add(xt_); z.add(yt_); z.add(xtemp_); z.add(ytemp_);
+  z.flush();
   cur_ = 0;
   zt_scale_ = 1;
   spec_valid_ = false;
diff --git a/pogs_amd/csrc/dense_setup.h b/pogs_amd/csrc/dense_setup.h
--- a/pogs_amd/csrc/dense_setup.h
+++ b/pogs_amd/csrc/dense_setup.h
@@ -58,37 +58,39 @@
   hipStream_t s = ctx_.stream;
   const size_t np = n_pad_;
   const size_t mp = m_pad_;
-  for (int i = 0; i < 2; ++i) { x_[i].alloc(np); y_[i].alloc(mp); x_[i].zero(s); y_[i].zero(s); }
+  ZeroBatch z(s);
+  for (int i = 0; i < 2; ++i) { x_[i].alloc(np); y_[i].alloc(mp); z.add(x_[i]); z.add(y_[i]); }
   xt_.alloc(np); yt_.alloc(mp); xtemp_.alloc(np); ytemp_.alloc(mp);
   const size_t kp = std::max<size_t>(np, k_pad_);
   x12_.alloc(np); y12_.alloc(mp); rhs_.alloc(kp); tvec_.alloc(kp); tmpn_.alloc(kp);
-  xt_.zero(s); yt_.zero(s); xtemp_.zero(s); ytemp_.zero(s); x12_.zero(s); y12_.zero(s);
-  rhs_.zero(s); tvec_.zero(s); tmpn_.zero(s);
-  d_.alloc(mp); d_.zero(s); e_.alloc(np); e_.zero(s);
-  if (tmode_) { uvec_.alloc(mp); uvec_.zero(s); }
+  z.add(xt_); z.add(yt_); z.add(xtemp_); z.add(ytemp_); z.add(x12_); z.add(y12_);
+  z.add(rhs_); z.add(tvec_); z.add(tmpn_);
+  d_.alloc(mp); z.add(d_); e_.alloc(np); z.add(e_);
+  if (tmode_) { uvec_.alloc(mp); z.add(uvec_); }
   xout_.alloc(np); yout_.alloc(m_); lout_.alloc(m_); muout_.alloc(np);
   f_.alloc(m_); g_.alloc(n_); fs_.alloc(m_); gs_.alloc(n_);
   colpart_.alloc(static_cast<size_t>(planA_.grid_max) * scols_pad_);
   ensure_xl(planA_, srows_, scols_pad_);
   if (use_cgls_) {
     cg_p_.alloc(np); cg_s_.alloc(np); cg_q_.alloc(m_); cg_r_.alloc(m_); cg_.alloc(kCgNumSlots);
-    cg_p_.zero(s); cg_s_.zero(s); cg_.zero(s);
+    z.add(cg_p_); z.add(cg_s_); z.add(cg_);
   }
   const char *fe = std::getenv("POGS_AMD_FUSED");
   fused_ok_ = (tall_ || tmode_) && !use_cgls_ && stream2_supported(planA_) && !(fe && fe[0] == '0');
   if (fused_ok_ && tmode_) {
     colpart2_.alloc(static_cast<size_t>(planA_.grid_max) * scols_pad_);
     x12s_.alloc(np); xtemps_.alloc(np);
-    x12s_.zero(s); xtemps_.zero(s);
+    z.add(x12s_); z.add(xtemps_);
   } else if (fused_ok_) {
     colpart2_.alloc(static_cast<size_t>(planA_.grid_max) * np);
     if (multi_) {
       pack_.alloc(2 * np + 8);
-      pack_.zero(s);
+      z.add(pack_);
     }
     y12s_.alloc(m_); ytemps_.alloc(m_);
-    y12s_.zero(s); ytemps_.zero(s);
-  }
+    z.add(y12s_); z.add(ytemps_);
+  }
+  z.flush();
   const size_t vb = vec_blocks(n_) + vec_blocks(m_);
   const size_t r01 = static_cast<size_t>(planA_.grid_max) * 6 + std::max<size_t>(4096, vb * 3 + 64);
   sp_pre_off_ = r01;
@@ -258,8 +260,15 @@
 
 template <typename T, typename Tag>
 void DenseSolver<T, Tag>::norm_est_gram(T *G, size_t ld) {
-  hipStream_t s = ctx_.stream;
-  PhaseTimer pt(s);
+  PhaseTimer pt(ctx_.stream);
+  norm_est_gram_begin(G, ld);
+  norm_est_gram_loop(G, ld, ctx_.stream);
+  ctx_.stats.normest_ms = pt.stop_ms();
+}
+
+template <typename T, typename Tag>
+void DenseSolver<T, Tag>::norm_est_gram_begin(T *G, size_t ld) {
+  hipStream_t s = ctx_.stream;
   launch_zero_upper<T>(G, ld, n_, s);
   ctx_.tmark("  ne: zero_upper");
   std::vector<T> x0(n_pad_, 0);
@@ -268,6 +277,10 @@
   POGS_HIP_CHECK(hipMemcpyAsync(xtemp_.p, x0.data(), n_pad_ * sizeof(T), hipMemcpyHostToDevice, s));
   ctx_.sync();
   ctx_.tmark("  ne: h2d");
+}
+
+template <typename T, typename Tag>
+void DenseSolver<T, Tag>::norm_est_gram_loop(const T *G, size_t ld, hipStream_t s) {
   T *xa = xtemp_.p, *xb = rhs_.p;
   const T kTol = static_cast<T>(1e-4);
   T norm_est = 0, last;
@@ -286,7 +299,7 @@
     launch_reduce_cols<T, SymColOp<T>>(colpart_.p, grid, n_pad_, SymColOp<T>{tvec_.p, xa, nrm, xb, n_}, sp, s);
     SumJob j{sp, reduce_cols_grid(n_pad_, Vec16<T>::N), 2, ctx_.S.p + kPowX2};
     launch_sum_jobs(&j, 1, s);
-    const double *S = ctx_.fetch_scalars();
+    const double *S = ctx_.fetch_scalars_on(s);
     const T normx = static_cast<T>(std::sqrt(S[kPowX2]));
     const T normSx = static_cast<T>(std::sqrt(S[kPowXGx]));
     norm_est = normx / normSx;
@@ -299,26 +312,36 @@
   xtemp_.zero(s);
   rhs_.zero(s);
   tvec_.zero(s);
+}
+
+template <typename T, typename Tag>
+void DenseSolver<T, Tag>::norm_est_gram_wide(T *G, size_t ld) {
+  PhaseTimer pt(ctx_.stream);
+  const double y2 = norm_est_gram_wide_begin(G, ld);
+  norm_est_gram_wide_loop(G, ld, y2, ctx_.stream);
   ctx_.stats.normest_ms = pt.stop_ms();
 }
 
 template <typename T, typename Tag>
-void DenseSolver<T, Tag>::norm_est_gram_wide(T *G, size_t ld) {
-  hipStream_t s = ctx_.stream;
-  PhaseTimer pt(s);
+double DenseSolver<T, Tag>::norm_est_gram_wide_begin(T *G, size_t ld) {
+  hipStream_t s = ctx_.stream;
   launch_zero_upper<T>(G, ld, k_, s);
   std::vector<T> x0(n_pad_, 0);
   rand_uniform_host(x0.data(), n_);
   POGS_HIP_CHECK(hipMemcpyAsync(xtemp_.p, x0.data(), n_pad_ * sizeof(T), hipMemcpyHostToDevice, s));
   ctx_.sync();
+  t_mul_n(xtemp_.p, nullptr, StoreNormRowOp<T>{ytemp_.p}, ctx_.S.p + kPowSx2);
+  ctx_.stats.matvecs_init += 1;
+  return ctx_.fetch_scalars()[kPowSx2];
+}
+
+template <typename T, typename Tag>
+void DenseSolver<T, Tag>::norm_est_gram_wide_loop(const T *G, size_t ld, double y2, hipStream_t s) {
   T *ya = ytemp_.p, *yb = uvec_.p;
-  t_mul_n(xtemp_.p, nullptr, StoreNormRowOp<T>{ya}, ctx_.S.p + kPowSx2);
-  ctx_.stats.matvecs_init += 1;
   const T kTol = static_cast<T>(1e-4);
   T norm_est = 0, last;
   const int grid = stream_grid<true, true>(planW_, k_);
   double *sp = ctx_.spart.p + static_cast<size_t>(planA_.grid_max) * 6;
-  double y2 = ctx_.fetch_scalars()[kPowSx2];
   unsigned i = 0;
   for (i = 0; i < 50; ++i) {
     last = norm_est;
@@ -335,7 +358,7 @@
     const double prev_w2 = (i == 0) ? y2 : ctx_.S_host.p[kPowX2];
     SumJob j{sp, reduce_cols_grid(k_pad_, Vec16<T>::N), 2, tmp2};
     launch_sum_jobs(&j, 1, s);
-    const double *S = ctx_.fetch_scalars();
+    const double *S = ctx_.fetch_scalars_on(s);
     y2 = prev_w2 / prev_xgx;
     norm_est = static_cast<T>(std::sqrt(S[kPowXGx])) / static_cast<T>(std::sqrt(y2));
     std::swap(ya, yb);
@@ -348,5 +371,4 @@
   ytemp_.zero(s);
   uvec_.zero(s);
   tvec_.zero(s);
-  ctx_.stats.normest_ms = pt.stop_ms();
-}
+}
diff --git a/pogs_amd/csrc/dense_solver.h b/pogs_amd/csrc/dense_solver.h
--- a/pogs_amd/csrc/dense_solver.h
+++ b/pogs_amd/csrc/dense_solver.h
@@ -27,27 +27,49 @@
 
 namespace {
 
+constexpr int kScaleDeU = 4;
 template <typename T, bool WRITE>
 __global__ void __launch_bounds__(256) scale_de_kernel(const T *src, T *dst, size_t lda, int m, int n_pad, const T *d,
                                                        const T *e, T post, double *partials, double *max_partials) {
   using V = typename Vec16<T>::type;
   constexpr int VEC = Vec16<T>::N;
+  constexpr int U = kScaleDeU;
   __shared__ double s_red[4];
   __shared__ double s_max[4];
   const int vpr = n_pad / VEC;
   double acc[1] = {0.0};
   T amax = 0;
-  for (int row = blockIdx.x; row < m; row += gridDim.x) {
-    const T di = d[row];
-    const T *rp = src + static_cast<size_t>(row) * lda;
-    for (int v = threadIdx.x; v < vpr; v += 256) {
-      V a = WRITE ? stream_load<V>(rp + v * VEC) : *reinterpret_cast<const V *>(rp + v * VEC);
-      const V ev = *reinterpret_cast<const V *>(e + v * VEC);
-      T *ap = reinterpret_cast<T *>(&a);
-      const T *ep = reinterpret_cast<const T *>(&ev);
+  const int per_row = (vpr + 255) / 256;
+  const int bx = static_cast<int>(blockIdx.x), gx = static_cast<int>(gridDim.x);
+  const int rows = bx < m ? (m - bx + gx - 1) / gx : 0;
+  int rl = 0, j = 0;
+  while (rl < rows) {
+    V a[U], ev[U];
+    T di[U];
+    int row[U], vv[U];
+    bool ok[U];
+#pragma unroll
+    for (int u = 0; u < U; ++u) {
+      const bool in_list = rl < rows;
+      const int rc = in_list ? rl : rows - 1;
+      const int v = j * 256 + static_cast<int>(threadIdx.x);
+      ok[u] = in_list && v < vpr;
+      if (++j == per_row) { j = 0; ++rl; }
+      row[u] = bx + rc * gx;
+      vv[u] = v < vpr ? v : vpr - 1;
+      const T *rp = src + static_cast<size_t>(row[u]) * lda;
+      a[u] = WRITE ? stream_load<V>(rp + vv[u] * VEC) : *reinterpret_cast<const V *>(rp + vv[u] * VEC);
+      ev[u] = *reinterpret_cast<const V *>(e + vv[u] * VEC);
+      di[u] = d[row[u]];
+    }
+#pragma unroll
+    for (int u = 0; u < U; ++u) {
+      if (!ok[u]) continue;
+      T *ap = reinterpret_cast<T *>(&a[u]);
+      const T *ep = reinterpret_cast<const T *>(&ev[u]);
 #pragma unroll
       for (int c = 0; c < VEC; ++c) {
-        const T val = ap[c] * (di * ep[c]);
+        const T val = ap[c] * (di[u] * ep[c]);
         if (WRITE) {
           ap[c] = val * post;
         } else {
@@ -55,7 +77,7 @@
           amax = fmax(amax, fabs(val));
         }
       }
-      if (WRITE) *reinterpret_cast<V *>(dst + static_cast<size_t>(row) * lda + v * VEC) = a;
+      if (WRITE) *reinterpret_cast<V *>(dst + static_cast<size_t>(row[u]) * lda + vv[u] * VEC) = a[u];
     }
   }
   if (WRITE) return;
@@ -109,6 +131,7 @@
     POGS_CHECK(tall_ || !multi_, "row sharding needs m > n (SURVEY.md section 8(e))");
     use_cgls_ = opt && opt->projector == POGS_AMD_PROJ_CGLS;
     if (const char *ys = std::getenv("POGS_AMD_YSYNC")) ysync_ = std::max(0, std::atoi(ys));
+    if (const char *so = std::getenv("POGS_AMD_SETUP_OVERLAP")) overlap_ = so[0] == '1';
     POGS_CHECK(!(use_cgls_ && multi_), "the CGLS projector is single-GPU");
     constexpr int VEC = Vec16<T>::N;
     n_pad_ = static_cast<int>(round_up(n, VEC));
@@ -413,10 +436,15 @@
   void norm_est();
 
   void norm_est_gram(T *G, size_t ld);
+  void norm_est_gram_begin(T *G, size_t ld);
+  void norm_est_gram_loop(const T *Gn, size_t ld, hipStream_t st);
 
   void norm_est_gram_wide(T *G, size_t ld);
+  double norm_est_gram_wide_begin(T *G, size_t ld);
+  void norm_est_gram_wide_loop(const T *Gn, size_t ld, double y2, hipStream_t st);
 
   void factor();
+  void factor_forked(T *G, size_t ld, T *tmp);
 
   template <typename TailOp>
   void solve_gram(const T *rhs, const T *add, const TailOp &tail, double *tail_scalars);
@@ -450,6 +478,7 @@
   Ctx ctx_;
   int m_ = 0, n_ = 0, n_pad_ = 0, k_ = 0, k_pad_ = 0;
   bool tall_ = true, multi_ = false, use_cgls_ = false;
+  bool overlap_ = false;
   double amax_ = 0;
   bool defer_sums_ = false;
   size_t sp_pre_off_ = 0, sp_tail_off_ = 0;
diff --git a/pogs_amd/csrc/engine.h b/pogs_amd/csrc/engine.h
--- a/pogs_amd/csrc/engine.h
+++ b/pogs_amd/csrc/engine.h
@@ -107,7 +107,11 @@
     POGS_HIP_CHECK(hipEventRecord(a, s));
   }
   double stop_ms() {
-    POGS_HIP_CHECK(hipEventRecord(b, s));
+    record_stop();
+    return read_ms();
+  }
+  void record_stop() { POGS_HIP_CHECK(hipEventRecord(b, s)); }
+  double read_ms() {
     POGS_HIP_CHECK(hipEventSynchronize(b));
     float ms = 0;
     POGS_HIP_CHECK(hipEventElapsedTime(&ms, a, b));
@@ -121,6 +125,7 @@
 
 struct CtxResources {
   hipStream_t stream = nullptr;
+  hipStream_t aux = nullptr;
   double *host = nullptr;
   int device = -1;
 };
@@ -130,6 +135,7 @@
   int device = 0;
   int num_cu = 256;
   hipStream_t stream = nullptr;
+  hipStream_t aux = nullptr;
   DistComm dist;
   size_t m_global = 0;
   DevBuf<double> S;
@@ -151,6 +157,7 @@
       for (size_t i = 0; i < pool.size(); ++i)
         if (pool[i].device == device) {
           stream = pool[i].stream;
+          aux = pool[i].aux;
           S_host.p = pool[i].host;
           pool.erase(pool.begin() + static_cast<long>(i));
           break;
@@ -176,6 +183,10 @@
     stream_timer.enable(profile != 0);
     stream_timer.set_every(profile > 1 ? static_cast<unsigned>(profile) : 1u);
   }
+  hipStream_t aux_stream() {
+    if (!aux) POGS_HIP_CHECK(hipStreamCreateWithFlags(&aux, hipStreamNonBlocking));
+    return aux;
+  }
   void ensure_spart(size_t count) {
     if (count > spart_cap) {
       POGS_HIP_CHECK(hipStreamSynchronize(stream));
@@ -192,7 +203,7 @@
     npending = 0;
   }
   void set_overlay(const ScalarOverlay &ov) { overlay = ov; }
-  const double *wait_publish(unsigned long long want) {
+  const double *wait_publish(unsigned long long want, hipStream_t st) {
     unsigned long long *seqp = reinterpret_cast<unsigned long long *>(S_host.p + kNumSlots);
     unsigned spins = 0, idle_seen = 0, checks = 0;
     double t_wait0 = 0;
@@ -212,7 +223,7 @@
             throw Error("row-sharded solve aborted: " + why);
           }
         }
-        const hipError_t q = hipStreamQuery(stream);
+        const hipError_t q = hipStreamQuery(st);
         if (q == hipSuccess) {
           if (__atomic_load_n(seqp, __ATOMIC_ACQUIRE) == want) break;
           if (++idle_seen >= 3) {
@@ -230,26 +241,28 @@
     }
     return S_host.p;
   }
-  const double *fetch_scalars() {
+  const double *fetch_scalars() { return fetch_scalars_on(stream); }
+  const double *fetch_scalars_on(hipStream_t st) {
     const ScalarOverlay ov = overlay;
     overlay = ScalarOverlay();
     if (!poll_fetch) {
-      flush_sums();
-      launch_apply_overlay(S.p, ov, stream);
-      POGS_HIP_CHECK(hipMemcpyAsync(S_host.p, S.p, kNumSlots * sizeof(double), hipMemcpyDeviceToHost, stream));
-      POGS_HIP_CHECK(hipStreamSynchronize(stream));
+      if (npending) launch_sum_jobs(pending, npending, st);
+      npending = 0;
+      launch_apply_overlay(S.p, ov, st);
+      POGS_HIP_CHECK(hipMemcpyAsync(S_host.p, S.p, kNumSlots * sizeof(double), hipMemcpyDeviceToHost, st));
+      POGS_HIP_CHECK(hipStreamSynchronize(st));
       return S_host.p;
     }
     const unsigned long long want = ++fetch_seq;
     if (npending) {
       launch_sum_publish(pending, npending, S.p, kNumSlots, S_host_dev,
-                         reinterpret_cast<unsigned long long *>(S_host_dev + kNumSlots), want, pub_counter.p, stream, ov);
+                         reinterpret_cast<unsigned long long *>(S_host_dev + kNumSlots), want, pub_counter.p, st, ov);
       npending = 0;
     } else {
       launch_publish_scalars(S.p, kNumSlots, S_host_dev, reinterpret_cast<unsigned long long *>(S_host_dev + kNumSlots),
-                             want, stream, ov);
-    }
-    return wait_publish(want);
+                             want, st, ov);
+    }
+    return wait_publish(want, st);
   }
   static double coll_timeout_s() {
     static const double v = [] {
@@ -298,16 +311,19 @@
   ~Ctx() {
     if (!stream) return;
     DeviceGuard guard(device);
-    const bool healthy = !poisoned && hipStreamSynchronize(stream) == hipSuccess;
+    const bool healthy = !poisoned && hipStreamSynchronize(stream) == hipSuccess &&
+                         (!aux || hipStreamSynchronize(aux) == hipSuccess);
     if (healthy) {
       std::lock_guard<std::mutex> lock(ctx_pool_mutex());
       CtxResources r;
       r.stream = stream;
+      r.aux = aux;
       r.host = S_host.p;
       r.device = device;
       ctx_pool().push_back(r);
     } else {
       (void)hipStreamDestroy(stream);
+      if (aux) (void)hipStreamDestroy(aux);
       if (S_host.p) (void)hipHostFree(S_host.p);
     }
   }
diff --git a/pogs_amd/csrc/vec_kernels.h b/pogs_amd/csrc/vec_kernels.h
--- a/pogs_amd/csrc/vec_kernels.h
+++ b/pogs_amd/csrc/vec_kernels.h
@@ -126,6 +126,34 @@
 
 template <typename T> void wave_sum_check(const T *in_host, size_t n, T *alu_host, T *lds_host);
 
+constexpr int kZeroListMax = 32;
+struct ZeroList {
+  void *p[kZeroListMax];
+  size_t bytes[kZeroListMax];
+  int n = 0;
+};
+void launch_zero_list(const ZeroList &l, hipStream_t s);
+class ZeroBatch {
+ public:
+  explicit ZeroBatch(hipStream_t s) : s_(s) {}
+  void add(void *p, size_t bytes) {
+    if (!bytes) return;
+    if (l_.n == kZeroListMax) flush();
+    l_.p[l_.n] = p;
+    l_.bytes[l_.n] = bytes;
+    ++l_.n;
+  }
+  template <typename T> void add(const DevBuf<T> &b) { add(b.p, b.n * sizeof(T)); }
+  void flush() {
+    if (l_.n) launch_zero_list(l_, s_);
+    l_.n = 0;
+  }
+ private:
+  hipStream_t s_;
+  ZeroList l_;
+};
+void zero_list_check(int count, const size_t *off, const size_t *bytes, void *buf_host, size_t buf_bytes);
+
 template <typename T> void launch_fill(T *p, T v, size_t n, hipStream_t s);
 void launch_fill_int(int *p, int v, size_t n, hipStream_t s);
 template <typename T> void launch_sqrt_inplace(T *p, size_t n, hipStream_t s);
diff --git a/pogs_amd/csrc/vec_kernels.hip b/pogs_amd/csrc/vec_kernels.hip
--- a/pogs_amd/csrc/vec_kernels.hip
+++ b/pogs_amd/csrc/vec_kernels.hip
@@ -432,6 +432,48 @@
 template <typename T>
 void launch_exact_u(int m, const T *y12, const T *yt, const T *yprev, T c, T *u, hipStream_t s) {
   if (m) hipLaunchKernelGGL(exact_u_vec_kernel<T>, dim3((m + 255) / 256), dim3(256), 0, s, m, y12, yt, yprev, c, u);
+}
+
+namespace {
+__global__ void __launch_bounds__(256) zero_list_kernel(ZeroList l) {
+  const int e = blockIdx.y;
+  char *p = static_cast<char *>(l.p[e]);
+  const size_t nb = l.bytes[e];
+  const size_t mis = reinterpret_cast<uintptr_t>(p) & 15;
+  size_t head = mis ? 16 - mis : 0;
+  if (head > nb) head = nb;
+  const size_t nvec = (nb - head) >> 4;
+  const size_t tail0 = head + (nvec << 4);
+  const size_t tid = static_cast<size_t>(blockIdx.x) * 256 + threadIdx.x, stride = static_cast<size_t>(gridDim.x) * 256;
+  uint4 *v = reinterpret_cast<uint4 *>(p + head);
+  for (size_t i = tid; i < nvec; i += stride) v[i] = make_uint4(0, 0, 0, 0);
+  if (tid < head) p[tid] = 0;
+  if (tid < nb - tail0) p[tail0 + tid] = 0;
+}
+}
+void launch_zero_list(const ZeroList &l, hipStream_t s) {
+  POGS_CHECK(l.n >= 0 && l.n <= kZeroListMax, "zero list");
+  if (!l.n) return;
+  size_t most = 0;
+  for (int i = 0; i < l.n; ++i) most = std::max(most, l.bytes[i]);
+  const unsigned gx = static_cast<unsigned>(std::min<size_t>(64, std::max<size_t>(1, (most + 16383) / 16384)));
+  ZeroList k = l;
+  for (int i = l.n; i < kZeroListMax; ++i) { k.p[i] = nullptr; k.bytes[i] = 0; }
+  hipLaunchKernelGGL(zero_list_kernel, dim3(gx, static_cast<unsigned>(l.n)), dim3(256), 0, s, k);
+}
+void zero_list_check(int count, const size_t *off, const size_t *bytes, void *buf_host, size_t buf_bytes) {
+  POGS_CHECK(count >= 0 && count <= kZeroListMax && (count == 0 || (off && bytes)) && buf_host && buf_bytes > 0,
+             "zero list check: 0 .. 32 ranges and a buffer");
+  for (int i = 0; i < count; ++i)
+    POGS_CHECK(off[i] <= buf_bytes && bytes[i] <= buf_bytes - off[i], "zero list check: a range leaves the buffer");
+  DevBuf<char> buf(buf_bytes);
+  POGS_HIP_CHECK(hipMemcpy(buf.p, buf_host, buf_bytes, hipMemcpyHostToDevice));
+  ZeroList l;
+  for (int i = 0; i < count; ++i) { l.p[i] = buf.p + off[i]; l.bytes[i] = bytes[i]; }
+  l.n = count;
+  launch_zero_list(l, nullptr);
+  POGS_HIP_CHECK(hipDeviceSynchronize());
+  POGS_HIP_CHECK(hipMemcpy(buf_host, buf.p, buf_bytes, hipMemcpyDeviceToHost));
 }
 
 template <typename T>
```

Result: no change. 1493 it/s (median of 3 runs) (+0.0%).
